# jacobwilliams/lbfgsb

Hardware: AMD Instinct MI355X
Metric: setulb iters/sec + achieved HBM GB/s on WS/WY matvec, n=1e8 m=10 (higher is better)
Workload: dtype f64; 1 GPU; separable bounded quadratic (SURVEY.md 8d), n=100000000, m=10, fp64, l=-1,u=1,x0=0, on-device objective; n=100000000, m=10, rows_per_gpu=100000000, parallelism=rows/1, collective=none, entry=lbfgsb_hip_setulb_dev_pp (ping-pong iterate buffers), defer_lnsrch=True

## Files before the change

### include/lbfgsb_hip_debug.h

```cpp
#ifndef LBFGSB_HIP_DEBUG_H
#define LBFGSB_HIP_DEBUG_H

#include "lbfgsb_hip.h"

#ifdef __cplusplus
extern "C" {
#endif

int lbfgsb_hip_wtv_launch_only(lbfgsb_hip_ctx *ctx, const void *v, int col, int head);
int lbfgsb_hip_wtv_time(lbfgsb_hip_ctx *ctx, const void *v, int col, int head, int reps,
                        double *h_ms_per_launch);
int lbfgsb_hip_kernel_time(lbfgsb_hip_ctx *ctx, int which, const void *x, const void *g, int col,
                           int head, int reps, double *h_ms_per_launch);

int lbfgsb_hip_stats(lbfgsb_hip_ctx *ctx, int64_t *launches, int64_t *syncs,
                     int64_t *cauchy_fullsorts, double *wait_seconds);

int lbfgsb_hip_freev_skipped(lbfgsb_hip_ctx *ctx, int64_t *count);
int lbfgsb_hip_bounds_stats(lbfgsb_hip_ctx *ctx, int64_t *checks, int64_t *changes, int64_t *rebuilds);

int lbfgsb_hip_comm_stats(lbfgsb_hip_ctx *ctx, int64_t *collectives, int64_t *bytes_contributed);

int lbfgsb_hip_path_counts(lbfgsb_hip_ctx *ctx, int64_t *closed_form, int64_t *three_pass,
                           int64_t *handed_windows);

int lbfgsb_hip_tie_splits(lbfgsb_hip_ctx *ctx, int64_t *count);

int lbfgsb_hip_host_gap(lbfgsb_hip_ctx *ctx, double *seconds, int64_t *count);
int lbfgsb_hip_compact_stats(lbfgsb_hip_ctx *ctx, int64_t *packs, int64_t *unpacks, int32_t *packed,
                             int32_t *eligible);
int lbfgsb_hip_collective_time(lbfgsb_hip_ctx *ctx, int reps, double *median_us, double *min_us);
int lbfgsb_hip_host_segments(lbfgsb_hip_ctx *ctx, double *seconds5);

int lbfgsb_hip_defer_stats(lbfgsb_hip_ctx *ctx, int64_t *deferred, int64_t *reissued);

int lbfgsb_hip_skip_stats(lbfgsb_hip_ctx *ctx, int64_t *scans_reused);

int lbfgsb_hip_pass_clock(lbfgsb_hip_ctx *ctx, int enable, double *ms_total, int64_t *count);

int lbfgsb_hip_refresh_count(lbfgsb_hip_ctx *ctx, int64_t *count);

#ifdef __cplusplus
}
#endif
#endif
```

### lbfgsb_amd/capi.py

```python
from __future__ import annotations

import ctypes as C
import os
import subprocess

HERE = os.path.dirname(os.path.abspath(__file__))
_LIB = None

_vp, _i32p, _dp, _cp = C.c_void_p, C.POINTER(C.c_int32), C.POINTER(C.c_double), C.c_char_p
ALLREDUCE_FN = C.CFUNCTYPE(C.c_int, C.c_void_p, C.POINTER(C.c_double), C.c_int, C.c_int, C.c_int)
ALLGATHER_FN = C.CFUNCTYPE(C.c_int, C.c_void_p, C.c_void_p, C.c_void_p, C.c_int64)
FG_FN = C.CFUNCTYPE(C.c_double, C.c_void_p, C.c_void_p, C.c_void_p)
PROTOTYPES = {
    "lbfgsb_hip_create": (C.c_int, [C.c_int64, C.c_int64, C.c_int64, C.c_int, C.c_int, C.c_int,
                                    _vp, C.POINTER(_vp)]),
    "lbfgsb_hip_destroy": (None, [_vp]),
    "lbfgsb_hip_last_error": (C.c_char_p, []),
    "lbfgsb_hip_rccl_unique_id": (C.c_int, [_vp]),
    "lbfgsb_hip_comm_init_rccl": (C.c_int, [_vp, _vp, C.c_int, C.c_int]),
    "lbfgsb_hip_comm_init_host": (C.c_int, [_vp, ALLREDUCE_FN, ALLGATHER_FN, _vp, C.c_int, C.c_int]),
    "lbfgsb_hip_setulb_dev": (C.c_int, [_vp, _vp, _vp, _vp, _vp, _vp, _vp, C.c_double, C.c_double,
                                        _vp, C.c_int, _vp, _vp, _vp, _vp]),
    "lbfgsb_hip_setulb_dev_pp": (C.c_int, [_vp, _vp, _vp, _vp, _vp, _vp, _vp, _vp, _vp, C.c_double,
                                           C.c_double, _vp, C.c_int, _vp, _vp, _vp, _vp, _vp]),
    "lbfgsb_hip_setulb_host": (C.c_int, [C.c_int32, C.c_int32, _vp, _vp, _vp, _vp, _vp, _vp,
                                         C.c_double, C.c_double, _vp, _vp, _vp, C.c_int32, _vp,
                                         _vp, _vp, _vp, _cp, C.c_int32, C.c_int32]),
    "lbfgsb_hip_setulb_host_ik": (C.c_int, [C.c_int64, C.c_int64, _vp, _vp, _vp, _vp, _vp, _vp,
                                            C.c_double, C.c_double, _vp, _vp, _vp, C.c_int64, _vp,
                                            _vp, _vp, _vp, _cp, C.c_int32, C.c_int32, C.c_int32]),
    "lbfgsb_hip_release_host_ik": (C.c_int, [_vp, C.c_int32]),
    "lbfgsb_hip_pass_clock": (C.c_int, [_vp, C.c_int, _vp, _vp]),
    "lbfgsb_hip_get_stream": (C.c_void_p, [_vp]),
    "lbfgsb_hip_wait_stream": (C.c_int, [_vp, _vp]),
    "lbfgsb_hip_release_host": (C.c_int, [_vp]),
    "lbfgsb_hip_host_pinning": (C.c_int, [C.c_int]),
    "lbfgsb_hip_return_event": (C.c_int, [_vp, _vp, C.c_int, _vp]),
    "lbfgsb_hip_f_device": (C.c_int, [_vp, _vp, _vp, C.c_int]),
    "lbfgsb_hip_tie_splits": (C.c_int, [_vp, _vp]),
    "lbfgsb_hip_defer_stats": (C.c_int, [_vp, _vp, _vp]),
    "lbfgsb_hip_host_gap": (C.c_int, [_vp, _vp, _vp]),
    "lbfgsb_hip_collective_time": (C.c_int, [_vp, C.c_int, _vp, _vp]),
    "lbfgsb_hip_compact_stats": (C.c_int, [_vp, _vp, _vp, _vp, _vp]),
    "lbfgsb_hip_host_segments": (C.c_int, [_vp, _vp]),
    "lbfgsb_hip_comm_info": (C.c_int, [_vp, _vp, _vp, _vp]),
    "lbfgsb_hip_path_counts": (C.c_int, [_vp, _vp, _vp, _vp]),
    "lbfgsb_hip_minimize": (C.c_int, [_vp, _vp, _vp, _vp, _vp, _vp, C.c_double, C.c_double, C.c_int,
                                      C.c_int, C.c_int, _vp, _vp, C.c_int, _vp, _vp, _vp, _vp, _vp]),
    "lbfgsb_hip_export_state": (C.c_int, [_vp, _vp, _vp]),
    "lbfgsb_hip_qn_apply": (C.c_int, [_vp, C.c_int, C.c_int64, _vp, C.c_int64, _vp, C.c_int64]),
    "lbfgsb_hip_qn_diag": (C.c_int, [_vp, C.c_int, _vp]),
    "lbfgsb_hip_qn_logdet": (C.c_int, [_vp, C.c_int, C.POINTER(C.c_double)]),
    "lbfgsb_hip_qn_draw": (C.c_int, [_vp, C.c_int, C.c_int64, C.c_uint64, C.c_int64, _vp, C.c_double, _vp,
                                     C.c_int64]),
    "lbfgsb_hip_qn_quad": (C.c_int, [_vp, C.c_int, C.c_int64, _vp, C.c_int64, _vp, C.POINTER(C.c_double)]),
    "lbfgsb_hip_qn_gram": (C.c_int, [_vp, C.c_int, C.c_int64, _vp, C.c_int64, _vp, C.POINTER(C.c_double),
                                     C.c_int64]),
    "lbfgsb_hip_qn_logpdf": (C.c_int, [_vp, C.c_int, C.c_int64, _vp, C.c_int64, _vp, C.c_double,
                                       C.POINTER(C.c_double)]),
    "lbfgsb_hip_qn_draw_logpdf": (C.c_int, [_vp, C.c_int, C.c_int64, C.c_uint64, C.c_int64, _vp, C.c_double, _vp,
                                            C.c_int64, C.POINTER(C.c_double)]),
    "lbfgsb_hip_qn_eig": (C.c_int, [_vp, C.c_int, C.c_int32, C.POINTER(C.c_int32), C.POINTER(C.c_double),
                                    C.POINTER(C.c_double)]),
    "lbfgsb_hip_qn_eigvec": (C.c_int, [_vp, C.c_int, C.c_int64, C.POINTER(C.c_int32), _vp, C.c_int64]),
    "lbfgsb_hip_kkt": (C.c_int, [_vp, _vp, _vp, _vp, _vp, _vp, C.c_double, _vp, _vp, _vp, _vp, _vp]),
    "lbfgsb_hip_kkt_list": (C.c_int, [_vp, _vp, C.c_int, _vp, C.c_int64, _vp]),
    "lbfgsb_hip_import_state": (C.c_int, [_vp, _vp, _vp, _vp]),
    "lbfgsb_hip_projgr": (C.c_int, [_vp, _vp, _vp, _vp, _vp, _vp, _vp]),
    "lbfgsb_hip_wtv": (C.c_int, [_vp, _vp, C.c_int, C.c_int, _vp]),
    "lbfgsb_hip_set_w": (C.c_int, [_vp, _vp, _vp]),
    "lbfgsb_hip_set_iwhere": (C.c_int, [_vp, _vp]),
    "lbfgsb_hip_formk_gram": (C.c_int, [_vp, C.c_int, C.c_int, _vp]),
    "lbfgsb_hip_wtv_launch_only": (C.c_int, [_vp, _vp, C.c_int, C.c_int]),
    "lbfgsb_hip_wtv_time": (C.c_int, [_vp, _vp, C.c_int, C.c_int, C.c_int, _vp]),
    "lbfgsb_hip_kernel_time": (C.c_int, [_vp, C.c_int, _vp, _vp, C.c_int, C.c_int, C.c_int, _vp]),
    "lbfgsb_hip_sync": (C.c_int, [_vp]),
    "lbfgsb_hip_objective": (C.c_int, [_vp, C.c_int, _vp, _vp, _vp]),
    "lbfgsb_hip_stats": (C.c_int, [_vp, _vp, _vp, _vp, _vp]),
    "lbfgsb_hip_set_option": (C.c_int, [_vp, _cp, C.c_double]),
    "lbfgsb_hip_comm_stats": (C.c_int, [_vp, _vp, _vp]),
    "lbfgsb_hip_uniform_bounds": (C.c_int, [_vp, _vp]),
    "lbfgsb_hip_bounds_changed": (C.c_int, [_vp]),
    "lbfgsb_hip_bounds_stats": (C.c_int, [_vp, _vp, _vp, _vp]),
    "lbfgsb_hip_freev_skipped": (C.c_int, [_vp, _vp]),
    "lbfgsb_hip_skip_stats": (C.c_int, [_vp, _vp]),
    "lbfgsb_hip_refresh_count": (C.c_int, [_vp, _vp]),
    "lbfgsb_hip_vec_sub": (C.c_int, [_vp, _vp, _vp, _vp]),
    "lbfgsb_hip_vec_scale": (C.c_int, [_vp, C.c_double, _vp]),
    "lbfgsb_hip_dot": (C.c_int, [_vp, _vp, _vp, _vp]),
    "lbfgsb_hip_active": (C.c_int, [_vp, _vp, _vp, _vp, _vp, _vp]),
    "lbfgsb_hip_errclb": (C.c_int, [_vp, _vp, _vp, _vp, C.c_double, _vp, _vp, _vp]),
    "lbfgsb_hip_cauchy": (C.c_int, [_vp, _vp, _vp, _vp, _vp, _vp, C.c_double, C.c_int, C.c_int, C.c_double,
                                    _vp, _vp, _vp]),
    "lbfgsb_hip_freev": (C.c_int, [_vp, C.c_int, C.c_int, C.c_int, _vp, _vp, _vp, _vp]),
    "lbfgsb_hip_formk": (C.c_int, [_vp, C.c_int, C.c_int, C.c_double, _vp]),
    "lbfgsb_hip_cmprlb": (C.c_int, [_vp, _vp, _vp, C.c_double, C.c_int, C.c_int, C.c_int, _vp, _vp]),
    "lbfgsb_hip_subsm": (C.c_int, [_vp, _vp, _vp, _vp, _vp, _vp, _vp, C.c_double, C.c_int, C.c_int, _vp, _vp,
                                   _vp]),
    "lbfgsb_hip_lnsrlb": (C.c_int, [_vp, _vp, _vp, _vp, _vp, _vp, C.c_double, _vp, _vp, _vp, _vp, _vp, _vp]),
    "lbfgsb_hip_matupd": (C.c_int, [_vp, _vp, C.c_double, C.c_double, C.c_double, _vp, _vp]),
}

E_NOGPU, E_ARG, E_ALLOC, E_COMM, E_STATE = -100, -101, -102, -103, -104
QN_B, QN_H = 0, 1
QN_B_SQRT, QN_H_SQRT = 4, 5
QN_ROOT_MAXCOL = 64
QN_EIG_CUT = 1e-8
KKT_CNT = ("n_unbounded", "n_free", "n_lower", "n_upper", "n_fixed", "n_binding", "n_weak", "n_leaving", "n_outside")
KKT_VAL = ("pg_max", "mult_max", "out_max", "gfree_max")
F_REAL32 = 1
F_MIRROR_INDEX = 2
F_NO_RETURN_SYNC = 4
F_PARALLEL_GCP = 8
F_EXACT_TIES = 16
F_INDEX_TIES = 32
F_DEFER_LNSRCH = 64
F_FOLLOW_BOUNDS = 128


class LbfgsbError(RuntimeError):
    pass


def lib_path() -> str:
    return os.environ.get("LBFGSB_HIP_LIBRARY") or os.path.join(HERE, "liblbfgsb_hip.so")


def build_library() -> str:
    subprocess.check_call(["make", "-s", "-C", os.path.join(HERE, "csrc")])
    return lib_path()


def load_library():
    global _LIB
    if _LIB is not None:
        return _LIB
    path = lib_path()
    if not os.path.exists(path):
        raise LbfgsbError("%s is missing: run lbfgsb_amd.build_library() (hipcc, gfx950). "
                          "There is no CPU fallback." % path)
    try:
        import torch
    except Exception:
        pass
    lib = C.CDLL(path, mode=C.RTLD_GLOBAL)
    for name, (res, args) in PROTOTYPES.items():
        fn = getattr(lib, name)
        fn.restype = res
        fn.argtypes = args
    _LIB = lib
    return lib


def check(rc: int):
    if rc != 0:
        msg = load_library().lbfgsb_hip_last_error()
        raise LbfgsbError("lbfgsb_hip error %d: %s" % (rc, (msg or b"").decode()))
```

### lbfgsb_amd/csrc/capi.hip

```cpp
#include "solver_base.hpp"

extern "C" {

const char *lbfgsb_hip_last_error(void) { return g_err.c_str(); }

int lbfgsb_hip_create(int64_t n_local, int64_t n_global, int64_t row0, int m, int flags,
                      int device, void *stream, lbfgsb_hip_ctx **out) {
  if (!out) return fail(LBFGSB_E_ARG, "out == NULL");
  *out = nullptr;
  if (n_local <= 0 || n_global < n_local || row0 < 0 || row0 + n_local > n_global)
    return fail(LBFGSB_E_ARG, "bad n_local / n_global / row0");
  if (m <= 0 || m > LBFGSB_MAX_M) return fail(LBFGSB_E_ARG, "m must be in 1..LBFGSB_MAX_M");
  if (n_local > (int64_t)INT32_MAX - 16) return fail(LBFGSB_E_ARG, "n_local must be < 2^31 - 16 rows per device");
  int rc = 0;
  *out = lbfgsb_make_solver(n_local, n_global, row0, m, flags, device, stream, &rc);
  if (!*out) return rc;
  return LBFGSB_OK;
}

void lbfgsb_hip_destroy(lbfgsb_hip_ctx *ctx) { delete ctx; }

int lbfgsb_hip_rccl_unique_id(void *id128) {
  if (!id128) return fail(LBFGSB_E_ARG, "rccl_unique_id: NULL argument");
  if (!g_rccl.load()) return fail(LBFGSB_E_COMM, "cannot load librccl");
// ... 194 lines not shown
  if (!qn_mode_ok(mode) && mode != LBFGSB_QN_B_SQRT && mode != LBFGSB_QN_H_SQRT)
    return fail(LBFGSB_E_ARG, "qn_apply: mode");
  if (k < 1 || ldv < ctx->n || ldo < ctx->n) return fail(LBFGSB_E_ARG, "qn_apply: k < 1 or ld < n_local");
  return ctx->qn_apply(mode, k, v, ldv, out, ldo);
}
int lbfgsb_hip_qn_diag(lbfgsb_hip_ctx *ctx, int mode, void *out) {
  if (!ctx || !out) return fail(LBFGSB_E_ARG, "qn_diag: NULL argument");
  if (!qn_mode_ok(mode)) return fail(LBFGSB_E_ARG, "qn_diag: mode");
  return ctx->qn_diag(mode, out);
}
int lbfgsb_hip_qn_logdet(lbfgsb_hip_ctx *ctx, int mode, double *h_logdet) {
  if (!ctx || !h_logdet) return fail(LBFGSB_E_ARG, "qn_logdet: NULL argument");
  if (!qn_mode_ok(mode)) return fail(LBFGSB_E_ARG, "qn_logdet: mode");
  return ctx->qn_logdet(mode, h_logdet);
}
int lbfgsb_hip_qn_draw(lbfgsb_hip_ctx *ctx, int mode, int64_t k, uint64_t seed, int64_t first, const void *mean,
                       double scale, void *out, int64_t ldo) {
  if (!ctx || !out) return fail(LBFGSB_E_ARG, "qn_draw: NULL argument");
  if (!qn_mode_ok(mode)) return fail(LBFGSB_E_ARG, "qn_draw: mode");
  if (k < 1 || first < 0 || ldo < ctx->n) return fail(LBFGSB_E_ARG, "qn_draw: k < 1, first < 0 or ldo < n_local");
  if (!std::isfinite(scale)) return fail(LBFGSB_E_ARG, "qn_draw: scale is not finite");
  return ctx->qn_draw(mode, k, seed, first, mean, scale, out, ldo);
}
int lbfgsb_hip_qn_quad(lbfgsb_hip_ctx *ctx, int mode, int64_t k, const void *v, int64_t ldv, const void *center,
                       double *h_q) {
  if (!ctx || !v || !h_q) return fail(LBFGSB_E_ARG, "qn_quad: NULL argument");
  if (!qn_mode_ok(mode)) return fail(LBFGSB_E_ARG, "qn_quad: mode");
  if (k < 1 || ldv < ctx->n) return fail(LBFGSB_E_ARG, "qn_quad: k < 1 or ldv < n_local");
  return ctx->qn_quad(mode, k, v, ldv, center, h_q);
}
int lbfgsb_hip_qn_logpdf(lbfgsb_hip_ctx *ctx, int mode, int64_t k, const void *x, int64_t ldx, const void *mean,
                         double scale, double *h_logp) {
  if (!ctx || !x || !h_logp) return fail(LBFGSB_E_ARG, "qn_logpdf: NULL argument");
  if (!qn_mode_ok(mode)) return fail(LBFGSB_E_ARG, "qn_logpdf: mode");
  if (k < 1 || ldx < ctx->n) return fail(LBFGSB_E_ARG, "qn_logpdf: k < 1 or ldx < n_local");
  if (!std::isfinite(scale) || scale == 0.0) return fail(LBFGSB_E_ARG, "qn_logpdf: scale is 0 or not finite");
  return ctx->qn_logpdf(mode, k, x, ldx, mean, scale, h_logp);
}
int lbfgsb_hip_qn_draw_logpdf(lbfgsb_hip_ctx *ctx, int mode, int64_t k, uint64_t seed, int64_t first,
                              const void *mean, double scale, void *out, int64_t ldo, double *h_logp) {
  if (!ctx || !out || !h_logp) return fail(LBFGSB_E_ARG, "qn_draw_logpdf: NULL argument");
  if (!qn_mode_ok(mode)) return fail(LBFGSB_E_ARG, "qn_draw_logpdf: mode");
  if (k < 1 || first < 0 || ldo < ctx->n)
    return fail(LBFGSB_E_ARG, "qn_draw_logpdf: k < 1, first < 0 or ldo < n_local");
  if (!std::isfinite(scale) || scale == 0.0)
    return fail(LBFGSB_E_ARG, "qn_draw_logpdf: scale is 0 or not finite");
  return ctx->qn_draw_logpdf(mode, k, seed, first, mean, scale, out, ldo, h_logp);
}
int lbfgsb_hip_qn_gram(lbfgsb_hip_ctx *ctx, int mode, int64_t k, const void *v, int64_t ldv, const void *center,
                       double *h_g, int64_t ldg) {
  if (!ctx || !v || !h_g) return fail(LBFGSB_E_ARG, "qn_gram: NULL argument");
  if (!qn_mode_ok(mode)) return fail(LBFGSB_E_ARG, "qn_gram: mode");
  if (k < 1 || k > LBFGSB_QN_GRAM_MAXK) return fail(LBFGSB_E_ARG, "qn_gram: k < 1 or k > LBFGSB_QN_GRAM_MAXK");
  if (ldv < ctx->n || ldg < k) return fail(LBFGSB_E_ARG, "qn_gram: ldv < n_local or ldg < k");
  return ctx->qn_vgram(mode, k, v, ldv, center, h_g, ldg);
}
int lbfgsb_hip_qn_eig(lbfgsb_hip_ctx *ctx, int mode, int32_t cap, int32_t *h_r, double *h_bulk, double *h_lambda) {
  if (!ctx || !h_r || !h_bulk) return fail(LBFGSB_E_ARG, "qn_eig: NULL argument");
  if (!qn_mode_ok(mode)) return fail(LBFGSB_E_ARG, "qn_eig: mode");
  if (cap < 0 || (cap > 0 && !h_lambda)) return fail(LBFGSB_E_ARG, "qn_eig: cap < 0, or cap > 0 without h_lambda");
  return ctx->qn_eig(mode, cap, h_r, h_bulk, h_lambda);
}
int lbfgsb_hip_qn_eigvec(lbfgsb_hip_ctx *ctx, int mode, int64_t k, const int32_t *h_which, void *out, int64_t ldo) {
  if (!ctx || !out) return fail(LBFGSB_E_ARG, "qn_eigvec: NULL argument");
  if (!qn_mode_ok(mode)) return fail(LBFGSB_E_ARG, "qn_eigvec: mode");
  if (k < 1 || k > 128 || ldo < ctx->n) return fail(LBFGSB_E_ARG, "qn_eigvec: k < 1, k > 128 or ldo < n_local");
  return ctx->qn_eigvec(mode, k, h_which, out, ldo);
}

int lbfgsb_hip_kkt(lbfgsb_hip_ctx *ctx, const void *x, const void *l, const void *u, const int32_t *nbd,
                   const void *g, double tol, void *pg_out, void *mult_out, int8_t *status_out, int64_t *h_cnt,
                   double *h_val) {
  if (!ctx || !x || !l || !u || !nbd || !g || !h_cnt || !h_val) return fail(LBFGSB_E_ARG, "kkt: NULL argument");
  if (!(tol >= 0.0)) return fail(LBFGSB_E_ARG, "kkt: tol is negative or NaN");
  return ctx->kkt(x, l, u, nbd, g, tol, pg_out, mult_out, status_out, h_cnt, h_val);
}
int lbfgsb_hip_kkt_list(lbfgsb_hip_ctx *ctx, const int8_t *status, int code_mask, int64_t *idx_out, int64_t cap,
                        int64_t *h_count) {
  if (!ctx || !status || !h_count) return fail(LBFGSB_E_ARG, "kkt_list: NULL argument");
  if (code_mask < 0 || code_mask > 31) return fail(LBFGSB_E_ARG, "kkt_list: code_mask has bits beyond the five codes");
  if (cap < 0 || (cap > 0 && !idx_out)) return fail(LBFGSB_E_ARG, "kkt_list: cap < 0, or cap > 0 without idx_out");
  return ctx->kkt_list(status, code_mask, idx_out, cap, h_count);
}

int lbfgsb_hip_projgr(lbfgsb_hip_ctx *ctx, const void *x, const void *l, const void *u,
                      const int32_t *nbd, const void *g, double *h_sbgnrm) {
  if (!ctx || !x || !l || !u || !nbd || !g || !h_sbgnrm) return fail(LBFGSB_E_ARG, "projgr: NULL argument");
  return ctx->k_projgr(x, l, u, nbd, g, h_sbgnrm);
}
int lbfgsb_hip_vec_sub(lbfgsb_hip_ctx *ctx, const void *a, const void *b, void *out) {
  if (!ctx || !a || !b || !out) return fail(LBFGSB_E_ARG, "vec_sub: NULL argument");
  return ctx->r_vec_sub(a, b, out);
}
int lbfgsb_hip_vec_scale(lbfgsb_hip_ctx *ctx, double alpha, void *v) {
  if (!ctx || !v) return fail(LBFGSB_E_ARG, "vec_scale: NULL argument");
  return ctx->r_vec_scale(alpha, v);
}
int lbfgsb_hip_dot(lbfgsb_hip_ctx *ctx, const void *a, const void *b, double *h_result) {
  if (!ctx || !a || !b || !h_result) return fail(LBFGSB_E_ARG, "dot: NULL argument");
  return ctx->r_dot(a, b, h_result);
}
int lbfgsb_hip_active(lbfgsb_hip_ctx *ctx, void *x, const void *l, const void *u, const int32_t *nbd,
                      int32_t *h_flags) {
  if (!ctx || !x || !l || !u || !nbd || !h_flags) return fail(LBFGSB_E_ARG, "active: NULL argument");
  return ctx->r_active(x, l, u, nbd, h_flags);
}
int lbfgsb_hip_errclb(lbfgsb_hip_ctx *ctx, const void *l, const void *u, const int32_t *nbd, double factr,
                      char *task, int32_t *h_info, int64_t *h_k) {
  if (!ctx || !l || !u || !nbd || !task || !h_info || !h_k) return fail(LBFGSB_E_ARG, "errclb: NULL argument");
  return ctx->r_errclb(l, u, nbd, factr, task, h_info, h_k);
}
int lbfgsb_hip_cauchy(lbfgsb_hip_ctx *ctx, const void *x, const void *l, const void *u, const int32_t *nbd,
                      const void *g, double theta, int col, int head, double sbgnrm, void *xcp_out,
                      int32_t *h_nseg, int32_t *h_info) {
  if (!ctx || !x || !l || !u || !nbd || !g || !h_nseg || !h_info)
    return fail(LBFGSB_E_ARG, "cauchy: NULL argument");
  return ctx->r_cauchy(x, l, u, nbd, g, theta, col, head, sbgnrm, xcp_out, h_nseg, h_info);
}
int lbfgsb_hip_freev(lbfgsb_hip_ctx *ctx, int iter, int cnstnd, int updatd, int64_t *h_nfree,
                     int64_t *h_nenter, int64_t *h_ileave, int32_t *h_wrk) {
  if (!ctx || !h_nfree || !h_nenter || !h_ileave || !h_wrk) return fail(LBFGSB_E_ARG, "freev: NULL argument");
  return ctx->r_freev(iter, cnstnd, updatd, h_nfree, h_nenter, h_ileave, h_wrk);
}
int lbfgsb_hip_formk(lbfgsb_hip_ctx *ctx, int col, int head, double theta, int32_t *h_info) {
  if (!ctx || !h_info) return fail(LBFGSB_E_ARG, "formk: NULL argument");
  return ctx->r_formk(col, head, theta, h_info);
}
int lbfgsb_hip_cmprlb(lbfgsb_hip_ctx *ctx, const void *x, const void *g, double theta, int col, int head,
                      int cnstnd, void *r_out, int32_t *h_info) {
  if (!ctx || !x || !g || !h_info) return fail(LBFGSB_E_ARG, "cmprlb: NULL argument");
  return ctx->r_cmprlb(x, g, theta, col, head, cnstnd, r_out, h_info);
}
int lbfgsb_hip_subsm(lbfgsb_hip_ctx *ctx, const void *x, const void *l, const void *u, const int32_t *nbd,
                     const void *g, const void *r_in, double theta, int col, int head, void *xhat_out,
                     int32_t *h_iword, int32_t *h_info) {
  if (!ctx || !x || !l || !u || !nbd || !g || !r_in || !h_iword || !h_info)
    return fail(LBFGSB_E_ARG, "subsm: NULL argument");
  return ctx->r_subsm(x, l, u, nbd, g, r_in, theta, col, head, xhat_out, h_iword, h_info);
}
int lbfgsb_hip_lnsrlb(lbfgsb_hip_ctx *ctx, void *x, const void *l, const void *u, const int32_t *nbd,
                      const void *g, double f, double *h_sc, int32_t *h_ic, char *task, char *csave,
                      int32_t *h_isave2, double *h_dsave13) {
  if (!ctx || !x || !l || !u || !nbd || !g || !h_sc || !h_ic || !task || !csave || !h_isave2 || !h_dsave13)
    return fail(LBFGSB_E_ARG, "lnsrlb: NULL argument");
  return ctx->r_lnsrlb(x, l, u, nbd, g, f, h_sc, h_ic, task, csave, h_isave2, h_dsave13);
}
int lbfgsb_hip_matupd(lbfgsb_hip_ctx *ctx, const void *g, double stp, double dr, double dtd, int32_t *h_ip,
                      double *h_theta) {
  if (!ctx || !g || !h_ip || !h_theta) return fail(LBFGSB_E_ARG, "matupd: NULL argument");
  return ctx->r_matupd(g, stp, dr, dtd, h_ip, h_theta);
}

int lbfgsb_hip_wtv(lbfgsb_hip_ctx *ctx, const void *v, int col, int head, double *h_out) {
  if (!ctx || !v || !h_out) return fail(LBFGSB_E_ARG, "wtv: NULL argument");
  return ctx->k_wtv(v, col, head, h_out, false);
}
int lbfgsb_hip_wtv_launch_only(lbfgsb_hip_ctx *ctx, const void *v, int col, int head) {
  if (!ctx || !v) return fail(LBFGSB_E_ARG, "wtv: NULL argument");
  return ctx->k_wtv(v, col, head, nullptr, true);
}
int lbfgsb_hip_wtv_time(lbfgsb_hip_ctx *ctx, const void *v, int col, int head, int reps,
                        double *h_ms_per_launch) {
  if (!ctx || !v || !h_ms_per_launch || reps < 1) return fail(LBFGSB_E_ARG, "wtv_time: bad arguments");
  HIPCHK(hipSetDevice(ctx->device));
  hipEvent_t e0 = nullptr, e1 = nullptr;
  GpuOwner tmp;
  HIPCHK(tmp.event(&e0));
  HIPCHK(tmp.event(&e1));
  for (int k = 0; k < 3; ++k) CHK(ctx->k_wtv(v, col, head, nullptr, true));
  HIPCHK(hipEventRecord(e0, ctx->q.stream));
  for (int k = 0; k < reps; ++k) CHK(ctx->k_wtv(v, col, head, nullptr, true));
  HIPCHK(hipEventRecord(e1, ctx->q.stream));
  HIPCHK(hipEventSynchronize(e1));
  float ms = 0.f;
  HIPCHK(hipEventElapsedTime(&ms, e0, e1));
  *h_ms_per_launch = (double)ms / reps;
  return 0;
}
int lbfgsb_hip_kernel_time(lbfgsb_hip_ctx *ctx, int which, const void *x, const void *g, int col,
                           int head, int reps, double *h_ms_per_launch) {
  if (!ctx || !x || !g || !h_ms_per_launch || reps < 1) return fail(LBFGSB_E_ARG, "kernel_time: bad arguments");
  HIPCHK(hipSetDevice(ctx->device));
  hipEvent_t e0 = nullptr, e1 = nullptr;
  GpuOwner tmp;
  HIPCHK(tmp.event(&e0));
  HIPCHK(tmp.event(&e1));
  for (int k = 0; k < 2; ++k) CHK(ctx->k_launch(which, x, g, col, head));
  HIPCHK(hipEventRecord(e0, ctx->q.stream));
  for (int k = 0; k < reps; ++k) CHK(ctx->k_launch(which, x, g, col, head));
  HIPCHK(hipEventRecord(e1, ctx->q.stream));
  HIPCHK(hipEventSynchronize(e1));
  float ms = 0.f;
  HIPCHK(hipEventElapsedTime(&ms, e0, e1));
  *h_ms_per_launch = (double)ms / reps;
  return 0;
}
int lbfgsb_hip_set_w(lbfgsb_hip_ctx *ctx, const void *h_ws, const void *h_wy) {
  if (!ctx || !h_ws || !h_wy) return fail(LBFGSB_E_ARG, "set_w: NULL argument");
  return ctx->k_set_w(h_ws, h_wy);
}
int lbfgsb_hip_set_iwhere(lbfgsb_hip_ctx *ctx, const int32_t *h_iwhere) {
  if (!ctx || !h_iwhere) return fail(LBFGSB_E_ARG, "set_iwhere: NULL argument");
  return ctx->k_set_iwhere(h_iwhere);
}
int lbfgsb_hip_formk_gram(lbfgsb_hip_ctx *ctx, int col, int head, double *h_out) {
  if (!ctx || !h_out) return fail(LBFGSB_E_ARG, "formk_gram: NULL argument");
  return ctx->k_formk_gram(col, head, h_out);
}
int lbfgsb_hip_sync(lbfgsb_hip_ctx *ctx) {
  if (!ctx) return fail(LBFGSB_E_ARG, "ctx == NULL");
  return ctx->sync();
}
int lbfgsb_hip_objective(lbfgsb_hip_ctx *ctx, int kind, const void *x, void *g, double *h_f) {
  if (!ctx || !x || !g) return fail(LBFGSB_E_ARG, "objective: NULL argument");
  return ctx->k_objective(kind, x, g, h_f);
}
int lbfgsb_hip_stats(lbfgsb_hip_ctx *ctx, int64_t *launches, int64_t *syncs,
                     int64_t *cauchy_fullsorts, double *wait_seconds) {
  if (!ctx) return fail(LBFGSB_E_ARG, "ctx == NULL");
  if (launches) *launches = ctx->q.launches;
  if (syncs) *syncs = ctx->nsync;
  if (cauchy_fullsorts) *cauchy_fullsorts = ctx->nfullsort;
  if (wait_seconds) *wait_seconds = ctx->t_wait;
  return 0;
}

int lbfgsb_hip_comm_stats(lbfgsb_hip_ctx *ctx, int64_t *collectives, int64_t *bytes_contributed) {
  if (!ctx) return fail(LBFGSB_E_ARG, "ctx == NULL");
  if (collectives) *collectives = ctx->ncoll;
  if (bytes_contributed) *bytes_contributed = ctx->coll_bytes;
  return 0;
}

int lbfgsb_hip_freev_skipped(lbfgsb_hip_ctx *ctx, int64_t *count) {
  if (!ctx || !count) return fail(LBFGSB_E_ARG, "freev_skipped: NULL argument");
  *count = ctx->freev_skipped();
  return 0;
}

int lbfgsb_hip_skip_stats(lbfgsb_hip_ctx *ctx, int64_t *scans_reused) {
  if (!ctx || !scans_reused) return fail(LBFGSB_E_ARG, "skip_stats: NULL argument");
  *scans_reused = ctx->skip_scans_reused();
  return 0;
}

int lbfgsb_hip_uniform_bounds(lbfgsb_hip_ctx *ctx, int32_t *mask) {
  if (!ctx || !mask) return fail(LBFGSB_E_ARG, "uniform_bounds: NULL argument");
  *mask = ctx->uniform_mask();
  return 0;
}

int lbfgsb_hip_bounds_changed(lbfgsb_hip_ctx *ctx) {
  if (!ctx) return fail(LBFGSB_E_ARG, "ctx == NULL");
  return ctx->bounds_changed();
}

int lbfgsb_hip_bounds_stats(lbfgsb_hip_ctx *ctx, int64_t *checks, int64_t *changes, int64_t *rebuilds) {
  if (!ctx) return fail(LBFGSB_E_ARG, "ctx == NULL");
  int64_t a = 0, b = 0, c = 0;
  ctx->bounds_stats(a, b, c);
  if (checks) *checks = a;
  if (changes) *changes = b;
  if (rebuilds) *rebuilds = c;
  return 0;
}

int lbfgsb_hip_path_counts(lbfgsb_hip_ctx *ctx, int64_t *closed_form, int64_t *three_pass,
                           int64_t *handed_windows) {
  if (!ctx) return fail(LBFGSB_E_ARG, "ctx == NULL");
  if (handed_windows) *handed_windows = ctx->nspecwin;
  int64_t a = 0, b = 0;
  ctx->path_counts(a, b);
  if (closed_form) *closed_form = a;
  if (three_pass) *three_pass = b;
  return 0;
}

int lbfgsb_hip_set_option(lbfgsb_hip_ctx *ctx, const char *name, double value) {
  if (!ctx || !name) return fail(LBFGSB_E_ARG, "set_option: NULL argument");
  return ctx->set_option(name, value);
}

int lbfgsb_hip_tie_splits(lbfgsb_hip_ctx *ctx, int64_t *count) {
  if (!ctx || !count) return fail(LBFGSB_E_ARG, "tie_splits: NULL argument");
  *count = ctx->ntiesplit;
  return 0;
}

int lbfgsb_hip_collective_time(lbfgsb_hip_ctx *ctx, int reps, double *median_us, double *min_us) {
  if (!ctx) return fail(LBFGSB_E_ARG, "ctx == NULL");
  return ctx->collective_time(reps, median_us, min_us);
}

int lbfgsb_hip_compact_stats(lbfgsb_hip_ctx *ctx, int64_t *packs, int64_t *unpacks, int32_t *packed,
                              int32_t *eligible) {
  if (!ctx) return fail(LBFGSB_E_ARG, "ctx == NULL");
  int64_t a = 0, b = 0;
  int c = 0, d = 0;
  ctx->compact_stats(a, b, c, d);
  if (packs) *packs = a;
  if (unpacks) *unpacks = b;
  if (packed) *packed = c;
  if (eligible) *eligible = d;
  return 0;
}

int lbfgsb_hip_refresh_count(lbfgsb_hip_ctx *ctx, int64_t *count) {
  if (!ctx || !count) return fail(LBFGSB_E_ARG, "refresh_count: NULL argument");
  *count = ctx->nrefresh;
  return 0;
}

int lbfgsb_hip_host_gap(lbfgsb_hip_ctx *ctx, double *seconds, int64_t *count) {
  if (!ctx) return fail(LBFGSB_E_ARG, "ctx == NULL");
  if (seconds) *seconds = ctx->t_mid;
  if (count) *count = ctx->n_mid;
  return 0;
}
int lbfgsb_hip_host_segments(lbfgsb_hip_ctx *ctx, double *seconds5) {
  if (!ctx || !seconds5) return fail(LBFGSB_E_ARG, "host_segments: NULL argument");
  for (int k = 0; k < 5; ++k) seconds5[k] = ctx->t_seg[k];
  return 0;
}

int lbfgsb_hip_defer_stats(lbfgsb_hip_ctx *ctx, int64_t *deferred, int64_t *reissued) {
  if (!ctx) return fail(LBFGSB_E_ARG, "ctx == NULL");
  int64_t a = 0, b = 0;
  ctx->defer_counts(a, b);
  if (deferred) *deferred = a;
  if (reissued) *reissued = b;
  return 0;
}

int lbfgsb_hip_pass_clock(lbfgsb_hip_ctx *ctx, int enable, double *ms_total, int64_t *count) {
  if (!ctx) return fail(LBFGSB_E_ARG, "ctx == NULL");
  HIPCHK(hipSetDevice(ctx->device));
  ctx->clk_stream = ctx->q.stream;
  if (enable == 1) {
    for (int k = 0; k < 3; ++k) {
      ctx->clk_ms[k] = 0.0, ctx->clk_n[k] = 0;
      for (bool &pnd : ctx->clk_pending[k]) pnd = false;
    }
    ctx->clk_dropped = 0;
    ctx->clock_on = true;
  } else {
    HIPCHK(hipStreamSynchronize(ctx->q.stream));
    ctx->clk_collect();
    if (enable == 0) ctx->clock_on = false;
  }
  for (int k = 0; k < 3; ++k) {
    if (ms_total) ms_total[k] = ctx->clk_ms[k];
    if (count) count[k] = ctx->clk_n[k];
  }
  return 0;
}

namespace {
constexpr int32_t HOST_TAG = 0x4C424642;
struct HostRegistry {
  std::mutex mu;
  std::unordered_map<int32_t, lbfgsb_hip_ctx *> live;
  int32_t next_id = 1;
  ~HostRegistry() { live.clear(); }
  int32_t add(lbfgsb_hip_ctx *c) {
    std::lock_guard<std::mutex> lk(mu);
    while (live.count(next_id) || next_id <= 0) next_id = next_id == INT32_MAX ? 1 : next_id + 1;
    live[next_id] = c;
    return next_id;
  }
  lbfgsb_hip_ctx *find(const int32_t *isave) {
    if (isave[17] != HOST_TAG) return nullptr;
    std::lock_guard<std::mutex> lk(mu);
    auto it = live.find(isave[16]);
    return it == live.end() ? nullptr : it->second;
  }
  void drop(int32_t *isave) {
    lbfgsb_hip_ctx *c = nullptr;
    if (isave[17] == HOST_TAG) {
      std::lock_guard<std::mutex> lk(mu);
      auto it = live.find(isave[16]);
      if (it != live.end()) {
        c = it->second;
        live.erase(it);
      }
    }
    delete c;
    isave[16] = isave[17] = 0;
  }
};
HostRegistry g_host;
std::atomic<int> g_host_pinning{1};

void drop_runs_overlapping(const void *const *ptr, const size_t *bytes, int cnt) {
  std::vector<lbfgsb_hip_ctx *> dead;
  {
    std::lock_guard<std::mutex> lk(g_host.mu);
    for (auto it = g_host.live.begin(); it != g_host.live.end();) {
      bool hit = false;
      for (const auto &r : it->second->host_reg)
        for (int k = 0; k < cnt && !hit; ++k)
          hit = r.p && ptr[k] && (const char *)ptr[k] < (const char *)r.p + r.bytes &&
                (const char *)r.p < (const char *)ptr[k] + bytes[k];
      if (hit) {
        dead.push_back(it->second);
        it = g_host.live.erase(it);
      } else {
        ++it;
      }
    }
  }
  for (lbfgsb_hip_ctx *c : dead) delete c;
}
}

int lbfgsb_hip_host_pinning(int mode) {
  if (mode != 0 && mode != 1) return fail(LBFGSB_E_ARG, "host_pinning: mode must be 0 or 1");
  g_host_pinning.store(mode);
  return 0;
}

int lbfgsb_hip_release_host(int32_t *isave) {
  if (!isave) return fail(LBFGSB_E_ARG, "isave == NULL");
  g_host.drop(isave);
  return 0;
}

static int setulb_host_impl(int64_t n, int64_t m, void *x, const void *l, const void *u, const void *nbd_,
                            void *f, void *g, double factr, double pgtol, void *wa, void *iwa_, char *task,
                            int32_t iprint, char *csave, void *lsave_, void *isave_, void *dsave,
                            const char *iteration_file, int32_t real_bytes, int32_t mirror, int int_bytes) {
  const bool r32 = real_bytes == 4;
  if (!x || !l || !u || !nbd_ || !f || !g || !task || !csave || !lsave_ || !isave_ || !dsave)
    return fail(LBFGSB_E_ARG, "setulb: NULL argument");
  if (mirror && (!wa || !iwa_)) return fail(LBFGSB_E_ARG, "setulb: mirror = 1 needs wa and iwa");
  if (real_bytes != 4 && real_bytes != 8) return fail(LBFGSB_E_ARG, "real_bytes must be 4 or 8");
  if (int_bytes != 4 && int_bytes != 8) return fail(LBFGSB_E_ARG, "int_bytes must be 4 or 8");
  const bool i8 = int_bytes == 8;
  const size_t rb = (size_t)real_bytes;
  int32_t isave[44], lsave[4];
  auto geti = [&](const void *p, int k) -> int64_t {
    return i8 ? ((const int64_t *)p)[k] : (int64_t)((const int32_t *)p)[k];
  };
  auto puti = [&](void *p, int k, int64_t v) {
    if (i8)
      ((int64_t *)p)[k] = v;
    else
      ((int32_t *)p)[k] = (int32_t)std::min<int64_t>(std::max<int64_t>(v, INT32_MIN), INT32_MAX);
  };
  for (int k = 0; k < 44; ++k) {
    const int64_t v = geti(isave_, k);
    isave[k] = (int32_t)std::min<int64_t>(std::max<int64_t>(v, INT32_MIN), INT32_MAX);
  }
  for (int k = 0; k < 4; ++k) lsave[k] = geti(lsave_, k) != 0;
  int64_t off64[16] = {0};
  bool have_off = false;
  auto finish_ints = [&]() {
    for (int k = 0; k < 44; ++k) puti(isave_, k, isave[k]);
    if (have_off)
      for (int k = 0; k < 16; ++k) puti(isave_, k, off64[k]);
    for (int k = 0; k < 4; ++k) puti(lsave_, k, lsave[k]);
  };
  auto upload_nbd = [&](int32_t *dst) -> int {
    std::vector<int32_t> nb;
    if (i8) {
      nb.resize((size_t)n);
      const int64_t *src = (const int64_t *)nbd_;
      for (int64_t k = 0; k < n; ++k) nb[(size_t)k] = (src[k] < 0 || src[k] > 3) ? -1 : (int32_t)src[k];
    }
    HIPCHK(hipMemcpy(dst, i8 ? (const void *)nb.data() : nbd_, (size_t)n * 4, hipMemcpyHostToDevice));
    return 0;
  };
  lbfgsb_hip_ctx *ctx = nullptr;
  const bool start = lbh::str60_eq(task, "START");
  if (start) {
    g_host.drop(isave);
    if (n <= 0 || m <= 0) {
      if (n <= 0) lbh::str60_set(task, "ERROR: N <= 0");
      if (m <= 0) lbh::str60_set(task, "ERROR: M <= 0");
      finish_ints();
      return 0;
    }
    if (m > LBFGSB_MAX_M) {
      lbh::str60_set(task, "ERROR: M > 1024 (LIMIT OF LBFGSB_HIP)");
      finish_ints();
      return 0;
    }
    if (n > (int64_t)INT32_MAX - 16) {
      lbh::str60_set(task, "ERROR: N >= 2**31 ON ONE DEVICE (LIMIT OF LBFGSB_HIP)");
      finish_ints();
      return 0;
    }
    int fl = (r32 ? LBFGSB_F_REAL32 : 0) | (mirror ? LBFGSB_F_MIRROR_INDEX : 0) | LBFGSB_F_NO_RETURN_SYNC;
    int rc = lbfgsb_hip_create(n, n, 0, (int)m, fl, 0, nullptr, &ctx);
    if (rc) return rc;
    if (g_host_pinning.load()) {
      void *tslot = (wa && !mirror) ? (char *)wa + (size_t)(2ll * m * n + 11ll * m * m + 3ll * n) * rb : nullptr;
      const void *pv[3] = {x, g, tslot};
      const size_t pb[3] = {(size_t)n * rb, (size_t)n * rb, (size_t)n * rb};
      drop_runs_overlapping(pv, pb, 3);
      ctx->host_register(0, x, pb[0]);
      ctx->host_register(1, g, pb[1]);
      if (tslot) ctx->host_register(2, tslot, pb[2]);
    }
    if (iteration_file && iteration_file[0]) ctx->itfile_name = iteration_file;
    const size_t vb = ((size_t)n + 32) * rb;
    auto stage = [&]() -> int {
      HIPCHK(ctx->own.device(&ctx->hx, vb));
      HIPCHK(ctx->own.device(&ctx->hg, vb));
      HIPCHK(ctx->own.device(&ctx->hl, vb));
      HIPCHK(ctx->own.device(&ctx->hu, vb));
      HIPCHK(ctx->own.device(&ctx->hnbd, ((size_t)n + 32) * 4));
      HIPCHK(hipMemset(ctx->hg, 0, vb));
      HIPCHK(hipMemcpy(ctx->hx, x, (size_t)n * rb, hipMemcpyHostToDevice));
      HIPCHK(hipMemcpy(ctx->hl, l, (size_t)n * rb, hipMemcpyHostToDevice));
      HIPCHK(hipMemcpy(ctx->hu, u, (size_t)n * rb, hipMemcpyHostToDevice));
      return upload_nbd(ctx->hnbd);
    };
    rc = stage();
    if (rc) {
      lbfgsb_hip_destroy(ctx);
      return rc;
    }
    std::memset(isave, 0, sizeof isave);
    isave[16] = g_host.add(ctx);
    isave[17] = HOST_TAG;
  } else {
    ctx = g_host.find(isave);
    if (!ctx || ctx->n != n || ctx->m != m)
      return fail(LBFGSB_E_STATE, "setulb called without a live context (task must be START first)");
    ctx->host_unregister_if_not(0, x);
    ctx->host_unregister_if_not(1, g);
    if (wa && !mirror)
      ctx->host_unregister_if_not(2, (char *)wa + (size_t)(2ll * m * n + 11ll * m * m + 3ll * n) * rb);
    if (lbh::str60_pre(task, "NEW_X") && (isave[29] == 1 || (isave[29] > 0 && isave[29] % 32 == 0))) {
      void *tl = nullptr, *tu = nullptr;
      int32_t *tn = nullptr;
      GpuOwner tmp;
      double ndiff = 0.0;
      auto check = [&]() -> int {
        const size_t vb = ((size_t)n + 32) * rb;
        HIPCHK(tmp.device(&tl, vb));
        HIPCHK(tmp.device(&tu, vb));
        HIPCHK(tmp.device(&tn, ((size_t)n + 32) * 4));
        HIPCHK(hipMemcpy(tl, l, (size_t)n * rb, hipMemcpyHostToDevice));
        HIPCHK(hipMemcpy(tu, u, (size_t)n * rb, hipMemcpyHostToDevice));
        CHK(upload_nbd(tn));
        return ctx->bounds_same(ctx->hl, ctx->hu, ctx->hnbd, tl, tu, tn, &ndiff);
      };
      int rcc = check();
      if (rcc && (!tl || !tu || !tn)) {
        (void)hipGetLastError();
        rcc = 0, ndiff = 0.0;
      }
      if (rcc) return rcc;
      if (ndiff != 0.0) {
        lbh::str60_set(task, "ERROR: BOUNDS CHANGED DURING RUN");
        if (iprint >= 0) std::printf("\n l, u or nbd were modified during the run (%.0f rows differ from the arrays of task = 'START').\n", ndiff);
        g_host.drop(isave);
        finish_ints();
        return 0;
      }
    }
    if (lbh::str60_pre(task, "FG"))
      HIPCHK(hipMemcpyAsync(ctx->hg, g, (size_t)n * rb, hipMemcpyHostToDevice, ctx->q.stream));
  }
  {
    const int64_t mn = m * n, mm = m * m;
    const int64_t lws = 1, lwy = lws + mn, lsy = lwy + mn, lss = lsy + mm, lwt = lss + mm,
                  lwn = lwt + mm, lsnd = lwn + 4 * mm, lz = lsnd + 4 * mm, lr = lz + n, ld_ = lr + n,
                  lt = ld_ + n, lxp = lt + n, lwa = lxp + n;
    const int64_t v[16] = {mn, mm, 4 * mm, lws, lwy, lsy, lss, lwt, lwn, lsnd, lz, lr, ld_, lt, lxp, lwa};
    std::memcpy(off64, v, sizeof off64);
    have_off = true;
  }
  const int32_t keep_id = isave[16], keep_tag = isave[17];
  double fd = r32 ? (double)*(float *)f : *(double *)f;
  double ds[29];
  for (int i = 0; i < 29; ++i) ds[i] = r32 ? (double)((float *)dsave)[i] : ((double *)dsave)[i];
  ctx->restored_xg = false;
  const int64_t setups0 = ctx->n_ls_setup;
  int rc = ctx->setulb_dev(ctx->hx, ctx->hl, ctx->hu, ctx->hnbd, &fd, ctx->hg, factr, pgtol, task,
                           iprint, csave, lsave, isave, ds);
  isave[16] = keep_id, isave[17] = keep_tag;
  if (iprint >= 0) std::fflush(stdout);
  if (rc) {
    if (start) g_host.drop(isave);
    return rc;
  }
  for (int i = 0; i < 29; ++i) {
    if (r32)
      ((float *)dsave)[i] = (float)ds[i];
    else
      ((double *)dsave)[i] = ds[i];
  }
  if (r32)
    *(float *)f = (float)fd;
  else
    *(double *)f = fd;
  hipStream_t st = ctx->q.stream;
  const bool x_back = start || ctx->restored_xg || lbh::str60_pre(task, "FG_LN");
  if (x_back) HIPCHK(hipMemcpyAsync(x, ctx->hx, (size_t)n * rb, hipMemcpyDeviceToHost, st));
  if (ctx->restored_xg) HIPCHK(hipMemcpyAsync(g, ctx->hg, (size_t)n * rb, hipMemcpyDeviceToHost, st));
  if (mirror) {
    HIPCHK(hipStreamSynchronize(st));
    if (i8) {
      std::vector<int32_t> iw((size_t)3 * (size_t)n);
// ... 56 lines not shown
```

### lbfgsb_amd/csrc/device_util.hpp

```cpp
#pragma once
#include <hip/hip_runtime.h>
#include <stdint.h>

#include <type_traits>

namespace lbk {

template <typename T>
struct VecOf;
template <>
struct VecOf<double> {
  static constexpr int V = 2;
};
template <>
struct VecOf<float> {
  static constexpr int V = 4;
};

template <int W>
using WTag = std::integral_constant<int, W>;

template <int W>
__device__ __forceinline__ void ld(const double *p, double (&o)[W]) {
  if constexpr (W == 2) {
// ... 87 lines not shown
  } else {
#pragma unroll
    for (int k = 0; k < W; ++k) __builtin_nontemporal_store(o[k], p + k);
  }
}
template <int W>
__device__ __forceinline__ void stnt(float *p, const double (&o)[W]) {
  if constexpr (W == 4) {
    typedef float f4 __attribute__((ext_vector_type(4)));
    f4 v = {(float)o[0], (float)o[1], (float)o[2], (float)o[3]};
    __builtin_nontemporal_store(v, reinterpret_cast<f4 *>(p));
  } else if constexpr (W == 2) {
    typedef float f2 __attribute__((ext_vector_type(2)));
    f2 v = {(float)o[0], (float)o[1]};
    __builtin_nontemporal_store(v, reinterpret_cast<f2 *>(p));
  } else {
#pragma unroll
    for (int k = 0; k < W; ++k) __builtin_nontemporal_store((float)o[k], p + k);
  }
}
template <int W>
__device__ __forceinline__ void ldi(const int32_t *p, int (&o)[W]) {
  if constexpr (W == 2) {
    int2 v = *reinterpret_cast<const int2 *>(p);
    o[0] = v.x;
    o[1] = v.y;
  } else if constexpr (W == 4) {
    int4 v = *reinterpret_cast<const int4 *>(p);
    o[0] = v.x;
    o[1] = v.y;
    o[2] = v.z;
    o[3] = v.w;
  } else {
#pragma unroll
    for (int k = 0; k < W; ++k) o[k] = p[k];
  }
}
template <int W>
__device__ __forceinline__ void ldi(const int8_t *p, int (&o)[W]) {
  if constexpr (W == 2) {
    const char2 v = *reinterpret_cast<const char2 *>(p);
    o[0] = v.x, o[1] = v.y;
  } else if constexpr (W == 4) {
    const char4 v = *reinterpret_cast<const char4 *>(p);
    o[0] = v.x, o[1] = v.y, o[2] = v.z, o[3] = v.w;
  } else {
#pragma unroll
    for (int k = 0; k < W; ++k) o[k] = p[k];
  }
}
template <int W>
__device__ __forceinline__ void sti(int8_t *p, const int (&o)[W]) {
  if constexpr (W == 2) {
    *reinterpret_cast<char2 *>(p) = make_char2((signed char)o[0], (signed char)o[1]);
  } else if constexpr (W == 4) {
    *reinterpret_cast<char4 *>(p) =
        make_char4((signed char)o[0], (signed char)o[1], (signed char)o[2], (signed char)o[3]);
  } else {
#pragma unroll
    for (int k = 0; k < W; ++k) p[k] = (int8_t)o[k];
  }
}
template <int W>
__device__ __forceinline__ void sti(int32_t *p, const int (&o)[W]) {
  if constexpr (W == 2) {
    *reinterpret_cast<int2 *>(p) = make_int2(o[0], o[1]);
  } else if constexpr (W == 4) {
    *reinterpret_cast<int4 *>(p) = make_int4(o[0], o[1], o[2], o[3]);
  } else {
#pragma unroll
    for (int k = 0; k < W; ++k) p[k] = o[k];
  }
}

typedef int i32x2_t __attribute__((ext_vector_type(2)));
typedef int i32x4_t __attribute__((ext_vector_type(4)));
template <int BYTES>
struct RawReg;
template <>
struct RawReg<16> {
  i32x4_t v;
};
template <>
struct RawReg<8> {
  i32x2_t v;
};
template <>
struct RawReg<4> {
  int v;
};
template <>
struct RawReg<2> {
  int v;
};
template <>
struct RawReg<1> {
  int v;
};
template <int BYTES, bool NT>
__device__ __forceinline__ void raw_issue(RawReg<BYTES> &r, const void *p) {
  if constexpr (BYTES == 16) {
    if constexpr (NT)
      r.v = __builtin_nontemporal_load(reinterpret_cast<const i32x4_t *>(p));
    else
      r.v = *reinterpret_cast<const i32x4_t *>(p);
  } else if constexpr (BYTES == 8) {
    if constexpr (NT)
      r.v = __builtin_nontemporal_load(reinterpret_cast<const i32x2_t *>(p));
    else
      r.v = *reinterpret_cast<const i32x2_t *>(p);
  } else if constexpr (BYTES == 4) {
    if constexpr (NT)
      r.v = __builtin_nontemporal_load(reinterpret_cast<const int *>(p));
    else
      r.v = *reinterpret_cast<const int *>(p);
  } else if constexpr (BYTES == 2) {
    r.v = (int)*reinterpret_cast<const unsigned short *>(p);
  } else {
    r.v = (int)*reinterpret_cast<const signed char *>(p);
  }
}
template <bool NT>
__device__ __forceinline__ void raw_issue_half(RawReg<16> &r, int half, const void *p) {
  i32x2_t v;
  if constexpr (NT)
    v = __builtin_nontemporal_load(reinterpret_cast<const i32x2_t *>(p));
  else
    v = *reinterpret_cast<const i32x2_t *>(p);
  if (half == 0)
    r.v.xy = v;
  else
    r.v.zw = v;
}
template <bool NT>
__device__ __forceinline__ void raw_issue_half_at(RawReg<16> &r, int half, const void *base, uint32_t byte_off) {
  raw_issue_half<NT>(r, half, (const char *)base + byte_off);
}
template <int N>
__device__ __forceinline__ void raw_wait() {
  __builtin_amdgcn_sched_barrier(0);
}
template <int BYTES>
__device__ __forceinline__ void raw_land(RawReg<BYTES> &) {}
template <int W>
__device__ __forceinline__ void raw_get(const RawReg<8 * W> &r, const double *, double (&o)[W]) {
  if constexpr (W == 2) {
    typedef double d2 __attribute__((ext_vector_type(2)));
    const d2 v = __builtin_bit_cast(d2, r.v);
    o[0] = v.x, o[1] = v.y;
  } else {
    static_assert(W == 1, "fp64: 1 or 2 rows per lane");
    o[0] = __builtin_bit_cast(double, r.v);
  }
}
template <int W>
__device__ __forceinline__ void raw_get(const RawReg<4 * W> &r, const float *, double (&o)[W]) {
  if constexpr (W == 4) {
    typedef float f4 __attribute__((ext_vector_type(4)));
    const f4 v = __builtin_bit_cast(f4, r.v);
    o[0] = v.x, o[1] = v.y, o[2] = v.z, o[3] = v.w;
  } else if constexpr (W == 2) {
    typedef float f2 __attribute__((ext_vector_type(2)));
    const f2 v = __builtin_bit_cast(f2, r.v);
    o[0] = v.x, o[1] = v.y;
  } else {
    static_assert(W == 1, "fp32: 1, 2 or 4 rows per lane");
    o[0] = __builtin_bit_cast(float, r.v);
  }
}
template <int W>
__device__ __forceinline__ void raw_geti(const RawReg<4 * W> &r, const int32_t *, int (&o)[W]) {
  if constexpr (W == 4) {
    o[0] = r.v.x, o[1] = r.v.y, o[2] = r.v.z, o[3] = r.v.w;
  } else if constexpr (W == 2) {
    o[0] = r.v.x, o[1] = r.v.y;
  } else {
    o[0] = r.v;
  }
}
template <int W>
__device__ __forceinline__ void raw_geti(const RawReg<W> &r, const int8_t *, int (&o)[W]) {
#pragma unroll
  for (int k = 0; k < W; ++k) o[k] = (int)(signed char)((unsigned)r.v >> (8 * k));
}
template <typename E, int W>
using RawOf = RawReg<(int)sizeof(E) * W>;

__device__ __forceinline__ int pair_xchg(int v) { return __builtin_amdgcn_update_dpp(0, v, 0xB1, 0xf, 0xf, true); }
__device__ __forceinline__ double pair_xchg(double v) {
  const long long b = __builtin_bit_cast(long long, v);
  const unsigned lo = (unsigned)pair_xchg((int)b), hi = (unsigned)pair_xchg((int)(b >> 32));
  return __builtin_bit_cast(double, (long long)(((unsigned long long)hi << 32) | lo));
}
__device__ __forceinline__ float pair_xchg(float v) {
  return __builtin_bit_cast(float, pair_xchg(__builtin_bit_cast(int, v)));
}
__device__ __forceinline__ void half_pair(int v, int &lo, int &hi) {
  const auto r = __builtin_amdgcn_permlane32_swap((unsigned)v, (unsigned)v, false, false);
  lo = (int)r[0], hi = (int)r[1];
}
__device__ __forceinline__ void half_pair(int64_t v, int64_t &lo, int64_t &hi) {
  int l0, h0, l1, h1;
  half_pair((int)v, l0, h0);
  half_pair((int)(v >> 32), l1, h1);
  lo = (int64_t)(((unsigned long long)(unsigned)l1 << 32) | (unsigned)l0);
  hi = (int64_t)(((unsigned long long)(unsigned)h1 << 32) | (unsigned)h0);
}
__device__ __forceinline__ void half_pair(double v, double &lo, double &hi) {
  int64_t l, h;
  half_pair(__builtin_bit_cast(int64_t, v), l, h);
  lo = __builtin_bit_cast(double, l), hi = __builtin_bit_cast(double, h);
}
__device__ __forceinline__ void half_pair(float v, float &lo, float &hi) {
  int l, h;
  half_pair(__builtin_bit_cast(int, v), l, h);
  lo = __builtin_bit_cast(float, l), hi = __builtin_bit_cast(float, h);
}
template <typename T, int MC>
struct RowsPer {
  static constexpr int V = MC >= 20 ? VecOf<T>::V / 2 : VecOf<T>::V;
};
template <typename T, int MC, int NACC>
struct RowsPerAcc {
  static constexpr int V0 = RowsPer<T, MC>::V;
  static constexpr int V =
      (V0 > 1 && (V0 / 2) * (int)sizeof(T) >= 8 && 2 * (2 * MC * V0 + NACC) > 240) ? V0 / 2 : V0;
};

template <typename T, int V = VecOf<T>::V, typename F>
__device__ __forceinline__ void for_rows(int64_t n, F &&f) {
  const int64_t nv = n / V;
  const int64_t stride = (int64_t)gridDim.x * blockDim.x;
  const int64_t t0 = (int64_t)blockIdx.x * blockDim.x + threadIdx.x;
  for (int64_t iv = t0; iv < nv; iv += stride) f(iv * V, WTag<V>{});
  const int64_t it = nv * V + t0;
  if (it < n) f(it, WTag<1>{});
}

template <typename TripV, typename Trip1, int V, bool PIPE, int NS, typename Ctx, typename F>
__device__ __forceinline__ void for_rows_raw(int64_t n, const Ctx &c, F &&f) {
  const int64_t nv = n / V;
  const int64_t stride = (int64_t)gridDim.x * blockDim.x;
  const int64_t t0 = (int64_t)blockIdx.x * blockDim.x + threadIdx.x;
  if constexpr (PIPE) {
    static_assert(TripV::NL + NS <= 63, "vmcnt counts to 63");
    if (t0 < nv) {
      TripV A, B;
      A.issue(c, t0 * V);
      int64_t n1 = t0 + stride;
      B.issue(c, (n1 < nv ? n1 : t0) * V);
      raw_wait<TripV::NL>();
      A.land();
      f(A, t0 * V, WTag<V>{});
      while (n1 < nv) {
        const int64_t n2 = n1 + stride;
        A.issue(c, (n2 < nv ? n2 : n1) * V);
        raw_wait<TripV::NL + NS>();
        B.land();
        f(B, n1 * V, WTag<V>{});
        if (n2 >= nv) break;
        const int64_t n3 = n2 + stride;
        B.issue(c, (n3 < nv ? n3 : n2) * V);
        raw_wait<TripV::NL + NS>();
        A.land();
        f(A, n2 * V, WTag<V>{});
        n1 = n3;
      }
      raw_wait<0>();
      A.land();
      B.land();
    }
  } else {
    for (int64_t iv = t0; iv < nv; iv += stride) {
      TripV A;
      A.issue(c, iv * V);
      raw_wait<0>();
      A.land();
      f(A, iv * V, WTag<V>{});
    }
  }
  const int64_t it = nv * V + t0;
  if (it < n) {
    Trip1 C;
    C.issue(c, it);
    raw_wait<0>();
    C.land();
    f(C, it, WTag<1>{});
  }
}

struct CwTile {
  int64_t tb;
  uint64_t m0, m1;
};
__device__ __forceinline__ void cw_slots(const CwTile &t, int (&sl)[2], bool (&lf)[2]) {
  const int lane = (int)(threadIdx.x & 63);
  const int c0 = __popcll(t.m0), tf = c0 + __popcll(t.m1);
  const int b0 = (int)__builtin_amdgcn_mbcnt_hi((uint32_t)(t.m0 >> 32), __builtin_amdgcn_mbcnt_lo((uint32_t)t.m0, 0u));
  const int b1 = c0 + (int)__builtin_amdgcn_mbcnt_hi((uint32_t)(t.m1 >> 32), __builtin_amdgcn_mbcnt_lo((uint32_t)t.m1, 0u));
  lf[0] = (t.m0 >> lane) & 1ull, lf[1] = (t.m1 >> lane) & 1ull;
  sl[0] = lf[0] ? b0 : tf + (lane - b0);
  sl[1] = lf[1] ? b1 : tf + (64 + lane - b1);
}
__device__ __forceinline__ int64_t wave_uniform(int64_t v) {
  return (int64_t)(((uint64_t)(uint32_t)__builtin_amdgcn_readfirstlane((int)(v >> 32)) << 32) |
                   (uint32_t)__builtin_amdgcn_readfirstlane((int)v));
}
template <typename Trip2, typename Trip1, typename Ctx, typename F>
__device__ __forceinline__ void for_tiles_cw(int64_t n, const Ctx &c, const uint64_t *__restrict__ lmask, F &&f) {
  const int lane = threadIdx.x & 63;
  const int64_t nfull = n >> 7;
  const int64_t stride = (int64_t)gridDim.x * (blockDim.x >> 6);
  const int64_t t0 = wave_uniform((int64_t)blockIdx.x * (blockDim.x >> 6) + (threadIdx.x >> 6));
  if (t0 < nfull) {
    uint64_t m0 = lmask[2 * t0], m1 = lmask[2 * t0 + 1];
    for (int64_t tr = t0;;) {
      const int64_t nx = tr + stride;
      const bool more = nx < nfull;
      const int64_t nxc = more ? nx : tr;
      const uint64_t m0n = lmask[2 * nxc], m1n = lmask[2 * nxc + 1];
      Trip2 A;
      A.issue_cw(c, CwTile{tr << 7, m0, m1});
      raw_wait<0>();
      A.land();
      f(A, tr << 7, WTag<2>{});
      if (!more) break;
      tr = nx, m0 = m0n, m1 = m1n;
    }
  }
  if ((n & 127) != 0 && t0 == nfull % stride) {
    const CwTile t{nfull << 7, lmask[2 * nfull], lmask[2 * nfull + 1]};
    int sl[2];
    bool lf[2];
    cw_slots(t, sl, lf);
    const int64_t i0 = t.tb + lane, i1 = i0 + 64;
    const bool v0 = i0 < n, v1 = i1 < n;
    Trip1 A, B;
    A.issue_cw(c, v0 ? i0 : n - 1, t.tb + sl[0], lf[0], t.tb);
    B.issue_cw(c, v1 ? i1 : n - 1, t.tb + sl[1], lf[1], t.tb);
    raw_wait<0>();
    A.land();
    B.land();
    if (v0) f(A, i0, WTag<1>{});
    if (v1) f(B, i1, WTag<1>{});
  }
}

template <typename Trip1, typename Ctx, typename F>
__device__ __forceinline__ void for_halves_cw(int64_t n, const Ctx &c, const uint64_t *__restrict__ lmask, F &&f) {
  const int lane = threadIdx.x & 63;
  const int64_t nh = n >> 6;
  const int64_t stride = (int64_t)gridDim.x * (blockDim.x >> 6);
  const int64_t t0 = wave_uniform((int64_t)blockIdx.x * (blockDim.x >> 6) + (threadIdx.x >> 6));
  auto issue = [&](Trip1 &A, int64_t h, uint64_t m0, uint64_t m1, int64_t row_limit) {
    const bool hi = (h & 1) != 0;
    const int c0 = __popcll(m0), tf = c0 + __popcll(m1);
    const uint64_t mw = hi ? m1 : m0;
    const int b = (hi ? c0 : 0) +
                  (int)__builtin_amdgcn_mbcnt_hi((uint32_t)(mw >> 32), __builtin_amdgcn_mbcnt_lo((uint32_t)mw, 0u));
    const bool lf = (mw >> lane) & 1ull;
    const int r = (hi ? 64 : 0) + lane;
    const int64_t tb = (h >> 1) << 7;
    int64_t i = (h << 6) + lane;
    if (i >= row_limit) i = row_limit - 1;
    A.issue_cw(c, i, tb + (lf ? b : tf + (r - b)), lf, tb);
  };
  if (t0 < nh) {
    const int64_t last = nh - 1;
    auto cl = [&](int64_t h) { return h < nh ? h : last; };
    uint64_t m0 = lmask[(t0 >> 1) * 2], m1 = lmask[(t0 >> 1) * 2 + 1];
    for (int64_t h = t0;;) {
      const int64_t nx = h + stride, nxc = cl(nx);
      const uint64_t m0n = lmask[(nxc >> 1) * 2], m1n = lmask[(nxc >> 1) * 2 + 1];
      Trip1 A;
      issue(A, h, m0, m1, n);
      raw_wait<0>();
      A.land();
      f(A, (h << 6) + lane, WTag<1>{});
      if (nx >= nh) break;
      h = nx, m0 = m0n, m1 = m1n;
    }
  }
  if ((n & 63) != 0 && t0 == nh % stride) {
    const uint64_t m0 = lmask[(nh >> 1) * 2], m1 = lmask[(nh >> 1) * 2 + 1];
    Trip1 A;
    issue(A, nh, m0, m1, n);
    raw_wait<0>();
    A.land();
    if ((nh << 6) + lane < n) f(A, (nh << 6) + lane, WTag<1>{});
  }
}

template <int CTRL>
__device__ __forceinline__ double dpp_mov(double v) {
  const long long b = __builtin_bit_cast(long long, v);
  const unsigned lo = (unsigned)__builtin_amdgcn_update_dpp(0, (int)b, CTRL, 0xf, 0xf, true);
  const unsigned hi = (unsigned)__builtin_amdgcn_update_dpp(0, (int)(b >> 32), CTRL, 0xf, 0xf, true);
  return __builtin_bit_cast(double, (long long)(((unsigned long long)hi << 32) | lo));
}
constexpr int DPP_XOR1 = 0xB1;
constexpr int DPP_XOR2 = 0x4E;
constexpr int DPP_HALF_MIRROR = 0x141;
constexpr int DPP_MIRROR = 0x140;
constexpr int DPP_ROR8 = 0x128;
template <int OP>
__device__ __forceinline__ double red_op(double a, double b) {
  return OP == 0 ? a + b : (OP == 1 ? fmin(a, b) : fmax(a, b));
}
template <int OP>
__device__ __forceinline__ double row_reduce(double v) {
  v = red_op<OP>(v, dpp_mov<DPP_XOR1>(v));
  v = red_op<OP>(v, dpp_mov<DPP_XOR2>(v));
  v = red_op<OP>(v, dpp_mov<DPP_HALF_MIRROR>(v));
  v = red_op<OP>(v, dpp_mov<DPP_MIRROR>(v));
  return v;
}
__device__ __forceinline__ double lane_bcast(double v, int lane) {
  const long long b = __builtin_bit_cast(long long, v);
  const unsigned lo = (unsigned)__builtin_amdgcn_readlane((int)b, lane);
  const unsigned hi = (unsigned)__builtin_amdgcn_readlane((int)(b >> 32), lane);
  return __builtin_bit_cast(double, (long long)(((unsigned long long)hi << 32) | lo));
}
template <int OP>
__device__ __forceinline__ double wave_reduce(double v) {
  v = row_reduce<OP>(v);
  return red_op<OP>(red_op<OP>(red_op<OP>(lane_bcast(v, 0), lane_bcast(v, 16)), lane_bcast(v, 32)),
                    lane_bcast(v, 48));
}
__device__ __forceinline__ double wave_sum(double v) { return wave_reduce<0>(v); }
__device__ __forceinline__ double wave_min(double v) { return wave_reduce<1>(v); }
__device__ __forceinline__ double wave_max(double v) { return wave_reduce<2>(v); }

template <int N, int CTRL>
__device__ __forceinline__ void row_halve(const double (&in)[N], double (&out)[N / 2], bool up) {
  static_assert(N % 2 == 0, "even slot count");
#pragma unroll
  for (int p = 0; p < N / 2; ++p) {
    const double keep = up ? in[p + N / 2] : in[p];
    const double send = up ? in[p] : in[p + N / 2];
    out[p] = keep + dpp_mov<CTRL>(send);
  }
}

template <int K>
__device__ __forceinline__ void block_reduce_store(const double (&acc)[K], int nsum, int nmin,
                                                   int nmax, double *__restrict__ part,
                                                   int pstride) {
  constexpr bool SCATTER = K >= 16;
  constexpr int KP = SCATTER ? (K + 15) / 16 * 16 : K;
  __shared__ double sm[16][KP];
  const int lane = threadIdx.x & 63, w = threadIdx.x >> 6;
  const int rr = w * 4 + (lane >> 4);
  const int ntot = nsum + nmin + nmax;
  if constexpr (SCATTER) {
    double t0[KP];
#pragma unroll
    for (int k = 0; k < KP; ++k) t0[k] = k < K ? acc[k] : 0.0;
    double t1[KP / 2], t2[KP / 4], t3[KP / 8], t4[KP / 16];
    const bool b0 = lane & 1, b1 = lane & 2, b2 = lane & 4, b3 = lane & 8;
    row_halve<KP, DPP_HALF_MIRROR>(t0, t1, b2);
    row_halve<KP / 2, DPP_XOR1>(t1, t2, b0);
    row_halve<KP / 4, DPP_XOR2>(t2, t3, b1);
    row_halve<KP / 8, DPP_ROR8>(t3, t4, b3);
    const int base = (b2 ? KP / 2 : 0) + (b0 ? KP / 4 : 0) + (b1 ? KP / 8 : 0) + (b3 ? KP / 16 : 0);
#pragma unroll
    for (int p = 0; p < KP / 16; ++p)
      if (base + p < nsum) sm[rr][base + p] = t4[p];
  } else {
#pragma unroll
    for (int k = 0; k < K; ++k)
      if (k < nsum) {
        const double v = row_reduce<0>(acc[k]);
        if ((lane & 15) == 0) sm[rr][k] = v;
      }
  }
#pragma unroll
  for (int k = 0; k < K; ++k) {
    if (k >= nsum && k < ntot) {
      const double v = k < nsum + nmin ? row_reduce<1>(acc[k]) : row_reduce<2>(acc[k]);
      if ((lane & 15) == 0) sm[rr][k] = v;
    }
  }
  __syncthreads();
  for (int k = threadIdx.x; k < ntot; k += blockDim.x) {
    double s = sm[0][k];
    if (k < nsum) {
#pragma unroll
      for (int q = 1; q < 16; ++q) s = s + sm[q][k];
    } else if (k < nsum + nmin) {
#pragma unroll
      for (int q = 1; q < 16; ++q) s = fmin(s, sm[q][k]);
    } else {
#pragma unroll
      for (int q = 1; q < 16; ++q) s = fmax(s, sm[q][k]);
    }
    part[(size_t)k * pstride + blockIdx.x] = s;
  }
}

}
```

### lbfgsb_amd/csrc/k_subsm.hip

```cpp
#include "kernels_common.hpp"

namespace lbk {

template <int MC, bool FULL = false>
__device__ __forceinline__ double subsm_dir(double xk, double zk, double gk, const double (&a)[MC],
                                            const double (&b)[MC], int col, double theta,
                                            double rtheta, const Coef &cf, const Coef &wv) {
  double dk = -theta * (zk - xk) - gk;
#pragma unroll
  for (int j = 0; j < MC; ++j)
    if (FULL || j < col) dk = dk + a[j] * cf.a[j] + b[j] * cf.a[MAXM + j];
#pragma unroll
  for (int j = 0; j < MC; ++j)
    if (FULL || j < col) dk = dk + a[j] * wv.a[j] / theta + b[j] * wv.a[MAXM + j];
  return rtheta * dk;
}

template <typename T>
struct SubsmCtx {
  const T *l, *u, *xx, *gg, *ws, *wy, *zero, *r, *pd;
  const nb_t *nbd;
  const iw_t *iwhere;
  int64_t ldw;
  int m, head, col;
  Pend pe;
  int ub;
};
template <typename T, int MC, int W>
struct SubsmRegs {
  RawOf<T, W> rl, ru, rx, rg, ra[MC], rb[MC];
  RawOf<nb_t, W> rnb;
  RawOf<iw_t, W> riw;
};
template <typename T, int MC, int W, bool NT, bool PSPEC>
struct SubsmTrip : SubsmRegs<T, MC, W>, NaturalRows<W> {
  static constexpr int NL = 6 + 2 * MC;
  __device__ __forceinline__ void issue(const SubsmCtx<T> &c, int64_t i) {
    constexpr int B = (int)sizeof(T) * W;
    raw_issue<B, NT>(this->rl, (c.ub & 1) ? c.l : c.l + i);
    raw_issue<B, NT>(this->ru, (c.ub & 2) ? c.u : c.u + i);
    raw_issue<B, NT>(this->rx, c.xx + i);
    raw_issue<B, NT>(this->rg, c.gg + i);
    raw_issue<W, false>(this->rnb, (c.ub & 4) ? c.nbd : c.nbd + i);
    raw_issue<W, false>(this->riw, c.iwhere + i);
    issue_cols<T, MC, W, NT, PSPEC>(c.wy, c.ws, c.r, c.pd, c.zero, i, c.col, c.head, c.m, c.ldw, c.pe,
                                    this->ra, this->rb);
  }
  __device__ __forceinline__ void land() {}
};
template <typename T, int MC, bool PSPEC>
__device__ __forceinline__ void subsm_cw_col(const SubsmCtx<T> &c, int j, int64_t i, int64_t slot, bool want,
                                             const T *&py, const T *&ps) {
  if constexpr (PSPEC) {
    if (j == MC - 1) {
      py = c.r + i, ps = c.pd + i;
    } else {
      const int64_t off = (int64_t)((c.head - 1 + j) % c.m) * c.ldw + slot;
      py = want ? c.wy + off : c.zero, ps = want ? c.ws + off : c.zero;
    }
  } else {
    const int64_t off = col_off(j, c.col, c.head, c.m, c.ldw) + slot;
    const bool live = j < c.col, pj = c.pe.on && j == c.col - 1;
    py = !live ? c.zero : (pj ? c.r + i : (want ? c.wy + off : c.zero));
    ps = !live ? c.zero : (pj ? c.pd + i : (want ? c.ws + off : c.zero));
  }
}
template <typename T, int MC, bool NT, bool PSPEC>
struct SubsmTripCW1 : SubsmRegs<T, MC, 1>, CwOneRow {
  static constexpr int NL = 6 + 2 * MC;
  template <bool NTL>
  __device__ __forceinline__ void cols(const SubsmCtx<T> &c, int64_t srow) {
    constexpr int B = (int)sizeof(T);
#pragma unroll
    for (int j = 0; j < MC; ++j) {
      const T *py, *ps;
      subsm_cw_col<T, MC, PSPEC>(c, j, this->ri_, srow, true, py, ps);
      raw_issue<B, NTL>(this->ra[j], py);
      raw_issue<B, NTL>(this->rb[j], ps);
    }
  }
  __device__ __forceinline__ void issue_cw(const SubsmCtx<T> &c, int64_t i, int64_t slot, bool lf, int64_t first) {
    constexpr int B = (int)sizeof(T);
    this->ri_ = i, this->ws_ = slot, this->lf_ = lf;
    raw_issue<B, NT>(this->rl, (c.ub & 1) ? c.l : c.l + i);
    raw_issue<B, NT>(this->ru, (c.ub & 2) ? c.u : c.u + i);
    raw_issue<B, NT>(this->rx, c.xx + i);
    raw_issue<B, NT>(this->rg, c.gg + i);
    raw_issue<1, false>(this->rnb, (c.ub & 4) ? c.nbd : c.nbd + i);
    raw_issue<1, false>(this->riw, c.iwhere + i);
    cols<NT>(c, lf ? slot : first);
  }
  __device__ __forceinline__ void land() {}
};
template <typename T, int MC, bool NT, bool PSPEC>
struct SubsmTripCW2 : SubsmRegs<T, MC, 2>, CwPairRows {
  static_assert(sizeof(T) == 8, "compact W: fp64");
  static constexpr int NL = 2 * (6 + 2 * MC);
  RawReg<1> nb_[2], iw_[2];
  template <bool NTL>
  __device__ __forceinline__ void cols_row(const SubsmCtx<T> &c, int k, int64_t srow) {
#pragma unroll
    for (int j = 0; j < (PSPEC ? MC - 1 : MC); ++j) {
      const int64_t off = (PSPEC ? (int64_t)((c.head - 1 + j) % c.m) * c.ldw : col_off(j, c.col, c.head, c.m, c.ldw)) + srow;
      const bool stored = PSPEC || (j < c.col && !(c.pe.on && j == c.col - 1));
      if (PSPEC || stored || j >= c.col) {
        raw_issue_half<NTL>(this->ra[j], k, stored ? c.wy + off : c.zero);
        raw_issue_half<NTL>(this->rb[j], k, stored ? c.ws + off : c.zero);
      }
    }
  }
  __device__ __forceinline__ void issue_cw(const SubsmCtx<T> &c, const CwTile &t) {
    this->tile_ = t;
    const int lane = (int)(threadIdx.x & 63);
#pragma unroll
    for (int k = 0; k < 2; ++k) {
      const int64_t i = t.tb + (lane + 64 * k);
      raw_issue_half<NT>(this->rl, k, (c.ub & 1) ? c.l : c.l + i);
      raw_issue_half<NT>(this->ru, k, (c.ub & 2) ? c.u : c.u + i);
      raw_issue_half<NT>(this->rx, k, c.xx + i);
      raw_issue_half<NT>(this->rg, k, c.gg + i);
      raw_issue<1, false>(nb_[k], (c.ub & 4) ? c.nbd : c.nbd + i);
      raw_issue<1, false>(iw_[k], c.iwhere + i);
      if constexpr (PSPEC) {
        raw_issue_half<NT>(this->ra[MC - 1], k, c.r + i);
        raw_issue_half<NT>(this->rb[MC - 1], k, c.pd + i);
      } else if (c.pe.on) {
#pragma unroll
        for (int j = 0; j < MC; ++j)
          if (j == c.col - 1) {
            raw_issue_half<NT>(this->ra[j], k, c.r + i);
            raw_issue_half<NT>(this->rb[j], k, c.pd + i);
          }
      }
    }
    int sl[2];
    bool lf[2];
    cw_slots(t, sl, lf);
    cols_row<false>(c, 0, t.tb + (lf[0] ? sl[0] : 0));
    cols_row<false>(c, 1, t.tb + (lf[1] ? sl[1] : 0));
  }
  __device__ __forceinline__ void land() {
    raw_join_bytes(this->rnb, nb_[0], nb_[1]);
    raw_join_bytes(this->riw, iw_[0], iw_[1]);
  }
};
template <typename T, int MC, bool NT, bool PSPEC, bool PIPE, bool CW = false>
__global__ __launch_bounds__(BLOCK) void subsm_update_kernel(
    int64_t n, double tsum, T *__restrict__ zout, const T *pr, T *rout,
    const T *__restrict__ l, const T *__restrict__ u, const nb_t *__restrict__ nbd,
    const iw_t *__restrict__ iwhere, const T *xx, const T *__restrict__ gg,
    const T *__restrict__ ws, const T *__restrict__ wy, const T *__restrict__ zero, int64_t ldw,
    int m, int head, int col, double theta, Coef cf, Coef wv, T *dvec, T *tvec,
    T *xout, int do_stpmx, Pend pe, const T *pd, T *cwy, T *cws, int ub, double *part, int pstride,
    const uint64_t *__restrict__ lmask = nullptr) {
  static_assert(!CW || (sizeof(T) == 8 && MC <= 10 && !PIPE), "compact W: fp64, MC <= 10, one trip in flight");
  double acc[SUBSM_SIZE] = {0.0, 0.0, 0.0, 1.0e10};
  const double rtheta = 1.0 / theta;
  constexpr int V = RowsPer<T, MC>::V;
  constexpr int NS = PSPEC ? 3 : 1;
  const SubsmCtx<T> ctx{l, u, xx, gg, ws, wy, zero, pr, pd, nbd, iwhere, ldw, m, head, col, pe, ub};
  __shared__ T dict[16];
  dict_fill<T>(dict, l, u, ub);
  auto body = [&](auto &tr, int64_t i, auto wt) {
    constexpr int W = decltype(wt)::value;
    double zv[W], lv[W], uv[W], xv[W], gv[W], a[MC][W], b[MC][W];
    int nb[W], iw[W];
    raw_get<W>(tr.rl, (const T *)nullptr, lv);
    raw_get<W>(tr.ru, (const T *)nullptr, uv);
    raw_get<W>(tr.rx, (const T *)nullptr, xv);
    raw_get<W>(tr.rg, (const T *)nullptr, gv);
    raw_geti<W>(tr.rnb, (const nb_t *)nullptr, nb);
    raw_geti<W>(tr.riw, (const iw_t *)nullptr, iw);
    dict_apply<T, W>(dict, ub, nb, lv, uv);
    if constexpr (std::remove_reference_t<decltype(tr)>::CW) {
#pragma unroll
      for (int k = 0; k < W; ++k)
        if (!tr.lf(k) && iw[k] <= 0) acc[SUBSM_IWORD] += 1.0e30;
    }
    get_cols<T, MC, W>(tr.ra, tr.rb, a, b);
    fix_pending<T, MC, W, PSPEC>(col, pe, gv, xv, a, b);
    if (PSPEC || pe.on) {
      double yn[W], sn[W];
      newest_cols<MC, W, PSPEC>(col, a, b, yn, sn);
      tr.template st_w<NT>(cwy, i, yn);
      tr.template st_w<NT>(cws, i, sn);
    }
#pragma unroll
    for (int k = 0; k < W; ++k) zv[k] = xcp_row<T>(xv[k], gv[k], iw[k], lv[k], uv[k], tsum);
    double dv[W];
#pragma unroll
    for (int k = 0; k < W; ++k) {
      if (iw[k] <= 0) {
        double ak[MC], bk[MC];
#pragma unroll
        for (int j = 0; j < MC; ++j) ak[j] = a[j][k], bk[j] = b[j][k];
        const double dk = subsm_dir<MC, PSPEC>(xv[k], zv[k], gv[k], ak, bk, col, theta, rtheta, cf, wv);
        const double xk = zv[k];
        if (nb[k] != 0) {
          if (nb[k] == 1) {
            zv[k] = fmax(lv[k], xk + dk);
            if (zv[k] == lv[k]) acc[SUBSM_IWORD] += 1.0;
          } else if (nb[k] == 2) {
            const double t1 = fmax(lv[k], xk + dk);
            zv[k] = fmin(uv[k], t1);
            if (zv[k] == lv[k] || zv[k] == uv[k]) acc[SUBSM_IWORD] += 1.0;
          } else if (nb[k] == 3) {
            zv[k] = fmin(uv[k], xk + dk);
            if (zv[k] == uv[k]) acc[SUBSM_IWORD] += 1.0;
          }
        } else {
          zv[k] = xk + dk;
        }
      }
      dv[k] = zv[k] - xv[k];
      acc[SUBSM_DDP] = acc[SUBSM_DDP] + dv[k] * gv[k];
      acc[SUBSM_DTD] = acc[SUBSM_DTD] + dv[k] * dv[k];
      if (do_stpmx && nb[k] != 0) {
        const double a1 = dv[k];
        if (a1 < 0.0 && nb[k] <= 2) {
          const double a2 = lv[k] - xv[k];
          acc[SUBSM_STPMX] = fmin(acc[SUBSM_STPMX], a2 >= 0.0 ? 0.0 : a2 / a1);
        } else if (a1 > 0.0 && nb[k] >= 2) {
          const double a2 = uv[k] - xv[k];
          acc[SUBSM_STPMX] = fmin(acc[SUBSM_STPMX], a2 <= 0.0 ? 0.0 : a2 / a1);
        }
      }
    }
    if (zout) tr.template st_rows<NT>(zout, i, zv);
    if (dvec) tr.template st_rows<NT>(dvec, i, dv);
    if (tvec) tr.template st_rows<NT>(tvec, i, xv);
    if (rout) tr.template st_rows<NT>(rout, i, gv);
    if (xout) tr.template st_rows<NT>(xout, i, zv);
  };
  if constexpr (CW)
    for_tiles_cw<SubsmTripCW2<T, MC, NT, PSPEC>, SubsmTripCW1<T, MC, NT, PSPEC>>(n, ctx, lmask, body);
  else
    for_rows_raw<SubsmTrip<T, MC, V, NT, PSPEC>, SubsmTrip<T, MC, 1, NT, PSPEC>, V, PIPE, NS>(n, ctx, body);
  block_reduce_store<SUBSM_SIZE>(acc, SUBSM_NSUM, 1, 0, part, pstride);
}
template <typename T>
void launch_subsm_update(Queue &q, int64_t n, double tsum, T *zout, const T *pr, T *rout, const T *l,
                         const T *u, const nb_t *nbd, const iw_t *iwhere, const T *xx, const T *gg,
                         WStore<T> w, int head, int col, double theta, const Coef &cf,
                         const Coef &wv, T *dvec, T *tvec, T *xout, int do_stpmx, Pend pe,
                         const T *pd, int ub) {
  int gr = 0;
  const int64_t slot = (int64_t)((head - 1 + col - 1) % w.m) * w.ld;
  const bool spec = pe.on && col == maxc_for(col);
  double *part = q.part();
  const int pstride = MAX_BLOCKS;
  if (w.lmask) {
    bool done = false;
    if constexpr (sizeof(T) == 8) {
      if (col <= 10) {
#define LB_SUBSM_CW(MCV, NTV, PSPECV)                                                                           \
  {                                                                                                             \
    gr = grid_for_w(q, n, VecOf<T>::V, (const void *)&subsm_update_kernel<T, MCV, NTV, PSPECV, false, true>);   \
    hipLaunchKernelGGL((subsm_update_kernel<T, MCV, NTV, PSPECV, false, true>), dim3(gr), dim3(BLOCK), 0,       \
                       q.stream, n, tsum, zout, pr, rout, l, u, nbd, iwhere, xx, gg, w.ws, w.wy, w.zero, w.ld,   \
                       w.m, head, col, theta, cf, wv, dvec, tvec, xout, do_stpmx, pe, pd, w.wy + slot,          \
                       w.ws + slot, ub, part, pstride, w.lmask);                                                \
  }
        if (col <= 5) {
          if (q.nt) { if (spec) LB_SUBSM_CW(5, true, true) else LB_SUBSM_CW(5, true, false) }
          else { if (spec) LB_SUBSM_CW(5, false, true) else LB_SUBSM_CW(5, false, false) }
        } else {
          if (q.nt) { if (spec) LB_SUBSM_CW(10, true, true) else LB_SUBSM_CW(10, true, false) }
          else { if (spec) LB_SUBSM_CW(10, false, true) else LB_SUBSM_CW(10, false, false) }
        }
#undef LB_SUBSM_CW
        LB_LAUNCHED(q);
        finalize_from(q, part, pstride, gr, SUBSM_NSUM, 1, 0);
        done = true;
      }
    }
    if (!done && q.launch_err == hipSuccess)
      q.launch_err = hipErrorInvalidValue, q.launch_err_where = "subsm_update: compact W needs fp64, col <= 10";
    return;
  }
#define LB_SUBSM(PSPECV)                                                                            \
  DISPATCH_MAXC_NT(col, q.nt, DISPATCH_PIPE(MC, {                                                   \
                     gr = grid_for_w(q, n, VecOf<T>::V,                                             \
                                     (const void *)&subsm_update_kernel<T, MC, NTV, PSPECV, PIPEV>); \
                     hipLaunchKernelGGL((subsm_update_kernel<T, MC, NTV, PSPECV, PIPEV>), dim3(gr), \
                                        dim3(BLOCK), 0, q.stream, n, tsum, zout, pr, rout, l, u,    \
                                        nbd, iwhere, xx, gg, w.ws, w.wy, w.zero, w.ld, w.m, head,   \
                                        col, theta, cf, wv, dvec, tvec, xout, do_stpmx, pe, pd,     \
                                        w.wy + slot, w.ws + slot, ub, part, pstride);               \
                   }))
  if (spec)
    LB_SUBSM(true);
  else
    LB_SUBSM(false);
#undef LB_SUBSM
  LB_LAUNCHED(q);
  finalize_from(q, part, pstride, gr, SUBSM_NSUM, 1, 0);
}

template <typename T, int MC, bool NT>
__global__ __launch_bounds__(BLOCK) void subsm_dir_kernel(
    int64_t n, const T *__restrict__ xcp, const iw_t *__restrict__ iwhere,
    const T *__restrict__ xx, const T *__restrict__ gg, const T *__restrict__ ws,
    const T *__restrict__ wy, const T *__restrict__ zero, int64_t ldw, int m, int head, int col,
    double theta, Coef cf, Coef wv, T *__restrict__ ndir) {
  const double rtheta = 1.0 / theta;
  for_rows<T, RowsPer<T, MC>::V>(n, [&](int64_t i, auto wt) {
    constexpr int W = decltype(wt)::value;
    double zv[W], xv[W], gv[W], a[MC][W], b[MC][W], out[W];
    int iw[W];
    ldx<W, NT>(xcp + i, zv);
    ldx<W, NT>(xx + i, xv);
    ldx<W, NT>(gg + i, gv);
    ldi<W>(iwhere + i, iw);
#pragma unroll
    for (int j = 0; j < MC; ++j) {
      const int64_t off = col_off(j, col, head, m, ldw) + i;
      ld_col<T, W, NT>(j < col, wy + off, zero, a[j]);
      ld_col<T, W, NT>(j < col, ws + off, zero, b[j]);
    }
#pragma unroll
    for (int k = 0; k < W; ++k) {
      out[k] = 0.0;
      if (iw[k] <= 0) {
        double ak[MC], bk[MC];
#pragma unroll
        for (int j = 0; j < MC; ++j) ak[j] = a[j][k], bk[j] = b[j][k];
        out[k] = subsm_dir<MC>(xv[k], zv[k], gv[k], ak, bk, col, theta, rtheta, cf, wv);
      }
    }
    st<W>(ndir + i, out);
  });
}
template <typename T>
void launch_subsm_dir(Queue &q, int64_t n, const T *xcp, const iw_t *iwhere, const T *xx,
                      const T *gg, WStore<T> w, int head, int col, double theta, const Coef &cf,
                      const Coef &wv, T *ndir) {
  const int gr = grid_for_w(q, n, VecOf<T>::V);
  DISPATCH_MAXC_NT(col, q.nt, hipLaunchKernelGGL((subsm_dir_kernel<T, MC, NTV>), dim3(gr), dim3(BLOCK), 0,
                                        q.stream, n, xcp, iwhere, xx, gg, w.ws, w.wy, w.zero, w.ld, w.m,
                                        head, col, theta, cf, wv, ndir));
  LB_LAUNCHED(q);
}

#define INSTANTIATE(T) \
  template void launch_subsm_update<T>(Queue &, int64_t, double, T *, const T *, T *, const T *, const T *, const nb_t *, const iw_t *, const T *, const T *, WStore<T>, int, int, double, const Coef &, const Coef &, T *, T *, T *, int, Pend, const T *, int); \
  template void launch_subsm_dir<T>(Queue &, int64_t, const T *, const iw_t *, const T *, const T *, WStore<T>, int, int, double, const Coef &, const Coef &, T *);
INSTANTIATE(double)
INSTANTIATE(float)
#undef INSTANTIATE

}
```

### lbfgsb_amd/csrc/k_update.hip

```cpp
#include "kernels_common.hpp"

namespace lbk {

template <typename T, int MC, bool NT>
__global__ __launch_bounds__(BLOCK) void update_pairs_kernel(
    int64_t n, const T *__restrict__ g, const T *__restrict__ r, const T *__restrict__ d,
    double stp, T *ws, T *wy, const T *__restrict__ zero, int64_t ldw, int m, int head, int nold,
    int itail, double *part) {
  static constexpr UpdatePairsSlots S{MC};
  constexpr int NA = S.size();
  double acc[NA];
#pragma unroll
  for (int k = 0; k < NA; ++k) acc[k] = 0.0;
  const int64_t offn = (int64_t)(itail - 1) * ldw;
  for_rows<T, RowsPer<T, MC>::V>(n, [&](int64_t i, auto wt) {
    constexpr int W = decltype(wt)::value;
    double gv[W], rv[W], dv[W], a[MC][W], b[MC][W];
    ldx<W, NT>(g + i, gv);
    ldx<W, NT>(r + i, rv);
    ldx<W, NT>(d + i, dv);
#pragma unroll
    for (int j = 0; j < MC; ++j) {
      const int64_t off = col_off(j, nold, head, m, ldw) + i;
      ld_col<T, W, NT>(j < nold, wy + off, zero, a[j]);
      ld_col<T, W, NT>(j < nold, ws + off, zero, b[j]);
    }
#pragma unroll
    for (int k = 0; k < W; ++k) {
      rv[k] = gv[k] - rv[k];
      acc[S.yy()] = acc[S.yy()] + rv[k] * rv[k];
      if (stp != 1.0) dv[k] = stp * dv[k];
    }
#pragma unroll
    for (int j = 0; j < MC; ++j) {
#pragma unroll
      for (int k = 0; k < W; ++k) {
        acc[S.sy(j)] += dv[k] * a[j][k];
        acc[S.ss(j)] += b[j][k] * dv[k];
      }
    }
    st<W>(ws + offn + i, dv);
    st<W>(wy + offn + i, rv);
  });
  block_reduce_store<NA>(acc, NA, 0, 0, part, MAX_BLOCKS);
}
template <typename T>
void launch_update_pairs(Queue &q, int64_t n, const T *g, const T *r, const T *d, double stp,
                         WStore<T> w, int head, int col, int itail) {
  const int gr = grid_for_w(q, n, VecOf<T>::V);
  const int nold = col - 1;
  DISPATCH_MAXC_NT(nold, q.nt, hipLaunchKernelGGL((update_pairs_kernel<T, MC, NTV>), dim3(gr), dim3(BLOCK), 0,
                                         q.stream, n, g, r, d, stp, w.ws, w.wy, w.zero, w.ld, w.m,
                                         head, nold, itail, q.part()));
  LB_LAUNCHED(q);
  launch_finalize(q, gr, UpdatePairsSlots{maxc_for(nold)}.size(), 0, 0);
}

template <typename T, bool FUSED = false>
__device__ __forceinline__ double dot_term(double acc, double a, double b) {
  if constexpr (sizeof(T) == 4 || FUSED)
    return __builtin_fma(a, b, acc);
  else
    return acc + a * b;
}
template <typename T>
struct UpdScanCtx {
  const T *x, *l, *u, *g, *r, *d, *ws, *wy, *zero;
  const nb_t *nbd;
  const iw_t *iwhere;
  int64_t ldw;
  int m, head, nold;
  int ub;
  const unsigned long long *ptab;
};
template <typename T, int MC, int W>
struct UpdScanRegs {
  RawOf<T, W> rx, rl, ru, rg, rr, rd, ra[MC], rb[MC];
  RawOf<nb_t, W> rnb;
  RawOf<iw_t, W> riw;
};
template <typename T, int MC, int W, bool NT>
struct UpdScanTrip : UpdScanRegs<T, MC, W>, NaturalRows<W> {
  static constexpr int NL = 8 + 2 * MC;
  __device__ __forceinline__ void issue(const UpdScanCtx<T> &c, int64_t i) {
    constexpr int B = (int)sizeof(T) * W;
    raw_issue<B, NT>(this->rx, c.x + i);
    raw_issue<B, NT>(this->rl, (c.ub & 1) ? c.l : c.l + i);
    raw_issue<B, NT>(this->ru, (c.ub & 2) ? c.u : c.u + i);
    raw_issue<B, NT>(this->rg, c.g + i);
    raw_issue<B, NT>(this->rr, c.r + i);
    raw_issue<B, NT>(this->rd, c.d + i);
    raw_issue<W, false>(this->rnb, (c.ub & 4) ? c.nbd : c.nbd + i);
    raw_issue<W, false>(this->riw, c.iwhere + i);
    issue_cols<T, MC, W, NT>(c.wy, c.ws, (const T *)nullptr, (const T *)nullptr, c.zero, i, c.nold, c.head,
                             c.m, c.ldw, Pend{0, 1.0}, this->ra, this->rb);
  }
  __device__ __forceinline__ void land() {}
};
template <typename T, int MC, bool NT>
struct UpdScanTripCW1 : UpdScanRegs<T, MC, 1>, CwOneRow {
  static constexpr int NL = 8 + 2 * MC;
  __device__ __forceinline__ void issue_cw(const UpdScanCtx<T> &c, int64_t i, int64_t slot, bool lf, int64_t first) {
    constexpr int B = (int)sizeof(T);
    this->ri_ = i, this->ws_ = slot, this->lf_ = lf;
    raw_issue<B, NT>(this->rx, c.x + i);
    raw_issue<B, NT>(this->rl, (c.ub & 1) ? c.l : c.l + i);
    raw_issue<B, NT>(this->ru, (c.ub & 2) ? c.u : c.u + i);
    raw_issue<B, NT>(this->rg, c.g + i);
    raw_issue<B, NT>(this->rr, c.r + i);
    raw_issue<B, NT>(this->rd, c.d + i);
    raw_issue<1, false>(this->rnb, (c.ub & 4) ? c.nbd : c.nbd + i);
    raw_issue<1, false>(this->riw, c.iwhere + i);
    cols<false>(c, lf ? slot : first);
  }
  template <bool NTL>
  __device__ __forceinline__ void cols(const UpdScanCtx<T> &c, int64_t srow) {
    constexpr int B = (int)sizeof(T);
#pragma unroll
    for (int j = 0; j < MC; ++j) {
      const int64_t off = col_off(j, c.nold, c.head, c.m, c.ldw) + srow;
      const bool live = j < c.nold;
      raw_issue<B, NTL>(this->ra[j], live ? c.wy + off : c.zero);
      raw_issue<B, NTL>(this->rb[j], live ? c.ws + off : c.zero);
    }
  }
  __device__ __forceinline__ void land() {}
  __device__ __forceinline__ void reload_cols(const UpdScanCtx<T> &c, const bool (&miss)[1]) {
    constexpr int B = (int)sizeof(T);
    RawOf<T, 1> ty[MC], ts[MC];
#pragma unroll
    for (int j = 0; j < MC; ++j) {
      const int64_t off = col_off(j, c.nold, c.head, c.m, c.ldw) + (miss[0] ? this->ws_ : this->ri_ & ~(int64_t)127);
      const bool live = j < c.nold;
      raw_issue<B, false>(ty[j], live ? c.wy + off : c.zero);
      raw_issue<B, false>(ts[j], live ? c.ws + off : c.zero);
    }
#pragma unroll
    for (int j = 0; j < MC; ++j) {
      this->ra[j].v = miss[0] ? ty[j].v : this->ra[j].v;
      this->rb[j].v = miss[0] ? ts[j].v : this->rb[j].v;
    }
  }
};
template <typename T, int MC, bool NT>
struct UpdScanTripCW2 : UpdScanRegs<T, MC, 2>, CwPairRows {
  static_assert(sizeof(T) == 8, "compact W: fp64");
  static constexpr int NL = 2 * (8 + 2 * MC);
  RawReg<1> nb_[2], iw_[2];
  template <bool NTL>
  __device__ __forceinline__ void cols_row(const UpdScanCtx<T> &c, int k, int64_t srow) {
#pragma unroll
    for (int j = 0; j < MC; ++j) {
      const int64_t off = col_off(j, c.nold, c.head, c.m, c.ldw) + srow;
      const bool live = j < c.nold;
      raw_issue_half<NTL>(this->ra[j], k, live ? c.wy + off : c.zero);
      raw_issue_half<NTL>(this->rb[j], k, live ? c.ws + off : c.zero);
    }
  }
  __device__ __forceinline__ void issue_cw(const UpdScanCtx<T> &c, const CwTile &t) {
    this->tile_ = t;
    const int lane = (int)(threadIdx.x & 63);
#pragma unroll
    for (int k = 0; k < 2; ++k) {
      const int64_t i = t.tb + (lane + 64 * k);
      raw_issue_half<NT>(this->rx, k, c.x + i);
      raw_issue_half<NT>(this->rl, k, (c.ub & 1) ? c.l : c.l + i);
      raw_issue_half<NT>(this->ru, k, (c.ub & 2) ? c.u : c.u + i);
      raw_issue_half<NT>(this->rg, k, c.g + i);
      raw_issue_half<NT>(this->rr, k, c.r + i);
      raw_issue_half<NT>(this->rd, k, c.d + i);
      raw_issue<1, false>(nb_[k], (c.ub & 4) ? c.nbd : c.nbd + i);
      raw_issue<1, false>(iw_[k], c.iwhere + i);
    }
    int sl[2];
    bool lf[2];
    cw_slots(t, sl, lf);
    cols_row<false>(c, 0, t.tb + (lf[0] ? sl[0] : 0));
    cols_row<false>(c, 1, t.tb + (lf[1] ? sl[1] : 0));
  }
  __device__ __forceinline__ void land() {
    raw_join_bytes(this->rnb, nb_[0], nb_[1]);
    raw_join_bytes(this->riw, iw_[0], iw_[1]);
  }
  __device__ __forceinline__ void reload_cols(const UpdScanCtx<T> &c, const bool (&miss)[2]) {
    int sl[2];
    bool lf[2];
    cw_slots(this->tile_, sl, lf);
    RawReg<8> ty[MC][2], ts[MC][2];
#pragma unroll
    for (int j = 0; j < MC; ++j) {
      const int64_t off = col_off(j, c.nold, c.head, c.m, c.ldw) + this->tile_.tb;
      const bool live = j < c.nold;
#pragma unroll
      for (int k = 0; k < 2; ++k) {
        raw_issue<8, false>(ty[j][k], live ? c.wy + off + (miss[k] ? sl[k] : 0) : c.zero);
        raw_issue<8, false>(ts[j][k], live ? c.ws + off + (miss[k] ? sl[k] : 0) : c.zero);
      }
    }
#pragma unroll
    for (int j = 0; j < MC; ++j) {
      if (miss[0]) this->ra[j].v.xy = ty[j][0].v, this->rb[j].v.xy = ts[j][0].v;
      if (miss[1]) this->ra[j].v.zw = ty[j][1].v, this->rb[j].v.zw = ts[j][1].v;
    }
  }
};
template <typename T, int MC, int W, bool NT>
struct UpdScanPairTrip : NaturalRows<W> {
  static constexpr int H = MC / 2;
  static constexpr int NL = 8 + 2 * H;
  RawOf<T, W> rx, rl, ru, rg, rr, rd;
  RawOf<T, 2 * W> ra[H], rb[H];
  RawOf<nb_t, W> rnb;
  RawOf<iw_t, W> riw;
  __device__ __forceinline__ void issue(const UpdScanCtx<T> &c, int64_t i) {
    constexpr int B = (int)sizeof(T) * W;
    const bool hi = threadIdx.x & 1;
    const int64_t i0 = i - (hi ? W : 0);
    int tb = hi ? 2 * H : 0;
    asm volatile("" : "+v"(tb));
    typedef unsigned long long u64x2 __attribute__((ext_vector_type(2)));
    u64x2 p[H];
#pragma unroll
    for (int jj = 0; jj < H; ++jj) p[jj] = *reinterpret_cast<const u64x2 *>(c.ptab + tb + 2 * jj);
    __builtin_amdgcn_sched_barrier(0);
    raw_issue<B, NT>(rx, c.x + i);
    raw_issue<B, NT>(rl, (c.ub & 1) ? c.l : c.l + i);
    raw_issue<B, NT>(ru, (c.ub & 2) ? c.u : c.u + i);
    raw_issue<B, NT>(rg, c.g + i);
    raw_issue<B, NT>(rr, c.r + i);
    raw_issue<B, NT>(rd, c.d + i);
    raw_issue<W, false>(rnb, (c.ub & 4) ? c.nbd : c.nbd + i);
    raw_issue<W, false>(riw, c.iwhere + i);
#pragma unroll
    for (int jj = 0; jj < H; ++jj) {
      const int64_t o = (hi && H + jj >= c.nold) ? 0 : i0;
      typedef const __attribute__((address_space(1))) T *gptr;
      raw_issue<2 * B, NT>(ra[jj], (const T *)((gptr)p[jj].x + o));
      raw_issue<2 * B, NT>(rb[jj], (const T *)((gptr)p[jj].y + o));
    }
  }
  __device__ __forceinline__ void land() {
    raw_land(rx);
    raw_land(rl);
    raw_land(ru);
    raw_land(rg);
    raw_land(rr);
    raw_land(rd);
    raw_land(rnb);
    raw_land(riw);
#pragma unroll
    for (int jj = 0; jj < H; ++jj) {
      raw_land(ra[jj]);
      raw_land(rb[jj]);
    }
  }
};
template <typename T, int MC, bool NT, bool TIGHT>
struct UpdScanPairTripCW : CwOneRow {
  static_assert(sizeof(T) == 8, "compact W: fp64");
  static constexpr int H = MC / 2;
  static constexpr int NL = 8 + 4 * H;
  RawOf<T, 1> rx, rl, ru, rg, rr, rd;
  RawOf<T, 2> ra[H], rb[H];
  RawOf<nb_t, 1> rnb;
  RawOf<iw_t, 1> riw;
  typedef unsigned long long u64x2 __attribute__((ext_vector_type(2)));
  typedef const __attribute__((address_space(1))) T *gptr;
  template <bool NTL, typename R>
  __device__ __forceinline__ void cols(const UpdScanCtx<T> &c, int64_t a0, int64_t a1, R (&qa)[H], R (&qb)[H]) {
    const bool hi = threadIdx.x & 32;
    int tb = hi ? 2 * H : 0;
    asm volatile("" : "+v"(tb));
    u64x2 p[H];
#pragma unroll
    for (int jj = 0; jj < H; ++jj) p[jj] = *reinterpret_cast<const u64x2 *>(c.ptab + tb + 2 * jj);
#pragma unroll
    for (int jj = 0; jj < H; ++jj) {
      const bool dead = TIGHT ? (jj == H - 1 && hi) : (hi && H + jj >= c.nold);
      raw_issue_half<NTL>(qa[jj], 0, (const T *)((gptr)p[jj].x + (dead ? 0 : a0)));
      raw_issue_half<NTL>(qa[jj], 1, (const T *)((gptr)p[jj].x + (dead ? 0 : a1)));
      raw_issue_half<NTL>(qb[jj], 0, (const T *)((gptr)p[jj].y + (dead ? 0 : a0)));
      raw_issue_half<NTL>(qb[jj], 1, (const T *)((gptr)p[jj].y + (dead ? 0 : a1)));
    }
  }
  __device__ __forceinline__ void issue_cw(const UpdScanCtx<T> &c, int64_t i, int64_t slot, bool lf, int64_t first) {
    constexpr int B = (int)sizeof(T);
    this->ri_ = i, this->ws_ = slot, this->lf_ = lf;
    raw_issue<B, NT>(rx, c.x + i);
    raw_issue<B, NT>(rl, (c.ub & 1) ? c.l : c.l + i);
    raw_issue<B, NT>(ru, (c.ub & 2) ? c.u : c.u + i);
    raw_issue<B, NT>(rg, c.g + i);
    raw_issue<B, NT>(rr, c.r + i);
    raw_issue<B, NT>(rd, c.d + i);
    raw_issue<1, false>(rnb, (c.ub & 4) ? c.nbd : c.nbd + i);
    raw_issue<1, false>(riw, c.iwhere + i);
    int64_t a0, a1;
    half_pair(lf ? slot : first, a0, a1);
    cols<false>(c, a0, a1, ra, rb);
  }
  __device__ __forceinline__ void land() {}
  __device__ __forceinline__ void reload_cols(const UpdScanCtx<T> &c, const bool (&miss)[1]) {
    int mi0, mi1;
    half_pair((int)miss[0], mi0, mi1);
    const bool m0 = mi0 != 0, m1 = mi1 != 0;
    const int64_t first = this->ri_ & ~(int64_t)127;
    int64_t a0, a1;
    half_pair((miss[0] || this->lf_) ? this->ws_ : first, a0, a1);
    RawOf<T, 2> ta[H], tb2[H];
    cols<false>(c, a0, a1, ta, tb2);
#pragma unroll
    for (int jj = 0; jj < H; ++jj) {
      if (m0) ra[jj].v.xy = ta[jj].v.xy, rb[jj].v.xy = tb2[jj].v.xy;
      if (m1) ra[jj].v.zw = ta[jj].v.zw, rb[jj].v.zw = tb2[jj].v.zw;
    }
  }
};
template <typename T, int MC, bool NT, bool PIPE, bool NEWROW, bool PAIR = false, bool CW = false, bool TIGHT = false>
__global__ __launch_bounds__(BLOCK) void update_scan_kernel(
    int64_t n, const T *__restrict__ x, const T *__restrict__ l, const T *__restrict__ u,
    const nb_t *__restrict__ nbd, const T *__restrict__ g, const T *__restrict__ r,
    const T *__restrict__ d, int dimpl, double stp, iw_t *iwhere, T *tbrk, T *ws, T *wy,
    const T *__restrict__ zero, int64_t ldw, int m, int head, int nold, int itail, int store_pair,
    int store_iw, double cand_hi, uint64_t *ckeys, uint32_t *cidx, uint32_t ccap, uint32_t *ccount,
    int ub, double *part, const uint64_t *__restrict__ lmask = nullptr) {
  static_assert(!CW || (sizeof(T) == 8 && MC <= 10 && !PIPE), "compact W: fp64, MC <= 10, one trip in flight");
  static constexpr UpdScanSlots S{MC, NEWROW};
  constexpr int NA = S.size(), NSUM = S.nsum();
  constexpr int V = CW ? 1 : ((sizeof(T) == 4 && MC == 10 && NEWROW) ? 4 : RowsPerAcc<T, MC, NA>::V);
  static_assert(!PAIR || (NEWROW && MC % 2 == 0), "PAIR: the new-row instantiation, even MC");
  constexpr int H = MC / 2;
  double acc[NA];
#pragma unroll
  for (int k = 0; k < NA; ++k) acc[k] = 0.0;
  acc[S.bkmin()] = LB_INF;
  double accp[PAIR ? 8 : 1][PAIR ? H : 1];
#pragma unroll
  for (int a = 0; a < (PAIR ? 8 : 1); ++a)
#pragma unroll
    for (int b = 0; b < (PAIR ? H : 1); ++b) accp[a][b] = 0.0;
  const bool hi = threadIdx.x & ((PAIR && CW) ? 32 : 1);
  const int64_t offn = (int64_t)(itail - 1) * ldw;
  __shared__ unsigned long long ptab[PAIR ? 2 * MC : 1];
  if constexpr (PAIR) {
    if (threadIdx.x < 2 * MC) {
      const int j = (int)threadIdx.x >> 1;
      const T *base = (threadIdx.x & 1) ? ws : wy;
      ptab[threadIdx.x] = (unsigned long long)(uintptr_t)(j < nold ? base + col_off(j, nold, head, m, ldw) : zero);
    }
    __syncthreads();
  }
  const UpdScanCtx<T> ctx{x, l, u, g, r, d, ws, wy, zero, nbd, iwhere, ldw, m, head, nold, ub, ptab};
  __shared__ T dict[16];
  dict_fill<T>(dict, l, u, ub);
  using TripV = std::conditional_t<PAIR, UpdScanPairTrip<T, MC, V, NT>, UpdScanTrip<T, MC, V, NT>>;
  using Trip1 = std::conditional_t<PAIR, UpdScanPairTrip<T, MC, 1, NT>, UpdScanTrip<T, MC, 1, NT>>;
  auto body = [&](auto &tr, int64_t i, auto wt) {
    constexpr int W = decltype(wt)::value;
    double xv[W], lv[W], uv[W], gv[W], rv[W], dv[W], tb[W], ng[W];
    int nb[W], iw[W];
    raw_get<W>(tr.rx, (const T *)nullptr, xv);
    raw_get<W>(tr.rl, (const T *)nullptr, lv);
    raw_get<W>(tr.ru, (const T *)nullptr, uv);
    raw_get<W>(tr.rg, (const T *)nullptr, gv);
    raw_get<W>(tr.rr, (const T *)nullptr, rv);
    raw_get<W>(tr.rd, (const T *)nullptr, dv);
    raw_geti<W>(tr.rnb, (const nb_t *)nullptr, nb);
    raw_geti<W>(tr.riw, (const iw_t *)nullptr, iw);
    dict_apply<T, W>(dict, ub, nb, lv, uv);
    bool iw_changed = false;
#pragma unroll
    for (int k = 0; k < W; ++k) {
      if (dimpl) dv[k] = (double)(T)(xv[k] - dv[k]);
      acc[S.gd()] = acc[S.gd()] + gv[k] * dv[k];
      acc[S.pgnorm()] = fmax(acc[S.pgnorm()], proj_g(xv[k], lv[k], uv[k], nb[k], gv[k]));
      rv[k] = gv[k] - rv[k];
      acc[S.yy()] = acc[S.yy()] + rv[k] * rv[k];
      if (stp != 1.0) dv[k] = stp * dv[k];
      const double neggi = -gv[k];
      double tl = 0.0, tu = 0.0;
      if (iw[k] != 3 && iw[k] != -1) {
        if (nb[k] <= 2) tl = xv[k] - lv[k];
        if (nb[k] >= 2) tu = uv[k] - xv[k];
        const bool xlower = nb[k] <= 2 && tl <= 0.0;
        const bool xupper = nb[k] >= 2 && tu <= 0.0;
        const int iw_old = iw[k];
        iw[k] = 0;
        if (xlower) {
          if (neggi <= 0.0) iw[k] = 1;
        } else if (xupper) {
          if (neggi >= 0.0) iw[k] = 2;
        } else {
          if (fabs(neggi) <= 0.0) iw[k] = -3;
        }
        iw_changed = iw_changed || iw[k] != iw_old;
        if (iw[k] != iw_old) acc[S.iw_changed()] += 1.0;
      }
      if (iw[k] != 0 && iw[k] != -1) {
        tb[k] = -1.0;
        ng[k] = 0.0;
      } else {
        ng[k] = neggi;
        acc[S.f1()] = acc[S.f1()] - neggi * neggi;
        if (nb[k] <= 2 && nb[k] != 0 && neggi < 0.0) {
          tb[k] = tl / (-neggi);
          acc[S.nbreak()] += 1.0;
          acc[S.bkmin()] = fmin(acc[S.bkmin()], tb[k]);
        } else if (nb[k] >= 2 && neggi > 0.0) {
          tb[k] = tu / neggi;
          acc[S.nbreak()] += 1.0;
          acc[S.bkmin()] = fmin(acc[S.bkmin()], tb[k]);
        } else {
          tb[k] = LB_INF;
          acc[S.nunb()] += 1.0;
          if (fabs(neggi) > 0.0) acc[S.nunbnz()] += 1.0;
        }
      }
      acc[S.yd()] += rv[k] * ng[k];
      acc[S.sd()] += dv[k] * ng[k];
    }
    double yf[W], sa[W];
    if constexpr (NEWROW) {
#pragma unroll
      for (int k = 0; k < W; ++k) {
        const double yst = (double)(T)rv[k], sst = (double)(T)dv[k];
        const bool fr = iw[k] <= 0;
        yf[k] = fr ? yst : 0.0;
        sa[k] = fr ? 0.0 : sst;
        acc[S.nr_scalar(0)] = __builtin_fma(yf[k], yst, acc[S.nr_scalar(0)]);
        acc[S.nr_scalar(1)] = __builtin_fma(sa[k], sst, acc[S.nr_scalar(1)]);
        acc[S.nr_scalar(2)] = __builtin_fma(sa[k], yst, acc[S.nr_scalar(2)]);
        acc[S.nr_scalar(3)] = __builtin_fma(fr ? sst : 0.0, yst, acc[S.nr_scalar(3)]);
      }
    }
    if constexpr (std::remove_reference_t<decltype(tr)>::CW) {
      bool miss[W], any = false;
#pragma unroll
      for (int k = 0; k < W; ++k) miss[k] = !tr.lf(k) && (dv[k] != 0.0 || iw[k] <= 0), any = any || miss[k];
      if (__ballot(any) != 0ull) tr.reload_cols(ctx, miss);
    }
    auto row_stores = [&]() {
      if (store_pair) {
        tr.template st_w<false>(ws + offn, i, dv);
        tr.template st_w<false>(wy + offn, i, rv);
      }
      if (store_iw && __ballot(iw_changed) != 0ull) tr.sti_rows(iwhere, i, iw);
      if (tbrk) tr.template st_rows<false>(tbrk, i, tb);
    };
    if constexpr (PAIR) row_stores();
    if constexpr (PAIR) {
      double qd[2 * W], qn[2 * W], qy[2 * W], qs[2 * W];
#pragma unroll
      for (int k = 0; k < W; ++k) {
        const T n_ = (T)ng[k], y_ = (T)yf[k], s_ = (T)sa[k];
        if constexpr (CW) {
          T n0, n1, y0, y1, s0, s1;
          half_pair(dv[k], qd[k], qd[W + k]);
          half_pair(n_, n0, n1);
          half_pair(y_, y0, y1);
          half_pair(s_, s0, s1);
          qn[k] = (double)n0, qn[W + k] = (double)n1;
          qy[k] = (double)y0, qy[W + k] = (double)y1;
          qs[k] = (double)s0, qs[W + k] = (double)s1;
        } else {
          const double od = pair_xchg(dv[k]);
          qd[k] = hi ? od : dv[k], qd[W + k] = hi ? dv[k] : od;
          const T on = pair_xchg(n_), oy = pair_xchg(y_), os = pair_xchg(s_);
          qn[k] = (double)(hi ? on : n_), qn[W + k] = (double)(hi ? n_ : on);
          qy[k] = (double)(hi ? oy : y_), qy[W + k] = (double)(hi ? y_ : oy);
          qs[k] = (double)(hi ? os : s_), qs[W + k] = (double)(hi ? s_ : os);
        }
      }
#pragma unroll
      for (int jj = 0; jj < H; ++jj) {
        double aj[2 * W], bj[2 * W];
        raw_get_col<2 * W, false>(tr.ra[jj], (const T *)nullptr, aj);
        raw_get_col<2 * W, false>(tr.rb[jj], (const T *)nullptr, bj);
#pragma unroll
        for (int k = 0; k < 2 * W; ++k) {
          accp[0][jj] = dot_term<T, CW>(accp[0][jj], qd[k], aj[k]);
          accp[1][jj] = dot_term<T, CW>(accp[1][jj], bj[k], qd[k]);
          accp[2][jj] = dot_term<T, CW>(accp[2][jj], aj[k], qn[k]);
          accp[3][jj] = dot_term<T, CW>(accp[3][jj], bj[k], qn[k]);
          accp[4][jj] = __builtin_fma(qy[k], aj[k], accp[4][jj]);
          accp[5][jj] = __builtin_fma(qs[k], bj[k], accp[5][jj]);
          accp[6][jj] = __builtin_fma(qs[k], aj[k], accp[6][jj]);
          accp[7][jj] = __builtin_fma(bj[k], qy[k], accp[7][jj]);
        }
      }
    } else
#pragma unroll
    for (int j = 0; j < MC; ++j) {
      double aj[W], bj[W];
      raw_get_col<W, false>(tr.ra[j], (const T *)nullptr, aj);
      raw_get_col<W, false>(tr.rb[j], (const T *)nullptr, bj);
#pragma unroll
      for (int k = 0; k < W; ++k) {
        acc[S.sy(j)] += dv[k] * aj[k];
        acc[S.ss(j)] += bj[k] * dv[k];
        acc[S.p_wy(j)] += aj[k] * ng[k];
        acc[S.p_ws(j)] += bj[k] * ng[k];
      }
      if constexpr (NEWROW) {
#pragma unroll
        for (int k = 0; k < W; ++k) {
          acc[S.nr_vec(0, j)] = __builtin_fma(yf[k], aj[k], acc[S.nr_vec(0, j)]);
          acc[S.nr_vec(1, j)] = __builtin_fma(sa[k], bj[k], acc[S.nr_vec(1, j)]);
          acc[S.nr_vec(2, j)] = __builtin_fma(sa[k], aj[k], acc[S.nr_vec(2, j)]);
          acc[S.nr_vec(3, j)] = __builtin_fma(bj[k], yf[k], acc[S.nr_vec(3, j)]);
        }
      }
    }
    if (!(NEWROW && MC > 10) && cand_hi >= 0.0) {
      unsigned bits = 0;
#pragma unroll
      for (int k = 0; k < W; ++k) {
        const double tr_ = (double)(T)tb[k];
        bits |= (tr_ >= 0.0 && tr_ <= cand_hi) ? (1u << k) : 0u;
      }
      if (__ballot(bits != 0) != 0ull && __builtin_nontemporal_load(ccount) <= ccap) {
        const int lane = threadIdx.x & 63;
#pragma unroll
        for (int k = 0; k < W; ++k) {
          const bool pred = (bits >> k) & 1u;
          const unsigned long long mask = __ballot(pred);
          if (mask == 0ull) continue;
          const int leader = __ffsll((long long)mask) - 1;
          uint32_t base = 0;
          if (lane == leader) base = atomicAdd(ccount, (uint32_t)__popcll(mask));
          base = __shfl(base, leader);
          if (pred) {
            const uint32_t pos = base + (uint32_t)__popcll(mask & ((1ull << lane) - 1ull));
            if (pos < ccap) {
              ckeys[pos] = key_of((double)(T)tb[k]);
              cidx[pos] = (uint32_t)tr.row(i, k);
            }
          }
        }
      }
    }
    if constexpr (!PAIR) row_stores();
  };
  if constexpr (CW && PAIR)
    for_halves_cw<UpdScanPairTripCW<T, MC, NT, TIGHT>>(n, ctx, lmask, body);
  else if constexpr (CW && NEWROW)
    for_halves_cw<UpdScanTripCW1<T, MC, NT>>(n, ctx, lmask, body);
  else if constexpr (CW)
    for_tiles_cw<UpdScanTripCW2<T, MC, NT>, UpdScanTripCW1<T, MC, NT>>(n, ctx, lmask, body);
  else
    for_rows_raw<TripV, Trip1, V, PIPE, 0>(n, ctx, body);
  if constexpr (PAIR) {
    constexpr int F0 = S.sy(0), F1 = S.ss(0), F2 = S.p_wy(0), F3 = S.p_ws(0);
    constexpr int F4 = S.nr_vec(0, 0), F5 = S.nr_vec(1, 0), F6 = S.nr_vec(2, 0), F7 = S.nr_vec(3, 0);
#pragma unroll
    for (int jj = 0; jj < H; ++jj) {
      const double z = 0.0;
      acc[F0 + jj] = hi ? z : accp[0][jj], acc[F0 + H + jj] = hi ? accp[0][jj] : z;
      acc[F1 + jj] = hi ? z : accp[1][jj], acc[F1 + H + jj] = hi ? accp[1][jj] : z;
      acc[F2 + jj] = hi ? z : accp[2][jj], acc[F2 + H + jj] = hi ? accp[2][jj] : z;
      acc[F3 + jj] = hi ? z : accp[3][jj], acc[F3 + H + jj] = hi ? accp[3][jj] : z;
      acc[F4 + jj] = hi ? z : accp[4][jj], acc[F4 + H + jj] = hi ? accp[4][jj] : z;
      acc[F5 + jj] = hi ? z : accp[5][jj], acc[F5 + H + jj] = hi ? accp[5][jj] : z;
      acc[F6 + jj] = hi ? z : accp[6][jj], acc[F6 + H + jj] = hi ? accp[6][jj] : z;
      acc[F7 + jj] = hi ? z : accp[7][jj], acc[F7 + H + jj] = hi ? accp[7][jj] : z;
    }
  }
  block_reduce_store<NA>(acc, NSUM, 1, 1, part, MAX_BLOCKS);
}
struct SplitPlan {
  int nparts, mo;
  int src[SPLIT_MAXPARTS], j0[SPLIT_MAXPARTS], cnt[SPLIT_MAXPARTS], mc[SPLIT_MAXPARTS];
};
__global__ __launch_bounds__(BLOCK) void update_split_merge_kernel(double *res, SplitPlan P, int dst) {
  const UpdScanSlots O{P.mo, true}, A{P.mc[0], true};
  double *out = res + dst;
  for (int j = threadIdx.x; j < O.mc; j += BLOCK) {
    int p = 0;
    while (p < P.nparts && j >= P.j0[p] + P.cnt[p]) ++p;
    const bool live = p < P.nparts;
    const UpdScanSlots I{live ? P.mc[p] : 0, true};
    const double *in = res + (live ? P.src[p] : 0);
    const int c = live ? j - P.j0[p] : 0;
    out[O.sy(j)] = live ? in[I.sy(c)] : 0.0;
    out[O.ss(j)] = live ? in[I.ss(c)] : 0.0;
    out[O.p_wy(j)] = live ? in[I.p_wy(c)] : 0.0;
    out[O.p_ws(j)] = live ? in[I.p_ws(c)] : 0.0;
    for (int k = 0; k < 4; ++k) out[O.nr_vec(k, j)] = live ? in[I.nr_vec(k, c)] : 0.0;
  }
  if (threadIdx.x == BLOCK - 1) {
    const double *a = res + P.src[0];
    out[O.yy()] = a[A.yy()], out[O.yd()] = a[A.yd()], out[O.sd()] = a[A.sd()];
    out[O.f1()] = a[A.f1()], out[O.nbreak()] = a[A.nbreak()], out[O.nunb()] = a[A.nunb()];
    out[O.nunbnz()] = a[A.nunbnz()], out[O.gd()] = a[A.gd()], out[O.iw_changed()] = a[A.iw_changed()];
    for (int k = 0; k < 4; ++k) out[O.nr_scalar(k)] = a[A.nr_scalar(k)];
    out[O.bkmin()] = a[A.bkmin()], out[O.pgnorm()] = a[A.pgnorm()];
  }
}

template <typename T>
void launch_update_scan(Queue &q, int64_t n, const T *x, const T *l, const T *u, const nb_t *nbd,
                        const T *g, const T *r, const T *d, int dimpl, double stp, iw_t *iwhere,
                        T *tbrk, WStore<T> w, int head, int col, int itail, int store_pair,
                        int store_iw, int newrow, double cand_hi, uint64_t *ckeys, uint32_t *cidx,
                        uint32_t ccap, uint32_t *ccount, int ub) {
  const int nold = col - 1;
  if (newrow && nold > q.tune.split_from) {
    const int nparts = split_parts(nold, q.tune.split_cols);
    if (nparts > SPLIT_MAXPARTS || q.part_sel != 0 || store_pair) {
      if (q.launch_err == hipSuccess) q.launch_err = hipErrorInvalidValue, q.launch_err_where = "update_scan: split pass";
      return;
    }
    SplitPlan P{};
    P.nparts = nparts, P.mo = maxc_stride(nold);
    const int dst = q.res_off, base = std::max(split_base(nold, dst), q.split_base_min);
    int j0 = 0;
    for (int k = 0; k < nparts; ++k) {
      const int cnt = (nold - j0 + (nparts - k) - 1) / (nparts - k);
      P.src[k] = base + k * SPLIT_SLOTS, P.j0[k] = j0, P.cnt[k] = cnt, P.mc[k] = maxc_for(cnt);
      q.res_off = P.src[k];
      launch_update_scan<T>(q, n, x, l, u, nbd, g, r, d, dimpl, stp, iwhere, k == 0 ? tbrk : (T *)nullptr, w,
                            (head - 1 + j0) % w.m + 1, cnt + 1, itail, 0, k == 0 ? store_iw : 0, 1, -1.0, ckeys,
                            cidx, ccap, ccount, ub);
      j0 += cnt;
    }
    q.res_off = dst;
    hipLaunchKernelGGL(update_split_merge_kernel, dim3(1), dim3(BLOCK), 0, q.stream, q.d_res, P, dst);
    LB_LAUNCHED(q);
    return;
  }
  if (cand_hi >= 0.0) (void)hipMemsetAsync(ccount, 0, sizeof(uint32_t), q.stream);
  int gr = 0;
  if (w.lmask) {
    bool done = false;
    if constexpr (sizeof(T) == 8) {
      if (nold <= 10) {
        const bool nrw = newrow != 0;
#define LB_UPDSCAN_CW(MCV, NTV, NRV)                                                                   \
  {                                                                                                    \
    gr = grid_for_w(q, n, VecOf<T>::V, (const void *)&update_scan_kernel<T, MCV, NTV, false, NRV, false, true>); \
    hipLaunchKernelGGL((update_scan_kernel<T, MCV, NTV, false, NRV, false, true>), dim3(gr), dim3(BLOCK), 0,     \
                       q.stream, n, x, l, u, nbd, g, r, d, dimpl, stp, iwhere, tbrk, w.ws, w.wy, w.zero, w.ld,   \
                       w.m, head, nold, itail, store_pair, store_iw, cand_hi, ckeys, cidx, ccap, ccount, ub,     \
                       q.part(), w.lmask);                                                                       \
  }
        int nblocks = -1;
        if (nold > 5 && nrw && q.tune.pair_cw && n >= CW_TILE) {
          const int64_t n_main = n / CW_TILE * CW_TILE, n_rest = n - n_main;
#define LB_PAIR_CW(NTV, TIGHTV)                                                                                   \
  {                                                                                                               \
    gr = grid_for_w(q, n_main, VecOf<T>::V,                                                                       \
                    (const void *)&update_scan_kernel<T, 10, NTV, false, true, true, true, TIGHTV>);              \
    hipLaunchKernelGGL((update_scan_kernel<T, 10, NTV, false, true, true, true, TIGHTV>), dim3(gr), dim3(BLOCK), 0, \
                       q.stream, n_main, x, l, u, nbd, g, r, d, dimpl, stp, iwhere, tbrk, w.ws, w.wy, w.zero,       \
                       w.ld, w.m, head, nold, itail, store_pair, store_iw, cand_hi, ckeys, cidx, ccap, ccount, ub,   \
                       q.part(), w.lmask);                                                                          \
  }
          if (nold == 9) {
            if (q.nt) LB_PAIR_CW(true, true) else LB_PAIR_CW(false, true)
          } else {
            if (q.nt) LB_PAIR_CW(true, false) else LB_PAIR_CW(false, false)
          }
#undef LB_PAIR_CW
          nblocks = gr;
          if (n_rest > 0) {
            LB_LAUNCHED(q);
            const int64_t o = n_main;
            hipLaunchKernelGGL((update_scan_kernel<T, 10, false, false, true, false, true>), dim3(1), dim3(BLOCK), 0,
                               q.stream, n_rest, x + o, (ub & 1) ? l : l + o, (ub & 2) ? u : u + o,
                               (ub & 4) ? nbd : nbd + o, g + o, r + o, d + o, dimpl, stp, iwhere + o,
                               tbrk ? tbrk + o : tbrk, w.ws + o, w.wy + o, w.zero, w.ld, w.m, head, nold, itail,
                               store_pair, store_iw, -1.0, ckeys, cidx, ccap, ccount, ub, q.part() + gr,
                               w.lmask + o / 64);
            nblocks = gr + 1;
          }
        } else if (nold <= 5) {
          if (q.nt) { if (nrw) LB_UPDSCAN_CW(5, true, true) else LB_UPDSCAN_CW(5, true, false) }
          else { if (nrw) LB_UPDSCAN_CW(5, false, true) else LB_UPDSCAN_CW(5, false, false) }
        } else {
          if (q.nt) { if (nrw) LB_UPDSCAN_CW(10, true, true) else LB_UPDSCAN_CW(10, true, false) }
          else { if (nrw) LB_UPDSCAN_CW(10, false, true) else LB_UPDSCAN_CW(10, false, false) }
        }
#undef LB_UPDSCAN_CW
        LB_LAUNCHED(q);
        launch_finalize(q, nblocks >= 0 ? nblocks : gr, UpdScanSlots{maxc_for(nold), nrw}.nsum(), 1, 1);
        done = true;
      }
    }
    if (!done && q.launch_err == hipSuccess)
      q.launch_err = hipErrorInvalidValue, q.launch_err_where = "update_scan: compact W needs fp64, col - 1 <= 10";
    return;
  }
#define LB_UPDSCAN(NEWROWV)                                                                          \
  DISPATCH_MAXC_NT(nold, q.nt, DISPATCH_PIPE(MC, {                                                   \
                     constexpr bool NRV = NEWROWV && MC <= 20;                                       \
                     constexpr bool PPV = MC <= 10 ? (PIPEV || NRV) : (PIPEV && !NRV && MC <= 20);   \
                     gr = grid_for_w(q, n, VecOf<T>::V,                                              \
                                     (const void *)&update_scan_kernel<T, MC, NTV, PPV, NRV>);       \
                     hipLaunchKernelGGL((update_scan_kernel<T, MC, NTV, PPV, NRV>), dim3(gr),        \
                                        dim3(BLOCK), 0, q.stream, n, x, l, u, nbd, g, r, d, dimpl,   \
                                        stp,                                                         \
                                        iwhere, tbrk, w.ws, w.wy, w.zero, w.ld, w.m, head, nold,     \
                                        itail, store_pair, store_iw, cand_hi, ckeys, cidx, ccap,     \
                                        ccount, ub, q.part());                                       \
                   }))
  const int mc = maxc_for(nold);
  const int pair_mode = q.tune.pair;
  int nblocks = 0;
  if (newrow && mc == 20 && pair_mode > 0) {
    constexpr int MC = 20;
    gr = grid_for_w(q, n, VecOf<T>::V, (const void *)&update_scan_kernel<T, MC, true, true, true, true>);
    nblocks = gr;
    constexpr int VP = RowsPerAcc<T, MC, UpdScanSlots{MC, true}.size()>::V;
    const int64_t n_main = n / (2 * VP) * (2 * VP), n_rest = n - n_main;
#define LB_PAIR(NTV, PIPEV)                                                                          \
  hipLaunchKernelGGL((update_scan_kernel<T, MC, NTV, PIPEV, true, true>), dim3(gr), dim3(BLOCK), 0,  \
                     q.stream, n_main, x, l, u, nbd, g, r, d, dimpl, stp, iwhere, tbrk, w.ws, w.wy,  \
                     w.zero, w.ld, w.m, head, nold, itail, store_pair, store_iw, -1.0, ckeys, cidx,   \
                     ccap, ccount, ub, q.part())
    if (n_main > 0) {
      if (q.nt) {
        if (pair_mode >= 2) LB_PAIR(true, true); else LB_PAIR(true, false);
      } else {
        if (pair_mode >= 2) LB_PAIR(false, true); else LB_PAIR(false, false);
      }
    }
#undef LB_PAIR
    if (n_rest > 0 || n_main == 0) {
      const int64_t o = n_main;
      hipLaunchKernelGGL((update_scan_kernel<T, MC, false, false, true>), dim3(1), dim3(BLOCK), 0, q.stream,
                         n_rest, x + o, (ub & 1) ? l : l + o, (ub & 2) ? u : u + o, (ub & 4) ? nbd : nbd + o,
                         g + o, r + o, d + o, dimpl, stp, iwhere + o,
                         tbrk ? tbrk + o : tbrk, w.ws + o, w.wy + o, w.zero, w.ld, w.m, head, nold, itail,
                         store_pair, store_iw, -1.0, ckeys, cidx, ccap, ccount, ub,
                         q.part() + (n_main > 0 ? gr : 0));
      nblocks = n_main > 0 ? gr + 1 : 1;
      LB_LAUNCHED(q);
    }
  } else if (newrow) {
    LB_UPDSCAN(true);
    nblocks = gr;
  } else {
    LB_UPDSCAN(false);
    nblocks = gr;
  }
#undef LB_UPDSCAN
  LB_LAUNCHED(q);
  launch_finalize(q, nblocks, UpdScanSlots{mc, newrow != 0}.nsum(), 1, 1);
}

#define INSTANTIATE(T) \
  template void launch_update_pairs<T>(Queue &, int64_t, const T *, const T *, const T *, double, WStore<T>, int, int, int); \
  template void launch_update_scan<T>(Queue &, int64_t, const T *, const T *, const T *, const nb_t *, const T *, const T *, const T *, int, double, iw_t *, T *, WStore<T>, int, int, int, int, int, int, double, uint64_t *, uint32_t *, uint32_t, uint32_t *, int);
INSTANTIATE(double)
INSTANTIATE(float)
#undef INSTANTIATE

}
```

### lbfgsb_amd/csrc/kernels.hpp

```cpp
#pragma once
#include <hip/hip_runtime.h>
#include <stdint.h>
#include "qn_plan.hpp"
#include "res_layout.hpp"

namespace lbk {

constexpr int BLOCK = 256;
constexpr int MAX_BLOCKS = 2048;
constexpr int GRAM_BLOCKS = 1024;

struct Tune {
  int wgrid = 0;
  int pipe = -1;
  int pair = 2;
  int split_from = 20;
  int split_cols = 16;
  int gram_rows = 0;
  int pair_cw = 1;
};

struct FinJob {
  const double *part;
  int pstride, nblocks, off, nsum, nmin, nmax;
};

struct Queue {
  hipStream_t stream;
  double *d_part;
  static constexpr int ALT_SLOTS = 8;
  double *d_part_alt[2] = {nullptr, nullptr};
  int part_sel = 0;
  bool hold_fin = false;
  FinJob held[2];
  int nheld = 0;
  double *part() const { return part_sel == 0 ? d_part : d_part_alt[part_sel - 1]; }
  bool fin_publish = false;
  double *hd_pub = nullptr;
  unsigned long long *hd_fin_flag = nullptr;
  unsigned int *d_fin_count = nullptr;
  unsigned long long fin_seq = 0;
  int64_t launches_at_fin = -1;
  double *d_res;
  double *d_gpart;
  int64_t launches;
  int res_off = 0;
  int split_base_min = 0;
  bool nt = false;
  Tune tune{};
  const char *launch_err_where = nullptr;
  hipError_t launch_err = hipSuccess;
  void launched(const char *where) {
    launches++;
    const hipError_t e = hipGetLastError();
    if (e != hipSuccess && launch_err == hipSuccess) launch_err = e, launch_err_where = where;
  }
};
#define LB_LAUNCHED(q) (q).launched(__func__)

template <typename T>
struct WStore {
  T *ws;
  T *wy;
  int64_t ld;
  int m;
  const T *zero;
  const uint64_t *lmask = nullptr;
};
constexpr int CW_TILE = 128;

using iw_t = int8_t;
using nb_t = int8_t;

struct Coef {
  double a[2 * MAXM];
};

struct Pend {
  int on;
  double stp;
  int impl;
};

int grid_for(int64_t n, int vec);
int grid_for_w(const Queue &q, int64_t n, int vec, const void *kernel = nullptr);

template <typename T>
void launch_active(Queue &q, int64_t n, T *x, const T *l, const T *u, const int32_t *nbd,
                   iw_t *iwhere, int8_t *wasfree);
template <typename T>
void launch_errclb(Queue &q, int64_t n, int64_t row0, const T *l, const T *u,
                   const int32_t *nbd);

template <typename T>
void launch_projgr(Queue &q, int64_t n, const T *x, const T *l, const T *u,
                   const int32_t *nbd, const T *g);
template <typename T>
void launch_vec_sub(Queue &q, int64_t n, const T *a, const T *b, T *out);
template <typename T>
void launch_vec_scale(Queue &q, int64_t n, double alpha, T *v);
template <typename T>
void launch_dot(Queue &q, int64_t n, const T *a, const T *b);

template <typename T>
void launch_wtv(Queue &q, int64_t n, WStore<T> w, int head, int col, const T *v);
template <typename T>
void launch_wtv_nofinalize(Queue &q, int64_t n, WStore<T> w, int head, int col, const T *v);

template <typename T>
void launch_cauchy_scan(Queue &q, int64_t n, const T *x, const T *l, const T *u,
                        const int32_t *nbd, const T *g, iw_t *iwhere, T *tbrk,
                        WStore<T> w, int head, int col);
template <typename T>
void launch_cauchy_window(Queue &q, int64_t n, int64_t row0, const T *tbrk, double lo_t,
                          int64_t lo_i, double hi_t, uint64_t *keys, uint32_t *idx,
                          uint32_t cap, uint32_t *d_count);
template <typename T>
void launch_cauchy_allkeys(Queue &q, int64_t n, int64_t row0, const T *tbrk, double lo_t,
                           int64_t lo_i, uint64_t *keys, uint32_t *idx);
size_t sort_pairs_temp_bytes(size_t count);
void launch_sort_pairs(Queue &q, void *d_temp, size_t temp_bytes, const uint64_t *keys_in,
                       uint64_t *keys_out, const uint32_t *idx_in, uint32_t *idx_out,
                       size_t count);
uint32_t *launch_sort_u32(Queue &q, void *d_temp, size_t temp_bytes, uint32_t *keys, uint32_t *scratch,
                          uint32_t count);
void launch_merge_chunks(Queue &q, int nranks, uint32_t chunk, int recl, size_t stride, const double *all,
                         uint64_t *keys0, uint64_t *keys1, uint32_t *vals0, uint32_t *vals1, void *d_temp,
                         size_t temp_bytes, double *out);
void launch_sort_by_idx(Queue &q, void *d_temp, size_t temp_bytes, const uint32_t *idx_in,
                        uint32_t *idx_out, const uint64_t *keys_in, uint64_t *keys_out,
                        size_t count);
template <typename T>
void launch_cauchy_gather(Queue &q, const uint32_t *idx, const uint64_t *keys, uint32_t cnt,
                          int64_t row0, const T *x, const T *l, const T *u, const T *g, WStore<T> w,
                          int head, int col, const T *pr, const T *pd, Pend pe, double *rec);
template <typename T>
void launch_cauchy_gather_dyn(Queue &q, const uint32_t *idx, const uint64_t *keys,
                              const uint32_t *d_count, uint32_t cap, int64_t row0, const T *x,
                              const T *l, const T *u, const T *g, WStore<T> w, int head, int col,
                              const T *pr, const T *pd, Pend pe, double *msg);
template <typename T>
void launch_cauchy_window_fly(Queue &q, int64_t n, int64_t row0, const T *x, const T *l, const T *u,
                              const nb_t *nbd, const T *g, const iw_t *iwhere, double lo_t,
                              int64_t lo_i, double hi_t, uint64_t *keys, uint32_t *idx, uint32_t cap,
                              uint32_t *d_count, int ub = 0);
template <typename T>
void launch_iwhere_update(Queue &q, int64_t n, const T *x, const T *l, const T *u,
                          const int32_t *nbd, const T *g, iw_t *iwhere);
template <typename T>
void launch_xcp_fill(Queue &q, int64_t n, const T *x, const T *g, const T *l, const T *u,
                     const iw_t *iwhere, double tsum, T *dst);
size_t scan_temp_bytes(size_t count);
void launch_scan(Queue &q, void *d_temp, size_t temp_bytes, const double *in, double *out,
                 size_t count, int exclusive);
template <typename T>
void launch_pgcp_gather(Queue &q, const uint32_t *idx, const uint64_t *keys, int64_t nb, int64_t nbp,
                        const T *x, const T *l, const T *u, const T *g, WStore<T> w, int head, int col,
                        double theta, const T *pr, const T *pd, Pend pe, double *tt, double *dd,
                        double *a0, double *wb, double *uu, double *gi, int64_t row0);
void launch_pgcp_mergekeys(Queue &q, int nranks, int64_t nbp, int narr, const double *counts,
                           const double *G, uint64_t *keys, uint32_t *vals);
void launch_pgcp_permute(Queue &q, int64_t NB, int64_t NBp, int64_t nbp, int narr, const uint32_t *vals,
                         const double *G, double *out, const int *map);
size_t f2scan_temp_bytes(size_t count);
void launch_pgcp_f2(Queue &q, void *d_temp, size_t temp_bytes, int64_t nb, double f2_0, double cl,
                    const double *df2, double *maps, double *F2);
template <typename T>
void launch_gcp_rest_mass(Queue &q, int64_t n, const T *g, const T *tbrk, double tstar);
void launch_pgcp_last(Queue &q, int64_t nb, int64_t nbp, int col2, const double *uu, double *uu_last);
void launch_pgcp_dtp(Queue &q, int64_t nb, int64_t nbp, int col2, const double *tt, const double *pp,
                     double *qq);
void launch_pgcp_terms(Queue &q, int64_t nb, int64_t nbp, int col2, double theta, const double *mm,
                       const double *p0, const double *tt, const double *dd, const double *a0,
                       const double *wb, const double *pp, const double *sq, double *df2, double *a1);
void launch_pgcp_f1(Queue &q, int64_t nb, double f2_0, const double *tt, const double *sf2,
                    const double *a1, double *df1);
void launch_pgcp_find(Queue &q, int64_t nb, double f1_0, double f2_0, const double *tt,
                      const double *sf1, const double *sf2);
void launch_pgcp_pick(Queue &q, int64_t ks, int64_t nb, int64_t nbp, int col2, double f1_0, double f2_0,
                      const double *tt, const double *sf1, const double *sf2, const double *pp,
                      const double *uu_last, const double *sq, const uint32_t *idx, const double *gi,
                      double *out);
template <typename T>
void launch_tbrk_fill(Queue &q, int64_t n, const T *x, const T *l, const T *u, const int32_t *nbd,
                      const T *g, const iw_t *iwhere, T *tbrk);
template <typename T>
void launch_cauchy_finish(Queue &q, int64_t n, int64_t row0, const T *x, const T *l, const T *u,
                          const T *g, const T *tbrk, iw_t *iwhere, T *xcp, double tsum,
                          double last_t, int64_t last_i, int count = 0);

void launch_cauchy_fix(Queue &q, const int64_t *list, int count, int64_t row0, int64_t n,
                       iw_t *iwhere);

void launch_freev_count(Queue &q, int64_t n, const iw_t *iwhere, int8_t *wasfree,
                        uint32_t *chg, uint32_t chg_cap, uint32_t *cnt2, int parity, int write = 1);
void launch_freev_apply(Queue &q, const uint32_t *chg, const uint32_t *cnt_ptr, uint32_t cap, int8_t *wasfree);
void launch_freev_lists(Queue &q, int64_t n, const iw_t *iwhere, const int8_t *prevfree,
                        int do_enterleave, int32_t *index, int32_t *indx2, int32_t *scan_tmp);

template <typename T>
void launch_formk_gram(Queue &q, int64_t n, WStore<T> w, int head, int col,
                       const iw_t *iwhere);

template <typename T>
void launch_cmprlb_wtv(Queue &q, int64_t n, const T *x, const T *g, double tsum,
                       const iw_t *iwhere, WStore<T> w, int head, int col, double theta,
                       const Coef &a, int newrow, const T *pr, const T *pd, Pend pe);
template <typename T>
void launch_formk_patch(Queue &q, const uint32_t *chg, uint32_t cnt, WStore<T> w, int head, int upcl);
template <typename T>
void launch_formk_patch_dev(Queue &q, const uint32_t *chg, const uint32_t *cnt_ptr, uint32_t cap, WStore<T> w,
                            int head, int upcl);
void launch_sort_u32_small_dev(Queue &q, uint32_t *keys, const uint32_t *cnt_ptr);
int small_sort_cap();

template <typename T>
void launch_subsm_update(Queue &q, int64_t n, double tsum, T *zout, const T *pr, T *rout, const T *l,
                         const T *u, const nb_t *nbd, const iw_t *iwhere, const T *xx, const T *gg,
                         WStore<T> w, int head, int col, double theta, const Coef &cf,
                         const Coef &wv, T *dvec, T *tvec, T *xout, int do_stpmx, Pend pe,
                         const T *pd, int ub = 0);
template <typename T>
void launch_subsm_dir(Queue &q, int64_t n, const T *xcp, const iw_t *iwhere, const T *xx,
                      const T *gg, WStore<T> w, int head, int col, double theta, const Coef &cf,
                      const Coef &wv, T *ndir);
template <typename T>
void launch_subsm_alpha(Queue &q, int64_t n, const T *xp, const T *r, const T *l, const T *u,
                        const int32_t *nbd, const iw_t *iwhere);
template <typename T>
void launch_subsm_argalpha(Queue &q, int64_t n, int64_t row0, const T *xp, const T *r,
                           const T *l, const T *u, const int32_t *nbd, const iw_t *iwhere,
                           double alpha);
template <typename T>
void launch_subsm_backtrack(Queue &q, int64_t n, int64_t row0, T *z, const T *xp, T *r,
                            const T *l, const T *u, const iw_t *iwhere, double alpha,
                            int64_t ibd);

template <typename T>
void launch_lnsrlb_begin(Queue &q, int64_t n, const T *z, const T *x, const T *g, const T *l,
                         const T *u, const int32_t *nbd, T *d, T *t, T *r, int do_stpmx);
template <typename T>
void launch_lnsrlb_step(Queue &q, int64_t n, T *x, const T *z, const T *d, const T *t,
                        double stp);
template <typename T>
void launch_lnsrlb_eval(Queue &q, int64_t n, const T *x, const T *l, const T *u,
                        const int32_t *nbd, const T *g, const T *d);

template <typename T>
void launch_update_pairs(Queue &q, int64_t n, const T *g, const T *r, const T *d, double stp,
                         WStore<T> w, int head, int col, int itail);

template <typename T>
void launch_update_scan(Queue &q, int64_t n, const T *x, const T *l, const T *u,
                        const nb_t *nbd, const T *g, const T *r, const T *d, int dimpl,
                        double stp, iw_t *iwhere, T *tbrk, WStore<T> w, int head, int col, int itail,
                        int store_pair, int store_iw, int newrow = 0, double cand_hi = -1.0,
                        uint64_t *ckeys = nullptr, uint32_t *cidx = nullptr, uint32_t ccap = 0,
                        uint32_t *ccount = nullptr, int ub = 0);
inline bool update_scan_hands_over(const Queue &q, int64_t n, int col, int newrow, bool layout) {
  const int nold = col - 1;
  if (newrow && (maxc_for(nold) > 10 || nold > q.tune.split_from)) return false;
  if (layout && newrow && nold > 5 && nold <= 10 && q.tune.pair_cw && n >= CW_TILE && n % CW_TILE != 0) return false;
  return true;
}
void launch_nbd_pack(Queue &q, int64_t n, const int32_t *nbd, nb_t *out);
constexpr int UB_DICT = 8;
struct BoundTables {
  double l[8], u[8];
  int nl, nu, nb0;
};
template <typename T>
void launch_dict_probe(Queue &q, int64_t n, const T *l, const T *u, const BoundTables &tb);
template <typename T>
void launch_nbd_pack_dict(Queue &q, int64_t n, const int32_t *nbd, const T *l, const T *u, const BoundTables &tb,
                          nb_t *out);
template <typename T>
void launch_bounds_verify(Queue &q, int64_t n, const T *l, const T *u, const int32_t *nbd, const nb_t *code,
                          int ub, const BoundTables &tb);
template <typename T>
void launch_bounds_follow(Queue &q, int64_t n, const T *l, const T *u, const int32_t *nbd, const T *l_snap,
                          const T *u_snap, const nb_t *code, int ub, const BoundTables &tb, int force);
template <typename T>
void launch_bounds_same(Queue &q, int64_t n, const T *l0, const T *u0, const int32_t *nb0, const T *l1,
                        const T *u1, const int32_t *nb1);
template <typename T>
void launch_dz_materialise(Queue &q, int64_t n, const T *x, const T *t, T *d, T *z, T *xnew = nullptr,
                           double stp = 1.0);
template <typename T>
void launch_pair_commit(Queue &q, int64_t n, const T *g, const T *r, const T *d, Pend pe,
                        WStore<T> w, int head, int col);

template <typename T>
void launch_w_relayout(Queue &q, int64_t n, const iw_t *iwhere, uint64_t *lmask, WStore<T> w, int head, int col);
void launch_lmask_ones(Queue &q, int64_t n, uint64_t *lmask);

template <typename T>
void launch_tile_axpy(Queue &q, int64_t n, WStore<T> w, int head, int tc, const Coef &cf, double div,
                      const iw_t *iwhere, int masked, T *out);
template <typename T>
struct WideTail {
  const T *x, *g, *l, *u;
  const int32_t *nbd;
  double tsum, theta;
  int plain, do_stpmx;
  T *zout, *dvec, *tvec, *rout, *xout;
};
template <typename T>
void launch_tile_axpy_fused(Queue &q, int64_t n, WStore<T> w, int head, int tc, const Coef &cf, const iw_t *iwhere,
                            T *out, int first, int last, const WideTail<T> &wt);
constexpr int WIDE_MAXC = 96;
struct CoefWide {
  double a[2 * WIDE_MAXC];
};
template <typename T>
void launch_wide_r_pass(Queue &q, int64_t n, WStore<T> w, int head, int col, const CoefWide &cf, const iw_t *iwhere,
                        const nb_t *nbd8, int ub, const WideTail<T> &wt, Pend pe, const T *pr, const T *pd);
template <typename T>
void launch_masked_copy(Queue &q, int64_t n, const T *src, const iw_t *iwhere, int want_free, T *out);
template <typename T>
void launch_rows_gather(Queue &q, const uint32_t *chg, uint32_t cnt, WStore<T> w, int head, int upcl, double *out);
template <typename T>
void launch_cauchy_dvec(Queue &q, int64_t n, const T *g, const T *tbrk, T *out);
template <typename T>
void launch_cmprlb_init(Queue &q, int64_t n, const T *x, const T *g, const T *z, const iw_t *iwhere,
                        double theta, int plain, T *out);
template <typename T>
void launch_subsm_project(Queue &q, int64_t n, T *z, T *dir, const T *x, const T *g, const T *l, const T *u,
                          const int32_t *nbd, const iw_t *iwhere, double rtheta);

template <typename T>
void launch_obj_quadratic(Queue &q, int64_t n, int64_t row0, const T *x, T *g);
template <typename T>
void launch_obj_rosenbrock(Queue &q, int64_t n, int64_t row0, int64_t nglob, const T *x, T *g,
                           double xl, double xr);
template <typename T>
void launch_halo_pack(Queue &q, int64_t n, const T *x, double *out);
void launch_scalar_partial(Queue &q, const double *d_val);

void launch_finalize(Queue &q, int nblocks, int nsum, int nmin, int nmax);
void finalize_flush(Queue &q);
void launch_publish(Queue &q, const double *src, double *dst_host, int count, unsigned long long seq,
                    unsigned long long *flag_host);

template <typename T>
struct QnVecs {
  const T *p[QN_KMAX];
};
template <typename T>
struct QnOuts {
  T *p[QN_KMAX];
};
// ... 42 lines not shown
```

### lbfgsb_amd/csrc/solver_base.hpp

```cpp
#pragma once
#include <dlfcn.h>
#include <hip/hip_runtime.h>
#include <rccl/rccl.h>

#include <algorithm>
#include <atomic>
#include <functional>
#include <chrono>
#include <condition_variable>
#include <memory>
#include <thread>
#include <cmath>
#include <cstdio>
#include <cstdlib>
#include <cstring>
#include <limits>
#include <mutex>
#include <string>
#include <unordered_map>
#include <vector>

#include "../../include/lbfgsb_hip.h"
#include "../../include/lbfgsb_hip_debug.h"
#include "gpu_owner.hpp"
#include "host_dense.hpp"
#include "kernels.hpp"
#include "report.hpp"

namespace lbs {

inline thread_local std::string g_err;

inline int fail(int code, const std::string &msg) {
  g_err = msg;
  return code;
}

#define HIPCHK(expr)                                                                    \
  do {                                                                                  \
    hipError_t e_ = (expr);                                                             \
    if (e_ != hipSuccess)                                                               \
      return fail(LBFGSB_E_NOGPU, std::string(#expr) + ": " + hipGetErrorString(e_));   \
  } while (0)
#define CHK(expr)          \
  do {                     \
    int rc_ = (expr);      \
    if (rc_ != 0) return rc_; \
  } while (0)

inline double now_s() {
  using namespace std::chrono;
  return duration<double>(steady_clock::now().time_since_epoch()).count();
}

struct Rccl {
  void *h = nullptr;
  ncclResult_t (*GetUniqueId)(ncclUniqueId *) = nullptr;
  ncclResult_t (*CommInitRank)(ncclComm_t *, int, ncclUniqueId, int) = nullptr;
  ncclResult_t (*CommDestroy)(ncclComm_t) = nullptr;
  ncclResult_t (*AllGather)(const void *, void *, size_t, ncclDataType_t, ncclComm_t,
                            hipStream_t) = nullptr;
  ncclResult_t (*CommCount)(const ncclComm_t, int *) = nullptr;
  ncclResult_t (*CommUserRank)(const ncclComm_t, int *) = nullptr;
  bool ok = false;
  std::mutex mtx;
  bool load() {
    std::lock_guard<std::mutex> lock(mtx);
    if (ok) return true;
    if (h) {
      dlclose(h);
      h = nullptr;
    }
    const char *names[] = {std::getenv("LBFGSB_RCCL_LIBRARY"), "librccl.so.1", "librccl.so",
                           "/opt/rocm/lib/librccl.so.1"};
    for (const char *nm : names) {
      if (!nm || !*nm) continue;
      h = dlopen(nm, RTLD_NOW | RTLD_GLOBAL);
      if (h) break;
    }
    if (!h) return false;
#define SYM(f, name) f = reinterpret_cast<decltype(f)>(dlsym(h, name))
    SYM(GetUniqueId, "ncclGetUniqueId");
    SYM(CommInitRank, "ncclCommInitRank");
    SYM(CommDestroy, "ncclCommDestroy");
    SYM(AllGather, "ncclAllGather");
    SYM(CommCount, "ncclCommCount");
    SYM(CommUserRank, "ncclCommUserRank");
#undef SYM
    ok = GetUniqueId && CommInitRank && CommDestroy && AllGather;
    if (!ok) {
      dlclose(h);
      h = nullptr;
    }
    return ok;
  }
};
inline Rccl g_rccl;

struct Rec {
  double t;
  int64_t gidx;
};

}
using namespace lbs;

struct lbfgsb_hip_ctx {
  virtual ~lbfgsb_hip_ctx() { host_unregister_all(); }
  virtual int setulb_dev(void *x, const void *l, const void *u, const int32_t *nbd, double *f,
                         void *g, double factr, double pgtol, char *task, int iprint, char *csave,
                         int32_t *lsave, int32_t *isave, double *dsave) = 0;
  virtual int setulb_dev_pp(void *x0, void *x1, const void *l, const void *u, const int32_t *nbd,
                            double *f, void *g0, void *g1, double factr, double pgtol, char *task,
                            int iprint, char *csave, int32_t *lsave, int32_t *isave, double *dsave,
                            int32_t *cur) = 0;
  virtual int export_state(void *wa, int32_t *iwa) = 0;
  virtual int import_state(const void *wa, const int32_t *iwa, const int32_t *isave) = 0;
  virtual int k_projgr(const void *x, const void *l, const void *u, const int32_t *nbd,
                       const void *g, double *out) = 0;
  virtual int k_wtv(const void *v, int col, int head, double *out, bool launch_only) = 0;
  virtual int k_set_w(const void *hws, const void *hwy) = 0;
  virtual int k_set_iwhere(const int32_t *h_iw) = 0;
  virtual int k_formk_gram(int col, int head, double *out) = 0;
  virtual int k_launch(int which, const void *x, const void *g, int col, int head) = 0;
  virtual int k_objective(int kind, const void *x, void *g, double *f) = 0;
  virtual int r_active(void *x, const void *l, const void *u, const int32_t *nbd, int32_t *out3) = 0;
  virtual int r_vec_sub(const void *a, const void *b, void *out) = 0;
  virtual int r_vec_scale(double alpha, void *v) = 0;
  virtual int r_dot(const void *a, const void *b, double *out) = 0;
  virtual int r_errclb(const void *l, const void *u, const int32_t *nbd, double factr, char *task,
                       int32_t *info, int64_t *k) = 0;
  virtual int r_cauchy(const void *x, const void *l, const void *u, const int32_t *nbd, const void *g,
                       double theta, int col, int head, double sbgnrm, void *xcp_out, int32_t *nseg,
                       int32_t *info) = 0;
  virtual int r_freev(int iter, int cnstnd, int updatd, int64_t *nfree, int64_t *nenter, int64_t *ileave,
                      int32_t *wrk) = 0;
  virtual int r_formk(int col, int head, double theta, int32_t *info) = 0;
  virtual int r_cmprlb(const void *x, const void *g, double theta, int col, int head, int cnstnd, void *r_out,
                       int32_t *info) = 0;
  virtual int r_subsm(const void *x, const void *l, const void *u, const int32_t *nbd, const void *g,
                      const void *r_in, double theta, int col, int head, void *xhat_out, int32_t *iword,
                      int32_t *info) = 0;
  virtual int r_lnsrlb(void *x, const void *l, const void *u, const int32_t *nbd, const void *g, double f,
                       double *sc, int32_t *ic, char *task, char *csave, int32_t *isave2, double *dsave13) = 0;
  virtual int r_matupd(const void *g, double stp, double dr, double dtd, int32_t *ip, double *theta_out) = 0;
  virtual int sync() = 0;
  virtual int qn_apply(int mode, int64_t k, const void *v, int64_t ldv, void *out, int64_t ldo) = 0;
  virtual int qn_diag(int mode, void *out) = 0;
  virtual int qn_logdet(int mode, double *h_logdet) = 0;
  virtual int qn_draw(int mode, int64_t k, uint64_t seed, int64_t first, const void *mean, double scale, void *out,
                      int64_t ldo) = 0;
  virtual int qn_quad(int mode, int64_t k, const void *v, int64_t ldv, const void *center, double *h_q) = 0;
  virtual int qn_logpdf(int mode, int64_t k, const void *x, int64_t ldx, const void *mean, double scale,
                        double *h_logp) = 0;
  virtual int qn_draw_logpdf(int mode, int64_t k, uint64_t seed, int64_t first, const void *mean, double scale,
                             void *out, int64_t ldo, double *h_logp) = 0;
  virtual int qn_vgram(int mode, int64_t k, const void *v, int64_t ldv, const void *center, double *h_g,
                       int64_t ldg) = 0;
  virtual int qn_eig(int mode, int32_t cap, int32_t *h_r, double *h_bulk, double *h_lambda) = 0;
  virtual int qn_eigvec(int mode, int64_t k, const int32_t *h_which, void *out, int64_t ldo) = 0;
  virtual int kkt(const void *x, const void *l, const void *u, const int32_t *nbd, const void *g, double tol,
                  void *pg_out, void *mult_out, int8_t *status_out, int64_t *h_cnt, double *h_val) = 0;
  virtual int kkt_list(const int8_t *status, int code_mask, int64_t *idx_out, int64_t cap, int64_t *h_count) = 0;
  virtual int attach_rccl(ncclComm_t comm, int rank, int nranks) = 0;
  virtual ncclComm_t rccl_comm() const = 0;
  virtual int attach_host(lbfgsb_allreduce_fn ar, lbfgsb_allgather_fn ag, void *user, int rank,
                          int nranks) = 0;
  virtual void path_counts(int64_t &closed_form, int64_t &three_pass) const = 0;
  virtual int set_option(const char *name, double value) = 0;
  virtual const void *prev_iterate() const = 0;

  GpuOwner own;
  void *hx = nullptr, *hg = nullptr, *hl = nullptr, *hu = nullptr;
  int32_t *hnbd = nullptr;
  bool restored_xg = false;
  int64_t n_ls_setup = 0;
  struct HostReg {
    void *p = nullptr;
    size_t bytes = 0;
  } host_reg[3];
  void host_register(int k, void *p, size_t bytes) {
    if (!p || bytes < ((size_t)1 << 20)) return;
    if (hipHostRegister(p, bytes, hipHostRegisterDefault) == hipSuccess)
      host_reg[k].p = p, host_reg[k].bytes = bytes;
    else
      (void)hipGetLastError();
  }
  void host_unregister_if_not(int k, const void *p) {
    HostReg &r = host_reg[k];
    if (r.p && r.p != p) {
      if (hipHostUnregister(r.p) != hipSuccess) (void)hipGetLastError();
      r.p = nullptr, r.bytes = 0;
    }
  }
  void host_unregister_all() {
    for (HostReg &r : host_reg) {
      if (r.p && hipHostUnregister(r.p) != hipSuccess) (void)hipGetLastError();
      r.p = nullptr, r.bytes = 0;
    }
  }
  std::string itfile_name = "iterate.dat";
  int64_t n = 0, nglob = 0, row0 = 0;
  int m = 0, flags = 0, device = 0;
  int rank = 0, nranks = 1;
  int64_t nsync = 0, nfullsort = 0;
  int64_t ntiesplit = 0;
  int64_t nrefresh = 0;
  int64_t ngcp_clamped = 0;
  int64_t nspecwin = 0;
  double t_wait = 0.0;
  double t_mid = 0.0, t_mid0 = 0.0;
  int64_t n_mid = 0;
  double t_seg[5] = {0, 0, 0, 0, 0}, t_mark = 0.0;
  void seg(int k) {
    if (t_mid0 <= 0.0) return;
    const double t = now_s();
    t_seg[k] += t - t_mark, t_mark = t;
  }
  int64_t ncoll = 0, coll_bytes = 0;
  virtual int uniform_mask() const = 0;
  virtual int bounds_changed() = 0;
  virtual void bounds_stats(int64_t &checks, int64_t &changes, int64_t &rebuilds) const = 0;
  virtual int bounds_same(const void *l0, const void *u0, const int32_t *nb0, const void *l1, const void *u1,
                          const int32_t *nb1, double *ndiff) = 0;
  virtual int64_t freev_skipped() const = 0;
  virtual int collective_time(int reps, double *median_us, double *min_us) = 0;
  virtual int f_device(const double *d_f) = 0;
  hipEvent_t return_ev = nullptr;
  virtual void compact_stats(int64_t &packs, int64_t &unpacks, int &packed, int &eligible) const = 0;
  virtual int64_t skip_scans_reused() const = 0;
  virtual void defer_counts(int64_t &deferred, int64_t &reissued) const = 0;
  bool f_pending = false;
  double f_scale = 1.0;
  static constexpr int CLK_RING = 4;
  bool clock_on = false;
  hipEvent_t clk_ev[3][CLK_RING][2] = {};
  bool clk_pending[3][CLK_RING] = {};
  int clk_cur[3] = {0, 0, 0};
  double clk_ms[3] = {0.0, 0.0, 0.0};
  int64_t clk_n[3] = {0, 0, 0};
  int64_t clk_dropped = 0;
  hipStream_t clk_stream = nullptr;
  hipEvent_t order_ev = nullptr;
  void clk_begin(int k) {
    if (!clock_on) return;
    clk_collect();
    int s = clk_cur[k];
    for (int tries = 0; tries < CLK_RING && clk_pending[k][s]; ++tries) s = (s + 1) % CLK_RING;
    if (clk_pending[k][s]) clk_dropped++, clk_pending[k][s] = false;
    clk_cur[k] = s;
    if (!clk_ev[k][s][0]) {
      (void)own.event(&clk_ev[k][s][0]);
      (void)own.event(&clk_ev[k][s][1]);
    }
    (void)hipEventRecord(clk_ev[k][s][0], clk_stream);
  }
  void clk_end(int k) {
    if (!clock_on) return;
    const int s = clk_cur[k];
    (void)hipEventRecord(clk_ev[k][s][1], clk_stream);
    clk_pending[k][s] = true;
    clk_cur[k] = (s + 1) % CLK_RING;
  }
  void clk_collect() {
    for (int k = 0; k < 3; ++k)
      for (int s = 0; s < CLK_RING; ++s) {
        if (!clk_pending[k][s]) continue;
        if (hipEventQuery(clk_ev[k][s][1]) != hipSuccess) continue;
        float ms = 0.f;
        if (hipEventElapsedTime(&ms, clk_ev[k][s][0], clk_ev[k][s][1]) == hipSuccess) {
          clk_ms[k] += ms;
          clk_n[k]++;
        }
        clk_pending[k][s] = false;
      }
  }
  lbk::Queue q{};
};


lbfgsb_hip_ctx *lbfgsb_make_solver(int64_t n_local, int64_t n_global, int64_t row0, int m, int flags,
                                   int device, void *stream, int *rc);
```

### lbfgsb_amd/solver.py

```python
from __future__ import annotations

import ctypes as C
from typing import Optional

import numpy as np

from . import capi
from .capi import LbfgsbError, check, load_library

TASK_LEN = 60


def wa_length(n: int, m: int) -> int:
    return 2 * m * n + 5 * n + 11 * m * m + 8 * m


def _p(a):
    if a is None:
        return None
    if isinstance(a, np.ndarray):
        return a.ctypes.data_as(C.c_void_p)
    return C.c_void_p(int(a.data_ptr()))


# ... 297 lines not shown
        import torch
        dt = torch.float32 if self.real == np.float32 else torch.float64
        if out is None:
            out = torch.empty((int(k), self.n), dtype=dt, device=torch.device("cuda", self.device))
        out = self._qn_vec(out, "out")
        if (out.dim() == 1 and k != 1) or (out.dim() == 2 and out.shape[0] != k):
            raise ValueError("out must have shape (k, n)")
        if mean is not None:
            mean = self._qn_vec(mean, "mean")
            if mean.dim() != 1:
                raise ValueError("mean must have shape (n,)")
        ldo = self.n if out.dim() == 1 else out.stride(0)
        self.wait_stream()
        if return_logpdf:
            logp = np.zeros(int(k), np.float64)
            check(self.lib.lbfgsb_hip_qn_draw_logpdf(self.h, capi.QN_H if inverse else capi.QN_B, int(k),
                                                     int(seed) & 0xFFFFFFFFFFFFFFFF, int(first),
                                                     None if mean is None else mean.data_ptr(), float(scale),
                                                     out.data_ptr(), ldo,
                                                     logp.ctypes.data_as(C.POINTER(C.c_double))))
            self._qn_done()
            return out, logp
        check(self.lib.lbfgsb_hip_qn_draw(self.h, capi.QN_H if inverse else capi.QN_B, int(k),
                                          int(seed) & 0xFFFFFFFFFFFFFFFF, int(first),
                                          None if mean is None else mean.data_ptr(), float(scale), out.data_ptr(),
                                          ldo))
        self._qn_done()
        return out

    def _qn_center(self, c, what):
        if c is None:
            return None
        c = self._qn_vec(c, what)
        if c.dim() != 1:
            raise ValueError("%s must have shape (n,)" % what)
        return c

    def qn_quad(self, v, center=None, inverse: bool = False):
        v = self._qn_vec(v, "v")
        center = self._qn_center(center, "center")
        k = 1 if v.dim() == 1 else v.shape[0]
        ldv = self.n if v.dim() == 1 else v.stride(0)
        q = np.zeros(k, np.float64)
        self.wait_stream()
        check(self.lib.lbfgsb_hip_qn_quad(self.h, capi.QN_H if inverse else capi.QN_B, k, v.data_ptr(), ldv,
                                          None if center is None else center.data_ptr(),
                                          q.ctypes.data_as(C.POINTER(C.c_double))))
        return float(q[0]) if v.dim() == 1 else q

    def qn_gram(self, v, center=None, inverse: bool = False):
        v = self._qn_vec(v, "v")
        center = self._qn_center(center, "center")
        k = 1 if v.dim() == 1 else v.shape[0]
        ldv = self.n if v.dim() == 1 else v.stride(0)
        g = np.zeros((k, k), np.float64)
        self.wait_stream()
        check(self.lib.lbfgsb_hip_qn_gram(self.h, capi.QN_H if inverse else capi.QN_B, k, v.data_ptr(), ldv,
                                          None if center is None else center.data_ptr(),
                                          g.ctypes.data_as(C.POINTER(C.c_double)), k))
        return g

    def qn_eig(self, inverse: bool = False):
        r, bulk = C.c_int32(0), C.c_double(0.0)
        mode = capi.QN_H if inverse else capi.QN_B
        self.wait_stream()
        check(self.lib.lbfgsb_hip_qn_eig(self.h, mode, 0, C.byref(r), C.byref(bulk), None))
        lam = np.zeros(r.value, np.float64)
        if r.value:
            check(self.lib.lbfgsb_hip_qn_eig(self.h, mode, r.value, C.byref(r), C.byref(bulk),
                                             lam.ctypes.data_as(C.POINTER(C.c_double))))
        return bulk.value, lam

    def qn_eigvec(self, which=None, out=None, inverse: bool = False):
        import torch
        dt = torch.float32 if self.real == np.float32 else torch.float64
        if which is None:
            k = out.shape[0] if out is not None and out.dim() == 2 else (1 if out is not None else
                                                                         len(self.qn_eig(inverse)[1]))
            idx = None
        else:
            idx = np.ascontiguousarray(which, np.int32).reshape(-1)
            k = int(idx.size)
        if out is None:
            out = torch.empty((k, self.n), dtype=dt, device=torch.device("cuda", self.device))
            if k == 0:
                return out
        out = self._qn_vec(out, "out")
        if (out.dim() == 1 and k != 1) or (out.dim() == 2 and out.shape[0] != k):
            raise ValueError("out must have shape (k, n)")
        ldo = self.n if out.dim() == 1 else out.stride(0)
        self.wait_stream()
        check(self.lib.lbfgsb_hip_qn_eigvec(self.h, capi.QN_H if inverse else capi.QN_B, k,
                                            None if idx is None else idx.ctypes.data_as(C.POINTER(C.c_int32)),
                                            out.data_ptr(), ldo))
        self._qn_done()
        return out

    def qn_logpdf(self, x, mean=None, scale: float = 1.0, inverse: bool = True):
        x = self._qn_vec(x, "x")
        mean = self._qn_center(mean, "mean")
        k = 1 if x.dim() == 1 else x.shape[0]
        ldx = self.n if x.dim() == 1 else x.stride(0)
        lp = np.zeros(k, np.float64)
        self.wait_stream()
        check(self.lib.lbfgsb_hip_qn_logpdf(self.h, capi.QN_H if inverse else capi.QN_B, k, x.data_ptr(), ldx,
                                            None if mean is None else mean.data_ptr(), float(scale),
                                            lp.ctypes.data_as(C.POINTER(C.c_double))))
        return float(lp[0]) if x.dim() == 1 else lp

    def qn_operator(self, inverse: bool = True) -> "QnOperator":
        return QnOperator(self, inverse)

    def kkt(self, x, l, u, nbd, g, tol: float = 0.0, pg=True, mult=True, status=True) -> "KktReport":
        import torch
        want = torch.float32 if self.real == np.float32 else torch.float64
        for name, t in (("x", x), ("l", l), ("u", u), ("g", g)):
            if not (isinstance(t, torch.Tensor) and t.is_cuda and t.dtype == want and t.dim() == 1
                    and t.numel() >= self.n and t.is_contiguous()):
                raise TypeError("%s must be a contiguous CUDA tensor of dtype %s with n = %d rows"
                                % (name, want, self.n))
        if not (isinstance(nbd, torch.Tensor) and nbd.is_cuda and nbd.dtype == torch.int32 and nbd.dim() == 1
                and nbd.numel() >= self.n and nbd.is_contiguous()):
            raise TypeError("nbd must be a contiguous int32 CUDA tensor with n = %d rows" % self.n)

        def out_of(o, dt, name):
            if o is None or o is False:
                return None
            if o is True:
                return torch.empty(self.n, dtype=dt, device=x.device)
            if not (isinstance(o, torch.Tensor) and o.is_cuda and o.dtype == dt and o.dim() == 1
                    and o.numel() >= self.n and o.is_contiguous()):
                raise TypeError("%s must be a contiguous CUDA tensor of dtype %s with n = %d rows"
                                % (name, dt, self.n))
            return o
        pg, mult, status = out_of(pg, want, "pg"), out_of(mult, want, "mult"), out_of(status, torch.int8, "status")
        cnt = np.zeros(len(capi.KKT_CNT), np.int64)
        val = np.zeros(len(capi.KKT_VAL), np.float64)
        self.wait_stream()
        check(self.lib.lbfgsb_hip_kkt(self.h, _p(x), _p(l), _p(u), _p(nbd), _p(g), float(tol), _p(pg), _p(mult),
                                      _p(status), _p(cnt), _p(val)))
        return KktReport(cnt, val, float(tol), pg, mult, status)

    def kkt_indices(self, status, codes):
        import torch
        if not (isinstance(status, torch.Tensor) and status.is_cuda and status.dtype == torch.int8
                and status.dim() == 1 and status.numel() >= self.n and status.is_contiguous()):
            raise TypeError("status must be a contiguous int8 CUDA tensor with n = %d rows" % self.n)
        mask = 0
        for c in ([codes] if isinstance(codes, (int, np.integer)) else codes):
            if not -1 <= int(c) <= 3:
                raise ValueError("status codes are -1 .. 3")
            mask |= 1 << (int(c) + 1)
        count = np.zeros(1, np.int64)
        self.wait_stream()
        check(self.lib.lbfgsb_hip_kkt_list(self.h, _p(status), mask, None, 0, _p(count)))
        idx = torch.empty(int(count[0]), dtype=torch.int64, device=status.device)
        if count[0] > 0:
            check(self.lib.lbfgsb_hip_kkt_list(self.h, _p(status), mask, _p(idx), int(count[0]), _p(count)))
        return idx

    def projgr(self, x, l, u, nbd, g) -> float:
        out = np.zeros(1)
        check(self.lib.lbfgsb_hip_projgr(self.h, _p(x), _p(l), _p(u), _p(nbd), _p(g), _p(out)))
        return float(out[0])

    def r_vec_sub(self, a, b, out):
        check(self.lib.lbfgsb_hip_vec_sub(self.h, _p(a), _p(b), _p(out)))

    def r_vec_scale(self, alpha, v):
        check(self.lib.lbfgsb_hip_vec_scale(self.h, float(alpha), _p(v)))

    def r_dot(self, a, b):
        out = np.zeros(1, np.float64)
        check(self.lib.lbfgsb_hip_dot(self.h, _p(a), _p(b), _p(out)))
        return float(out[0])

    def r_active(self, x, l, u, nbd):
        out = np.zeros(3, np.int32)
        check(self.lib.lbfgsb_hip_active(self.h, _p(x), _p(l), _p(u), _p(nbd), _p(out)))
        return bool(out[0]), bool(out[1]), bool(out[2])

    def r_errclb(self, l, u, nbd, factr, task=b"START"):
        t = np.frombuffer(task.ljust(60), dtype="S1").copy()
        info, k = np.zeros(1, np.int32), np.zeros(1, np.int64)
        check(self.lib.lbfgsb_hip_errclb(self.h, _p(l), _p(u), _p(nbd), float(factr), _p(t), _p(info), _p(k)))
        return t.tobytes().decode().rstrip(), int(info[0]), int(k[0])

    def r_cauchy(self, x, l, u, nbd, g, theta, col, head, sbgnrm, xcp_out=None):
        nseg, info = np.zeros(1, np.int32), np.zeros(1, np.int32)
        check(self.lib.lbfgsb_hip_cauchy(self.h, _p(x), _p(l), _p(u), _p(nbd), _p(g), float(theta), int(col),
                                         int(head), float(sbgnrm), _p(xcp_out) if xcp_out is not None else None,
                                         _p(nseg), _p(info)))
        return int(nseg[0]), int(info[0])

    def r_freev(self, iter_, cnstnd, updatd):
        o = np.zeros(3, np.int64)
        wrk = np.zeros(1, np.int32)
        check(self.lib.lbfgsb_hip_freev(self.h, int(iter_), int(bool(cnstnd)), int(bool(updatd)), _p(o[0:1]),
                                        _p(o[1:2]), _p(o[2:3]), _p(wrk)))
        return int(o[0]), int(o[1]), int(o[2]), bool(wrk[0])

    def r_formk(self, col, head, theta):
        info = np.zeros(1, np.int32)
        check(self.lib.lbfgsb_hip_formk(self.h, int(col), int(head), float(theta), _p(info)))
        return int(info[0])

    def r_cmprlb(self, x, g, theta, col, head, cnstnd, r_out):
        info = np.zeros(1, np.int32)
        check(self.lib.lbfgsb_hip_cmprlb(self.h, _p(x), _p(g), float(theta), int(col), int(head),
                                         int(bool(cnstnd)), _p(r_out), _p(info)))
        return int(info[0])

    def r_subsm(self, x, l, u, nbd, g, r_in, theta, col, head, xhat_out=None):
        iword, info = np.zeros(1, np.int32), np.zeros(1, np.int32)
        check(self.lib.lbfgsb_hip_subsm(self.h, _p(x), _p(l), _p(u), _p(nbd), _p(g), _p(r_in), float(theta),
                                        int(col), int(head), _p(xhat_out) if xhat_out is not None else None,
                                        _p(iword), _p(info)))
        return int(iword[0]), int(info[0])

    def r_lnsrlb(self, x, l, u, nbd, g, f, sc, ic, task, csave, isave2, dsave13):
        check(self.lib.lbfgsb_hip_lnsrlb(self.h, _p(x), _p(l), _p(u), _p(nbd), _p(g), float(f), _p(sc), _p(ic),
                                         _p(task), _p(csave), _p(isave2), _p(dsave13)))

    def r_matupd(self, g, stp, dr, dtd, ip):
        th = np.zeros(1)
        check(self.lib.lbfgsb_hip_matupd(self.h, _p(g), float(stp), float(dr), float(dtd), _p(ip), _p(th)))
        return float(th[0])

    def set_w(self, ws: np.ndarray, wy: np.ndarray):
        ws = np.ascontiguousarray(ws, self.real)
        wy = np.ascontiguousarray(wy, self.real)
        assert ws.shape == (self.m, self.n) and wy.shape == (self.m, self.n)
        check(self.lib.lbfgsb_hip_set_w(self.h, _p(ws), _p(wy)))

    def set_iwhere(self, iwhere: np.ndarray):
        iw = np.ascontiguousarray(iwhere, np.int32)
        assert iw.shape == (self.n,)
        check(self.lib.lbfgsb_hip_set_iwhere(self.h, _p(iw)))

    def formk_gram(self, col: int, head: int = 1) -> np.ndarray:
        out = np.zeros(2 * col * col + col)
        check(self.lib.lbfgsb_hip_formk_gram(self.h, col, head, _p(out)))
        return out

    def wtv(self, v, col: int, head: int = 1) -> np.ndarray:
        out = np.zeros(2 * col)
        check(self.lib.lbfgsb_hip_wtv(self.h, _p(v), col, head, _p(out)))
        return out

    def wtv_launch(self, v, col: int, head: int = 1):
        check(self.lib.lbfgsb_hip_wtv_launch_only(self.h, _p(v), col, head))

    def wtv_time(self, v, col: int, head: int = 1, reps: int = 20) -> float:
        out = np.zeros(1)
        check(self.lib.lbfgsb_hip_wtv_time(self.h, _p(v), col, head, reps, _p(out)))
        return float(out[0])

    def kernel_time(self, which: int, x, g, col: int, head: int = 1, reps: int = 20) -> float:
        out = np.zeros(1)
        check(self.lib.lbfgsb_hip_kernel_time(self.h, which, _p(x), _p(g), col, head, reps, _p(out)))
        return float(out[0])

    def sync(self):
        check(self.lib.lbfgsb_hip_sync(self.h))

    def objective(self, kind: int, x, g, deferred: bool = False):
        if deferred:
            check(self.lib.lbfgsb_hip_objective(self.h, kind, self._addr(x), self._addr(g), None))
            return None
        out = np.zeros(1)
        check(self.lib.lbfgsb_hip_objective(self.h, kind, _p(x), _p(g), _p(out)))
        return float(out[0])

    def pass_clock(self, enable: int):
        ms = (C.c_double * 3)()
        cnt = (C.c_int64 * 3)()
        check(self.lib.lbfgsb_hip_pass_clock(self.h, int(enable), ms, cnt))
        names = ("cmprlb_wtv", "update_scan", "subsm_update")
        return {nm: (ms[k], cnt[k]) for k, nm in enumerate(names)}

    def path_counts(self):
        a, b, c = C.c_int64(), C.c_int64(), C.c_int64()
        check(self.lib.lbfgsb_hip_path_counts(self.h, C.byref(a), C.byref(b), C.byref(c)))
        return int(a.value), int(b.value), int(c.value)

    def uniform_bounds(self) -> int:
        c = C.c_int32()
        check(self.lib.lbfgsb_hip_uniform_bounds(self.h, C.byref(c)))
        return int(c.value)

    def bounds_changed(self):
        check(self.lib.lbfgsb_hip_bounds_changed(self.h))

    def bounds_stats(self):
        a, b, c = C.c_int64(), C.c_int64(), C.c_int64()
        check(self.lib.lbfgsb_hip_bounds_stats(self.h, C.byref(a), C.byref(b), C.byref(c)))
        return int(a.value), int(b.value), int(c.value)

    def comm_info(self):
        a, b, k = C.c_int32(), C.c_int32(), C.c_int32()
        check(self.lib.lbfgsb_hip_comm_info(self.h, C.byref(a), C.byref(b), C.byref(k)))
        return int(a.value), int(b.value), int(k.value)

    def compact_stats(self):
        a, b = C.c_int64(0), C.c_int64(0)
        c, d = C.c_int32(0), C.c_int32(0)
        check(self.lib.lbfgsb_hip_compact_stats(self.h, C.byref(a), C.byref(b), C.byref(c), C.byref(d)))
        return a.value, b.value, c.value, d.value

    def collective_time(self, reps: int = 1000):
        a, b = C.c_double(0.0), C.c_double(0.0)
        check(self.lib.lbfgsb_hip_collective_time(self.h, int(reps), C.byref(a), C.byref(b)))
        return a.value, b.value

    def host_gap(self):
        a, b = C.c_double(), C.c_int64()
        check(self.lib.lbfgsb_hip_host_gap(self.h, C.byref(a), C.byref(b)))
        return float(a.value), int(b.value)

    def host_segments(self):
        a = (C.c_double * 5)()
        check(self.lib.lbfgsb_hip_host_segments(self.h, a))
        return [float(v) for v in a]

    def defer_stats(self):
        a, b = C.c_int64(), C.c_int64()
        check(self.lib.lbfgsb_hip_defer_stats(self.h, C.byref(a), C.byref(b)))
        return int(a.value), int(b.value)

    def tie_splits(self) -> int:
        c = C.c_int64()
        check(self.lib.lbfgsb_hip_tie_splits(self.h, C.byref(c)))
        return int(c.value)

    def stats(self):
        a, b, c, w = C.c_int64(), C.c_int64(), C.c_int64(), C.c_double()
        check(self.lib.lbfgsb_hip_stats(self.h, C.byref(a), C.byref(b), C.byref(c), C.byref(w)))
        nc, nb = C.c_int64(), C.c_int64()
        check(self.lib.lbfgsb_hip_comm_stats(self.h, C.byref(nc), C.byref(nb)))
        fs = C.c_int64()
        check(self.lib.lbfgsb_hip_freev_skipped(self.h, C.byref(fs)))
        sr = C.c_int64()
        check(self.lib.lbfgsb_hip_skip_stats(self.h, C.byref(sr)))
        rf = C.c_int64()
        check(self.lib.lbfgsb_hip_refresh_count(self.h, C.byref(rf)))
        return dict(launches=a.value, syncs=b.value, cauchy_fullsorts=c.value, wait_seconds=w.value,
                    collectives=nc.value, collective_bytes=nb.value, freev_skipped=fs.value,
                    skip_scans_reused=sr.value, refreshes=rf.value)


class KktReport:

    def __init__(self, counts, values, tol, pg, mult, status):
        self.counts, self.values, self.tol = counts, values, tol
        self.pg, self.mult, self.status = pg, mult, status
        for k, name in enumerate(capi.KKT_CNT):
            setattr(self, name, int(counts[k]))
        for k, name in enumerate(capi.KKT_VAL):
            setattr(self, name, float(values[k]))

    def __repr__(self):
        return "KktReport(%s)" % ", ".join(
            ["%s=%d" % (k, getattr(self, k)) for k in capi.KKT_CNT]
            + ["%s=%r" % (k, getattr(self, k)) for k in capi.KKT_VAL])


class QnOperator:

    def __init__(self, solver: DeviceSolver, inverse: bool = True, root: bool = False):
        self.solver, self.inverse, self.root = solver, bool(inverse), bool(root)
        self.shape = (solver.n, solver.n)
        self.dtype = np.dtype(solver.real)

    def matvec(self, v):
        return self.solver.qn_apply(v, inverse=self.inverse, sqrt=self.root)

    def matmat(self, vs):
        if vs.dim() != 2 or vs.shape[0] != self.shape[1]:
            raise ValueError("matmat takes an (n, k) tensor")
        return self.solver.qn_apply(vs.t().contiguous(), inverse=self.inverse, sqrt=self.root).t()

    def diagonal(self):
        if self.root:
            raise ValueError("qn_diag takes B or H, not a square root")
        return self.solver.qn_diag(inverse=self.inverse)

    def sqrt(self) -> "QnOperator":
        if self.root:
            raise ValueError("this operator is a square root already")
        return QnOperator(self.solver, self.inverse, root=True)

    def logdet(self) -> float:
        v = self.solver.qn_logdet(inverse=self.inverse)
        return 0.5 * v if self.root else v

    def sample(self, k: int, seed: int, first: int = 0, mean=None, scale: float = 1.0, log_prob: bool = False):
        if self.root:
            raise ValueError("sample() draws with covariance A: call it on the operator, not on its root")
        return self.solver.qn_draw(k, seed, first=first, mean=mean, scale=scale, inverse=self.inverse,
                                   return_logpdf=log_prob)

    def quad(self, v, center=None):
        if self.root:
            raise ValueError("quad() takes B or H, not a square root")
        return self.solver.qn_quad(v, center=center, inverse=self.inverse)

    def gram(self, v, center=None):
        if self.root:
            raise ValueError("gram() takes B or H, not a square root")
        return self.solver.qn_gram(v, center=center, inverse=self.inverse)

    def _spectrum(self, what):
        if self.root:
            raise ValueError("%s takes B or H, not a square root" % what)
        return self.solver.qn_eig(inverse=self.inverse)

    def eigvalsh(self):
        return self._spectrum("eigvalsh()")

    def eigh(self):
        bulk, values = self._spectrum("eigh()")
        return bulk, values, self.solver.qn_eigvec(inverse=self.inverse)

    def cond(self) -> float:
        bulk, values = self._spectrum("cond()")
        ev = list(values) + ([bulk] if self.solver.n_global > len(values) else [])
        return float(max(ev) / min(ev))

    def log_prob(self, x, mean=None, scale: float = 1.0):
        if self.root:
            raise ValueError("log_prob() takes the covariance A: call it on the operator, not on its root")
        return self.solver.qn_logpdf(x, mean=mean, scale=scale, inverse=self.inverse)

    def __matmul__(self, v):
        return self.matvec(v) if v.dim() == 1 else self.matmat(v)
```

Measured before the change: 180.7 iters/sec.

## Load compact W tiles as dense 16-byte runs and redistribute through LDS

```diff
diff --git a/include/lbfgsb_hip_debug.h b/include/lbfgsb_hip_debug.h
--- a/include/lbfgsb_hip_debug.h
+++ b/include/lbfgsb_hip_debug.h
@@ -29,6 +29,7 @@
 int lbfgsb_hip_host_gap(lbfgsb_hip_ctx *ctx, double *seconds, int64_t *count);
 int lbfgsb_hip_compact_stats(lbfgsb_hip_ctx *ctx, int64_t *packs, int64_t *unpacks, int32_t *packed,
                              int32_t *eligible);
+int lbfgsb_hip_dense_launches(lbfgsb_hip_ctx *ctx, int64_t *storing, int64_t *update);
 int lbfgsb_hip_collective_time(lbfgsb_hip_ctx *ctx, int reps, double *median_us, double *min_us);
 int lbfgsb_hip_host_segments(lbfgsb_hip_ctx *ctx, double *seconds5);
 
diff --git a/lbfgsb_amd/capi.py b/lbfgsb_amd/capi.py
--- a/lbfgsb_amd/capi.py
+++ b/lbfgsb_amd/capi.py
@@ -42,6 +42,7 @@
     "lbfgsb_hip_host_gap": (C.c_int, [_vp, _vp, _vp]),
     "lbfgsb_hip_collective_time": (C.c_int, [_vp, C.c_int, _vp, _vp]),
     "lbfgsb_hip_compact_stats": (C.c_int, [_vp, _vp, _vp, _vp, _vp]),
+    "lbfgsb_hip_dense_launches": (C.c_int, [_vp, _vp, _vp]),
     "lbfgsb_hip_host_segments": (C.c_int, [_vp, _vp]),
     "lbfgsb_hip_comm_info": (C.c_int, [_vp, _vp, _vp, _vp]),
     "lbfgsb_hip_path_counts": (C.c_int, [_vp, _vp, _vp, _vp]),
diff --git a/lbfgsb_amd/csrc/capi.hip b/lbfgsb_amd/csrc/capi.hip
--- a/lbfgsb_amd/csrc/capi.hip
+++ b/lbfgsb_amd/csrc/capi.hip
@@ -520,6 +520,15 @@
   if (unpacks) *unpacks = b;
   if (packed) *packed = c;
   if (eligible) *eligible = d;
+  return 0;
+}
+
+int lbfgsb_hip_dense_launches(lbfgsb_hip_ctx *ctx, int64_t *storing, int64_t *update) {
+  if (!ctx) return fail(LBFGSB_E_ARG, "ctx == NULL");
+  int64_t a = 0, b = 0;
+  ctx->dense_launches(a, b);
+  if (storing) *storing = a;
+  if (update) *update = b;
   return 0;
 }
 
diff --git a/lbfgsb_amd/csrc/device_util.hpp b/lbfgsb_amd/csrc/device_util.hpp
--- a/lbfgsb_amd/csrc/device_util.hpp
+++ b/lbfgsb_amd/csrc/device_util.hpp
@@ -413,6 +413,10 @@
   sl[0] = lf[0] ? b0 : tf + (lane - b0);
   sl[1] = lf[1] ? b1 : tf + (64 + lane - b1);
 }
+__device__ __forceinline__ void wave_lds_order() {
+  __builtin_amdgcn_fence(__ATOMIC_RELEASE, "wavefront");
+  __builtin_amdgcn_wave_barrier();
+}
 __device__ __forceinline__ int64_t wave_uniform(int64_t v) {
   return (int64_t)(((uint64_t)(uint32_t)__builtin_amdgcn_readfirstlane((int)(v >> 32)) << 32) |
                    (uint32_t)__builtin_amdgcn_readfirstlane((int)v));
@@ -433,7 +437,7 @@
       Trip2 A;
       A.issue_cw(c, CwTile{tr << 7, m0, m1});
       raw_wait<0>();
-      A.land();
+      A.land_cw(c);
       f(A, tr << 7, WTag<2>{});
       if (!more) break;
       tr = nx, m0 = m0n, m1 = m1n;
@@ -463,7 +467,7 @@
   const int64_t nh = n >> 6;
   const int64_t stride = (int64_t)gridDim.x * (blockDim.x >> 6);
   const int64_t t0 = wave_uniform((int64_t)blockIdx.x * (blockDim.x >> 6) + (threadIdx.x >> 6));
-  auto issue = [&](Trip1 &A, int64_t h, uint64_t m0, uint64_t m1, int64_t row_limit) {
+  auto issue = [&](Trip1 &A, int64_t h, uint64_t m0, uint64_t m1, int64_t row_limit, bool full) {
     const bool hi = (h & 1) != 0;
     const int c0 = __popcll(m0), tf = c0 + __popcll(m1);
     const uint64_t mw = hi ? m1 : m0;
@@ -474,6 +478,12 @@
     const int64_t tb = (h >> 1) << 7;
     int64_t i = (h << 6) + lane;
     if (i >= row_limit) i = row_limit - 1;
+    if constexpr (Trip1::DENSE) {
+      if (full) {
+        A.issue_cw_run(c, i, tb + (lf ? b : tf + (r - b)), lf, tb, hi ? c0 : 0, hi ? tf : c0);
+        return;
+      }
+    }
     A.issue_cw(c, i, tb + (lf ? b : tf + (r - b)), lf, tb);
   };
   if (t0 < nh) {
@@ -484,9 +494,9 @@
       const int64_t nx = h + stride, nxc = cl(nx);
       const uint64_t m0n = lmask[(nxc >> 1) * 2], m1n = lmask[(nxc >> 1) * 2 + 1];
       Trip1 A;
-      issue(A, h, m0, m1, n);
+      issue(A, h, m0, m1, n, true);
       raw_wait<0>();
-      A.land();
+      A.land_cw(c);
       f(A, (h << 6) + lane, WTag<1>{});
       if (nx >= nh) break;
       h = nx, m0 = m0n, m1 = m1n;
@@ -495,9 +505,9 @@
   if ((n & 63) != 0 && t0 == nh % stride) {
     const uint64_t m0 = lmask[(nh >> 1) * 2], m1 = lmask[(nh >> 1) * 2 + 1];
     Trip1 A;
-    issue(A, nh, m0, m1, n);
+    issue(A, nh, m0, m1, n, false);
     raw_wait<0>();
-    A.land();
+    A.land_cw(c);
     if ((nh << 6) + lane < n) f(A, (nh << 6) + lane, WTag<1>{});
   }
 }
diff --git a/lbfgsb_amd/csrc/k_subsm.hip b/lbfgsb_amd/csrc/k_subsm.hip
--- a/lbfgsb_amd/csrc/k_subsm.hip
+++ b/lbfgsb_amd/csrc/k_subsm.hip
@@ -25,6 +25,7 @@
   int m, head, col;
   Pend pe;
   int ub;
+  i32x4_t *scr = nullptr;
 };
 template <typename T, int MC, int W>
 struct SubsmRegs {
@@ -92,7 +93,7 @@
   }
   __device__ __forceinline__ void land() {}
 };
-template <typename T, int MC, bool NT, bool PSPEC>
+template <typename T, int MC, bool NT, bool PSPEC, bool DN = false>
 struct SubsmTripCW2 : SubsmRegs<T, MC, 2>, CwPairRows {
   static_assert(sizeof(T) == 8, "compact W: fp64");
   static constexpr int NL = 2 * (6 + 2 * MC);
@@ -133,32 +134,76 @@
           }
       }
     }
+    if constexpr (DN) {
+      const int tf = __popcll(t.m0) + __popcll(t.m1);
+#pragma unroll
+      for (int j = 0; j < (PSPEC ? MC - 1 : MC); ++j)
+        if (!PSPEC && j >= c.col) this->ra[j].v = i32x4_t{0, 0, 0, 0}, this->rb[j].v = i32x4_t{0, 0, 0, 0};
+      if (2 * lane < tf) {
+#pragma unroll
+        for (int j = 0; j < (PSPEC ? MC - 1 : MC); ++j)
+          if (stored_col(c, j)) {
+            const int64_t off = (PSPEC ? (int64_t)((c.head - 1 + j) % c.m) * c.ldw : col_off(j, c.col, c.head, c.m, c.ldw)) + t.tb + 2 * lane;
+            raw_issue<16, false>(this->ra[j], c.wy + off);
+            raw_issue<16, false>(this->rb[j], c.ws + off);
+          }
+      }
+      return;
+    }
     int sl[2];
     bool lf[2];
     cw_slots(t, sl, lf);
     cols_row<false>(c, 0, t.tb + (lf[0] ? sl[0] : 0));
     cols_row<false>(c, 1, t.tb + (lf[1] ? sl[1] : 0));
   }
-  __device__ __forceinline__ void land() {
+  __device__ __forceinline__ static bool stored_col(const SubsmCtx<T> &c, int j) {
+    return PSPEC || (j < c.col && !(c.pe.on && j == c.col - 1));
+  }
+  __device__ __forceinline__ void land_cw(const SubsmCtx<T> &c) {
     raw_join_bytes(this->rnb, nb_[0], nb_[1]);
     raw_join_bytes(this->riw, iw_[0], iw_[1]);
+    if constexpr (DN) {
+      const int lane = (int)(threadIdx.x & 63);
+      int sl[2];
+      bool lf[2];
+      cw_slots(this->tile_, sl, lf);
+      const bool act = 2 * lane < __popcll(this->tile_.m0) + __popcll(this->tile_.m1);
+      i32x4_t *wa = c.scr + (threadIdx.x >> 6) * 128, *wb = wa + 64;
+      const i32x2_t *pa = reinterpret_cast<const i32x2_t *>(wa), *pb = reinterpret_cast<const i32x2_t *>(wb);
+      const int d0 = lf[0] ? sl[0] : 0, d1 = lf[1] ? sl[1] : 0;
+#pragma unroll
+      for (int j = 0; j < (PSPEC ? MC - 1 : MC); ++j)
+        if (stored_col(c, j)) {
+          if (act) wa[lane] = this->ra[j].v, wb[lane] = this->rb[j].v;
+          wave_lds_order();
+          this->ra[j].v.xy = pa[d0], this->ra[j].v.zw = pa[d1];
+          this->rb[j].v.xy = pb[d0], this->rb[j].v.zw = pb[d1];
+          wave_lds_order();
+        }
+    }
   }
 };
-template <typename T, int MC, bool NT, bool PSPEC, bool PIPE, bool CW = false>
-__global__ __launch_bounds__(BLOCK) void subsm_update_kernel(
+template <typename T, int MC, bool NT, bool PSPEC, bool PIPE, bool CW, bool DN>
+__device__ __forceinline__ void subsm_update_body(
     int64_t n, double tsum, T *__restrict__ zout, const T *pr, T *rout,
     const T *__restrict__ l, const T *__restrict__ u, const nb_t *__restrict__ nbd,
     const iw_t *__restrict__ iwhere, const T *xx, const T *__restrict__ gg,
     const T *__restrict__ ws, const T *__restrict__ wy, const T *__restrict__ zero, int64_t ldw,
     int m, int head, int col, double theta, Coef cf, Coef wv, T *dvec, T *tvec,
     T *xout, int do_stpmx, Pend pe, const T *pd, T *cwy, T *cws, int ub, double *part, int pstride,
-    const uint64_t *__restrict__ lmask = nullptr) {
+    const uint64_t *__restrict__ lmask) {
   static_assert(!CW || (sizeof(T) == 8 && MC <= 10 && !PIPE), "compact W: fp64, MC <= 10, one trip in flight");
+  static_assert(CW || !DN, "dense loads: the layout's instantiations");
   double acc[SUBSM_SIZE] = {0.0, 0.0, 0.0, 1.0e10};
   const double rtheta = 1.0 / theta;
   constexpr int V = RowsPer<T, MC>::V;
   constexpr int NS = PSPEC ? 3 : 1;
-  const SubsmCtx<T> ctx{l, u, xx, gg, ws, wy, zero, pr, pd, nbd, iwhere, ldw, m, head, col, pe, ub};
+  __shared__ i32x4_t cw_scr[DN ? (BLOCK / 64) * 128 : 1];
+  if constexpr (DN) {
+    i32x4_t *own = cw_scr + (threadIdx.x >> 6) * 128 + (threadIdx.x & 63);
+    own[0] = i32x4_t{0, 0, 0, 0}, own[64] = i32x4_t{0, 0, 0, 0};
+  }
+  const SubsmCtx<T> ctx{l, u, xx, gg, ws, wy, zero, pr, pd, nbd, iwhere, ldw, m, head, col, pe, ub, cw_scr};
   __shared__ T dict[16];
   dict_fill<T>(dict, l, u, ub);
   auto body = [&](auto &tr, int64_t i, auto wt) {
@@ -233,10 +278,36 @@
     if (xout) tr.template st_rows<NT>(xout, i, zv);
   };
   if constexpr (CW)
-    for_tiles_cw<SubsmTripCW2<T, MC, NT, PSPEC>, SubsmTripCW1<T, MC, NT, PSPEC>>(n, ctx, lmask, body);
+    for_tiles_cw<SubsmTripCW2<T, MC, NT, PSPEC, DN>, SubsmTripCW1<T, MC, NT, PSPEC>>(n, ctx, lmask, body);
   else
     for_rows_raw<SubsmTrip<T, MC, V, NT, PSPEC>, SubsmTrip<T, MC, 1, NT, PSPEC>, V, PIPE, NS>(n, ctx, body);
   block_reduce_store<SUBSM_SIZE>(acc, SUBSM_NSUM, 1, 0, part, pstride);
+}
+template <typename T, int MC, bool NT, bool PSPEC, bool PIPE, bool CW = false>
+__global__ __launch_bounds__(BLOCK) void subsm_update_kernel(
+    int64_t n, double tsum, T *__restrict__ zout, const T *pr, T *rout,
+    const T *__restrict__ l, const T *__restrict__ u, const nb_t *__restrict__ nbd,
+    const iw_t *__restrict__ iwhere, const T *xx, const T *__restrict__ gg,
+    const T *__restrict__ ws, const T *__restrict__ wy, const T *__restrict__ zero, int64_t ldw,
+    int m, int head, int col, double theta, Coef cf, Coef wv, T *dvec, T *tvec,
+    T *xout, int do_stpmx, Pend pe, const T *pd, T *cwy, T *cws, int ub, double *part, int pstride,
+    const uint64_t *__restrict__ lmask = nullptr) {
+  subsm_update_body<T, MC, NT, PSPEC, PIPE, CW, false>(
+      n, tsum, zout, pr, rout, l, u, nbd, iwhere, xx, gg, ws, wy, zero, ldw, m, head, col, theta, cf, wv, dvec, tvec, xout,
+      do_stpmx, pe, pd, cwy, cws, ub, part, pstride, lmask);
+}
+template <typename T, int MC, bool NT, bool PSPEC>
+__global__ __launch_bounds__(BLOCK) void subsm_update_kernel_dense(
+    int64_t n, double tsum, T *__restrict__ zout, const T *pr, T *rout,
+    const T *__restrict__ l, const T *__restrict__ u, const nb_t *__restrict__ nbd,
+    const iw_t *__restrict__ iwhere, const T *xx, const T *__restrict__ gg,
+    const T *__restrict__ ws, const T *__restrict__ wy, const T *__restrict__ zero, int64_t ldw,
+    int m, int head, int col, double theta, Coef cf, Coef wv, T *dvec, T *tvec,
+    T *xout, int do_stpmx, Pend pe, const T *pd, T *cwy, T *cws, int ub, double *part, int pstride,
+    const uint64_t *__restrict__ lmask) {
+  subsm_update_body<T, MC, NT, PSPEC, false, true, true>(
+      n, tsum, zout, pr, rout, l, u, nbd, iwhere, xx, gg, ws, wy, zero, ldw, m, head, col, theta, cf, wv, dvec, tvec, xout,
+      do_stpmx, pe, pd, cwy, cws, ub, part, pstride, lmask);
 }
 template <typename T>
 void launch_subsm_update(Queue &q, int64_t n, double tsum, T *zout, const T *pr, T *rout, const T *l,
@@ -253,14 +324,17 @@
     bool done = false;
     if constexpr (sizeof(T) == 8) {
       if (col <= 10) {
-#define LB_SUBSM_CW(MCV, NTV, PSPECV)                                                                           \
-  {                                                                                                             \
-    gr = grid_for_w(q, n, VecOf<T>::V, (const void *)&subsm_update_kernel<T, MCV, NTV, PSPECV, false, true>);   \
-    hipLaunchKernelGGL((subsm_update_kernel<T, MCV, NTV, PSPECV, false, true>), dim3(gr), dim3(BLOCK), 0,       \
-                       q.stream, n, tsum, zout, pr, rout, l, u, nbd, iwhere, xx, gg, w.ws, w.wy, w.zero, w.ld,   \
-                       w.m, head, col, theta, cf, wv, dvec, tvec, xout, do_stpmx, pe, pd, w.wy + slot,          \
-                       w.ws + slot, ub, part, pstride, w.lmask);                                                \
-  }
+#define LB_SUBSM_CW_(...)                                                                                      \
+  {                                                                                                           \
+    gr = grid_for_w(q, n, VecOf<T>::V, (const void *)&__VA_ARGS__);                                                  \
+    hipLaunchKernelGGL((__VA_ARGS__), dim3(gr), dim3(BLOCK), 0,                                                      \
+                       q.stream, n, tsum, zout, pr, rout, l, u, nbd, iwhere, xx, gg, w.ws, w.wy, w.zero, w.ld, \
+                       w.m, head, col, theta, cf, wv, dvec, tvec, xout, do_stpmx, pe, pd, w.wy + slot,        \
+                       w.ws + slot, ub, part, pstride, w.lmask);                                              \
+  }
+#define LB_SUBSM_CW(MCV, NTV, PSPECV) \
+  { if (q.cw_dense) { q.n_dense_subsm++; LB_SUBSM_CW_(subsm_update_kernel_dense<T, MCV, NTV, PSPECV>) } \
+    else LB_SUBSM_CW_(subsm_update_kernel<T, MCV, NTV, PSPECV, false, true>) }
         if (col <= 5) {
           if (q.nt) { if (spec) LB_SUBSM_CW(5, true, true) else LB_SUBSM_CW(5, true, false) }
           else { if (spec) LB_SUBSM_CW(5, false, true) else LB_SUBSM_CW(5, false, false) }
@@ -269,6 +343,7 @@
           else { if (spec) LB_SUBSM_CW(10, false, true) else LB_SUBSM_CW(10, false, false) }
         }
 #undef LB_SUBSM_CW
+#undef LB_SUBSM_CW_
         LB_LAUNCHED(q);
         finalize_from(q, part, pstride, gr, SUBSM_NSUM, 1, 0);
         done = true;
diff --git a/lbfgsb_amd/csrc/k_update.hip b/lbfgsb_amd/csrc/k_update.hip
--- a/lbfgsb_amd/csrc/k_update.hip
+++ b/lbfgsb_amd/csrc/k_update.hip
@@ -72,6 +72,7 @@
   int m, head, nold;
   int ub;
   const unsigned long long *ptab;
+  i32x4_t *scr = nullptr;
 };
 template <typename T, int MC, int W>
 struct UpdScanRegs {
@@ -124,7 +125,9 @@
       raw_issue<B, NTL>(this->rb[j], live ? c.ws + off : c.zero);
     }
   }
+  static constexpr bool DENSE = false;
   __device__ __forceinline__ void land() {}
+  __device__ __forceinline__ void land_cw(const UpdScanCtx<T> &) {}
   __device__ __forceinline__ void reload_cols(const UpdScanCtx<T> &c, const bool (&miss)[1]) {
     constexpr int B = (int)sizeof(T);
     RawOf<T, 1> ty[MC], ts[MC];
@@ -178,7 +181,7 @@
     cols_row<false>(c, 0, t.tb + (lf[0] ? sl[0] : 0));
     cols_row<false>(c, 1, t.tb + (lf[1] ? sl[1] : 0));
   }
-  __device__ __forceinline__ void land() {
+  __device__ __forceinline__ void land_cw(const UpdScanCtx<T> &) {
     raw_join_bytes(this->rnb, nb_[0], nb_[1]);
     raw_join_bytes(this->riw, iw_[0], iw_[1]);
   }
@@ -255,11 +258,14 @@
     }
   }
 };
-template <typename T, int MC, bool NT, bool TIGHT>
+template <typename T, int MC, bool NT, bool TIGHT, bool DN = false>
 struct UpdScanPairTripCW : CwOneRow {
   static_assert(sizeof(T) == 8, "compact W: fp64");
   static constexpr int H = MC / 2;
   static constexpr int NL = 8 + 4 * H;
+  static constexpr bool DENSE = DN;
+  bool dense_ = false;
+  int es_ = 0, re_ = 0;
   RawOf<T, 1> rx, rl, ru, rg, rr, rd;
   RawOf<T, 2> ra[H], rb[H];
   RawOf<nb_t, 1> rnb;
@@ -283,7 +289,7 @@
       raw_issue_half<NTL>(qb[jj], 1, (const T *)((gptr)p[jj].y + (dead ? 0 : a1)));
     }
   }
-  __device__ __forceinline__ void issue_cw(const UpdScanCtx<T> &c, int64_t i, int64_t slot, bool lf, int64_t first) {
+  __device__ __forceinline__ void issue_rows(const UpdScanCtx<T> &c, int64_t i, int64_t slot, bool lf) {
     constexpr int B = (int)sizeof(T);
     this->ri_ = i, this->ws_ = slot, this->lf_ = lf;
     raw_issue<B, NT>(rx, c.x + i);
@@ -294,11 +300,68 @@
     raw_issue<B, NT>(rd, c.d + i);
     raw_issue<1, false>(rnb, (c.ub & 4) ? c.nbd : c.nbd + i);
     raw_issue<1, false>(riw, c.iwhere + i);
+  }
+  __device__ __forceinline__ bool dead_col(const UpdScanCtx<T> &c, int jj) const {
+    const bool hi = threadIdx.x & 32;
+    return TIGHT ? (jj == H - 1 && hi) : (hi && H + jj >= c.nold);
+  }
+  __device__ __forceinline__ void issue_cw_run(const UpdScanCtx<T> &c, int64_t i, int64_t slot, bool lf, int64_t first,
+                                               int rs, int re) {
+    const int es = rs & ~1;
+    if (re - es > 64) {
+      issue_cw(c, i, slot, lf, first);
+      return;
+    }
+    issue_rows(c, i, slot, lf);
+    dense_ = true, es_ = es, re_ = re;
+    const bool hi = threadIdx.x & 32;
+    const int q = (int)(threadIdx.x & 31);
+    int tb = hi ? 2 * H : 0;
+    asm volatile("" : "+v"(tb));
+    u64x2 p[H];
+#pragma unroll
+    for (int jj = 0; jj < H; ++jj) p[jj] = *reinterpret_cast<const u64x2 *>(c.ptab + tb + 2 * jj);
+    const bool act = es + 2 * q < re;
+    const int64_t a = first + es + 2 * q;
+#pragma unroll
+    for (int jj = 0; jj < H; ++jj) {
+      const bool dead = dead_col(c, jj);
+      if (act || dead) {
+        raw_issue<16, false>(ra[jj], (const T *)((gptr)p[jj].x + (dead ? 0 : a)));
+        raw_issue<16, false>(rb[jj], (const T *)((gptr)p[jj].y + (dead ? 0 : a)));
+      }
+    }
+  }
+  __device__ __forceinline__ void issue_cw(const UpdScanCtx<T> &c, int64_t i, int64_t slot, bool lf, int64_t first) {
+    issue_rows(c, i, slot, lf);
+    dense_ = false;
     int64_t a0, a1;
     half_pair(lf ? slot : first, a0, a1);
     cols<false>(c, a0, a1, ra, rb);
   }
   __device__ __forceinline__ void land() {}
+  __device__ __forceinline__ void land_cw(const UpdScanCtx<T> &c) {
+    if constexpr (DN) {
+      if (dense_) {
+        const bool hi = threadIdx.x & 32;
+        const int q = (int)(threadIdx.x & 31);
+        const bool act = es_ + 2 * q < re_;
+        const int own = this->lf_ ? (int)(this->ws_ & 127) - es_ : 0;
+        int r0, r1;
+        half_pair(own, r0, r1);
+        i32x4_t *wa = c.scr + (threadIdx.x >> 6) * 128 + (hi ? 32 : 0), *wb = wa + 64;
+        const i32x2_t *pa = reinterpret_cast<const i32x2_t *>(wa), *pb = reinterpret_cast<const i32x2_t *>(wb);
+#pragma unroll
+        for (int jj = 0; jj < H; ++jj) {
+          if (act || dead_col(c, jj)) wa[q] = ra[jj].v, wb[q] = rb[jj].v;
+          wave_lds_order();
+          ra[jj].v.xy = pa[r0], ra[jj].v.zw = pa[r1];
+          rb[jj].v.xy = pb[r0], rb[jj].v.zw = pb[r1];
+          wave_lds_order();
+        }
+      }
+    }
+  }
   __device__ __forceinline__ void reload_cols(const UpdScanCtx<T> &c, const bool (&miss)[1]) {
     int mi0, mi1;
     half_pair((int)miss[0], mi0, mi1);
@@ -315,14 +378,14 @@
     }
   }
 };
-template <typename T, int MC, bool NT, bool PIPE, bool NEWROW, bool PAIR = false, bool CW = false, bool TIGHT = false>
-__global__ __launch_bounds__(BLOCK) void update_scan_kernel(
+template <typename T, int MC, bool NT, bool PIPE, bool NEWROW, bool PAIR, bool CW, bool TIGHT, bool DN>
+__device__ __forceinline__ void update_scan_body(
     int64_t n, const T *__restrict__ x, const T *__restrict__ l, const T *__restrict__ u,
     const nb_t *__restrict__ nbd, const T *__restrict__ g, const T *__restrict__ r,
     const T *__restrict__ d, int dimpl, double stp, iw_t *iwhere, T *tbrk, T *ws, T *wy,
     const T *__restrict__ zero, int64_t ldw, int m, int head, int nold, int itail, int store_pair,
     int store_iw, double cand_hi, uint64_t *ckeys, uint32_t *cidx, uint32_t ccap, uint32_t *ccount,
-    int ub, double *part, const uint64_t *__restrict__ lmask = nullptr) {
+    int ub, double *part, const uint64_t *__restrict__ lmask) {
   static_assert(!CW || (sizeof(T) == 8 && MC <= 10 && !PIPE), "compact W: fp64, MC <= 10, one trip in flight");
   static constexpr UpdScanSlots S{MC, NEWROW};
   constexpr int NA = S.size(), NSUM = S.nsum();
@@ -349,7 +412,13 @@
     }
     __syncthreads();
   }
-  const UpdScanCtx<T> ctx{x, l, u, g, r, d, ws, wy, zero, nbd, iwhere, ldw, m, head, nold, ub, ptab};
+  static_assert(!DN || (CW && PAIR), "dense loads: the layout's lane-pair instantiation");
+  __shared__ i32x4_t cw_scr[DN ? (BLOCK / 64) * 128 : 1];
+  if constexpr (DN) {
+    i32x4_t *own = cw_scr + (threadIdx.x >> 6) * 128 + (threadIdx.x & 63);
+    own[0] = i32x4_t{0, 0, 0, 0}, own[64] = i32x4_t{0, 0, 0, 0};
+  }
+  const UpdScanCtx<T> ctx{x, l, u, g, r, d, ws, wy, zero, nbd, iwhere, ldw, m, head, nold, ub, ptab, cw_scr};
   __shared__ T dict[16];
   dict_fill<T>(dict, l, u, ub);
   using TripV = std::conditional_t<PAIR, UpdScanPairTrip<T, MC, V, NT>, UpdScanTrip<T, MC, V, NT>>;
@@ -541,7 +610,7 @@
     if constexpr (!PAIR) row_stores();
   };
   if constexpr (CW && PAIR)
-    for_halves_cw<UpdScanPairTripCW<T, MC, NT, TIGHT>>(n, ctx, lmask, body);
+    for_halves_cw<UpdScanPairTripCW<T, MC, NT, TIGHT, DN>>(n, ctx, lmask, body);
   else if constexpr (CW && NEWROW)
     for_halves_cw<UpdScanTripCW1<T, MC, NT>>(n, ctx, lmask, body);
   else if constexpr (CW)
@@ -565,6 +634,30 @@
     }
   }
   block_reduce_store<NA>(acc, NSUM, 1, 1, part, MAX_BLOCKS);
+}
+template <typename T, int MC, bool NT, bool PIPE, bool NEWROW, bool PAIR = false, bool CW = false, bool TIGHT = false>
+__global__ __launch_bounds__(BLOCK) void update_scan_kernel(
+    int64_t n, const T *__restrict__ x, const T *__restrict__ l, const T *__restrict__ u,
+    const nb_t *__restrict__ nbd, const T *__restrict__ g, const T *__restrict__ r,
+    const T *__restrict__ d, int dimpl, double stp, iw_t *iwhere, T *tbrk, T *ws, T *wy,
+    const T *__restrict__ zero, int64_t ldw, int m, int head, int nold, int itail, int store_pair,
+    int store_iw, double cand_hi, uint64_t *ckeys, uint32_t *cidx, uint32_t ccap, uint32_t *ccount,
+    int ub, double *part, const uint64_t *__restrict__ lmask = nullptr) {
+  update_scan_body<T, MC, NT, PIPE, NEWROW, PAIR, CW, TIGHT, false>(
+      n, x, l, u, nbd, g, r, d, dimpl, stp, iwhere, tbrk, ws, wy, zero, ldw, m, head, nold, itail, store_pair, store_iw,
+      cand_hi, ckeys, cidx, ccap, ccount, ub, part, lmask);
+}
+template <typename T, int MC, bool NT, bool TIGHT>
+__global__ __launch_bounds__(BLOCK) void update_scan_kernel_dense(
+    int64_t n, const T *__restrict__ x, const T *__restrict__ l, const T *__restrict__ u,
+    const nb_t *__restrict__ nbd, const T *__restrict__ g, const T *__restrict__ r,
+    const T *__restrict__ d, int dimpl, double stp, iw_t *iwhere, T *tbrk, T *ws, T *wy,
+    const T *__restrict__ zero, int64_t ldw, int m, int head, int nold, int itail, int store_pair,
+    int store_iw, double cand_hi, uint64_t *ckeys, uint32_t *cidx, uint32_t ccap, uint32_t *ccount,
+    int ub, double *part, const uint64_t *__restrict__ lmask) {
+  update_scan_body<T, MC, NT, false, true, true, true, TIGHT, true>(
+      n, x, l, u, nbd, g, r, d, dimpl, stp, iwhere, tbrk, ws, wy, zero, ldw, m, head, nold, itail, store_pair, store_iw,
+      cand_hi, ckeys, cidx, ccap, ccount, ub, part, lmask);
 }
 struct SplitPlan {
   int nparts, mo;
@@ -645,21 +738,24 @@
         int nblocks = -1;
         if (nold > 5 && nrw && q.tune.pair_cw && n >= CW_TILE) {
           const int64_t n_main = n / CW_TILE * CW_TILE, n_rest = n - n_main;
-#define LB_PAIR_CW(NTV, TIGHTV)                                                                                   \
+#define LB_PAIR_CW_(...)                                                                                           \
   {                                                                                                               \
-    gr = grid_for_w(q, n_main, VecOf<T>::V,                                                                       \
-                    (const void *)&update_scan_kernel<T, 10, NTV, false, true, true, true, TIGHTV>);              \
-    hipLaunchKernelGGL((update_scan_kernel<T, 10, NTV, false, true, true, true, TIGHTV>), dim3(gr), dim3(BLOCK), 0, \
+    gr = grid_for_w(q, n_main, VecOf<T>::V, (const void *)&__VA_ARGS__);                                                 \
+    hipLaunchKernelGGL((__VA_ARGS__), dim3(gr), dim3(BLOCK), 0,                                                          \
                        q.stream, n_main, x, l, u, nbd, g, r, d, dimpl, stp, iwhere, tbrk, w.ws, w.wy, w.zero,       \
                        w.ld, w.m, head, nold, itail, store_pair, store_iw, cand_hi, ckeys, cidx, ccap, ccount, ub,   \
                        q.part(), w.lmask);                                                                          \
   }
+#define LB_PAIR_CW(NTV, TIGHTV)                                                      \
+  { if (q.cw_dense) { q.n_dense_update++; LB_PAIR_CW_(update_scan_kernel_dense<T, 10, NTV, TIGHTV>) } \
+    else LB_PAIR_CW_(update_scan_kernel<T, 10, NTV, false, true, true, true, TIGHTV>) }
           if (nold == 9) {
             if (q.nt) LB_PAIR_CW(true, true) else LB_PAIR_CW(false, true)
           } else {
             if (q.nt) LB_PAIR_CW(true, false) else LB_PAIR_CW(false, false)
           }
 #undef LB_PAIR_CW
+#undef LB_PAIR_CW_
           nblocks = gr;
           if (n_rest > 0) {
             LB_LAUNCHED(q);
diff --git a/lbfgsb_amd/csrc/kernels.hpp b/lbfgsb_amd/csrc/kernels.hpp
--- a/lbfgsb_amd/csrc/kernels.hpp
+++ b/lbfgsb_amd/csrc/kernels.hpp
@@ -47,6 +47,8 @@
   int res_off = 0;
   int split_base_min = 0;
   bool nt = false;
+  bool cw_dense = true;
+  int64_t n_dense_subsm = 0, n_dense_update = 0;
   Tune tune{};
   const char *launch_err_where = nullptr;
   hipError_t launch_err = hipSuccess;
diff --git a/lbfgsb_amd/csrc/solver_base.hpp b/lbfgsb_amd/csrc/solver_base.hpp
--- a/lbfgsb_amd/csrc/solver_base.hpp
+++ b/lbfgsb_amd/csrc/solver_base.hpp
@@ -228,6 +228,7 @@
   virtual int f_device(const double *d_f) = 0;
   hipEvent_t return_ev = nullptr;
   virtual void compact_stats(int64_t &packs, int64_t &unpacks, int &packed, int &eligible) const = 0;
+  virtual void dense_launches(int64_t &storing, int64_t &update) const = 0;
   virtual int64_t skip_scans_reused() const = 0;
   virtual void defer_counts(int64_t &deferred, int64_t &reissued) const = 0;
   bool f_pending = false;
diff --git a/lbfgsb_amd/solver.py b/lbfgsb_amd/solver.py
--- a/lbfgsb_amd/solver.py
+++ b/lbfgsb_amd/solver.py
@@ -623,6 +623,11 @@
         check(self.lib.lbfgsb_hip_comm_info(self.h, C.byref(a), C.byref(b), C.byref(k)))
         return int(a.value), int(b.value), int(k.value)
 
+    def dense_launches(self):
+        a, b = C.c_int64(0), C.c_int64(0)
+        check(self.lib.lbfgsb_hip_dense_launches(self.h, C.byref(a), C.byref(b)))
+        return a.value, b.value
+
     def compact_stats(self):
         a, b = C.c_int64(0), C.c_int64(0)
         c, d = C.c_int32(0), C.c_int32(0)
```

Result: faster. 194.2 iters/sec (median of 6 runs) (+7.5%).
